# cucibala/FaceRecognizeOnnx

Measured on AMD Instinct MI355X. Metric: faces/sec end-to-end (detect+align+embed), batch=128 640x640, higher is better.
Workload: dtype f32; 1 GPU; C-headline: 128 frames 640x640 per GPU, SCRFD det_500m + decode + NMS, first 1 face(s)/frame aligned to 112x112, IResNet-50 (w600k_r50) embed, L2-norm; frames_per_gpu=128, faces_per_frame=1, weights=synthetic seeded (det seed 100, rec seed 200), input_residency=HBM-resident before the timed region, gallery_rows=0, topk=0, parallelism=frame-sharded x1, no data-path collective

## Files before the change

### facerecognizeonnx_amd/_lib.py

```python
from __future__ import annotations

import ctypes as C
import os
import subprocess

import numpy as np

_HERE = os.path.dirname(os.path.abspath(__file__))
LIB_PATH = os.path.join(_HERE, "libfacehip.so")
CSRC = os.path.join(_HERE, "csrc")

FACE_DTYPE = np.dtype([("x", "<i4"), ("y", "<i4"), ("w", "<i4"), ("h", "<i4"),
                       ("score", "<f4"), ("lm", "<f4", (10,))])
assert FACE_DTYPE.itemsize == 60


class FhFace(C.Structure):
    _fields_ = [("x", C.c_int32), ("y", C.c_int32), ("w", C.c_int32), ("h", C.c_int32),
                ("score", C.c_float), ("lm", C.c_float * 10)]


class FhFrame(C.Structure):
    _fields_ = [("bgr", C.c_void_p), ("rows", C.c_int32), ("cols", C.c_int32), ("step", C.c_int32)]

# ... 90 lines not shown
    "fh_det_input_dev": (_vp, [_vp]),
    "fh_det_postprocess_dev": (_i, [_vp, _i, _f, _f, _vp, _i, _vp, _vp]),
    "fh_postprocess_rows_dev": (_i, [_vp, _i, _i, _i, _f, _f, _f, _vp, _i, _vp, _vp]),
    "fh_rec_create": (_vp, [C.c_char_p]),
    "fh_rec_destroy": (None, [_vp]),
    "fh_rec_input_size": (_i, [_vp, _ip, _ip]),
    "fh_rec_feature_dim": (_i, [_vp]),
    "fh_rec_macs_per_face": (_d, [_vp]),
    "fh_rec_act_bytes_per_face": (_d, [_vp]),
    "fh_rec_set_chunk": (_i, [_vp, _i]),
    "fh_rec_extract": (_i, [_vp, _vp, _i, _i, _i, _vp, _vp, _i]),
    "fh_rec_extract_simple": (_i, [_vp, _vp, _i, _i, _i, _vp, _i]),
    "fh_compare": (_f, [_vp, _i, _vp, _i]),
    "fh_rec_embed_aligned_dev": (_i, [_vp, _vp, _i, _vp, _vp, _vp]),
    "fh_rec_run_input_dev": (_i, [_vp, _vp, _i, _vp, _vp, _vp]),
    "fh_rec_align_dev": (_i, [_vp, _vp, _i, _i, _i, _ll, _vp, _vp, _i, _vp, _vp, _vp]),
    "fh_rec_input_dev": (_vp, [_vp]),
    "fh_rec_embed_faces_dev": (_i, [_vp, _vp, _i, _i, _i, _ll, _vp, _vp, _i, _vp, _vp, _vp]),
    "fh_pipeline_run_dev": (_i, [_vp, _vp, _vp, _i, _i, _i, _i, _ll, _f, _f, _i, _vp, _vp, _vp, _vp]),
    "fh_pipeline_submit_dev": (_i, [_vp, _vp, _vp, _i, _i, _i, _i, _ll, _f, _f, _i, _vp, _vp, _vp, _vp, _vp, _vp]),
    "fh_letterbox_plan": (_i, [_i, _i, _i, _i, _ip, _ip, C.POINTER(C.c_float)]),
    "fh_det_letterbox_ragged_dev": (_i, [_vp, _vp, _i, _vp, _vp]),
    "fh_det_run_network_ragged_dev": (_i, [_vp, _vp, _i, _vp]),
    "fh_det_detect_ragged_dev": (_i, [_vp, _vp, _i, _f, _f, _vp, _i, _vp, _vp]),
    "fh_rec_align_ragged_dev": (_i, [_vp, _vp, _i, _vp, _vp, _i, _vp, _vp, _vp]),
    "fh_rec_embed_faces_ragged_dev": (_i, [_vp, _vp, _i, _vp, _vp, _i, _vp, _vp, _vp]),
    "fh_pipeline_run_ragged_dev": (_i, [_vp, _vp, _vp, _i, _f, _f, _i, _vp, _vp, _vp, _vp]),
    "fh_pipeline_run_images": (_i, [_vp, _vp, _vp, _i, _f, _f, _i, _vp, _vp, _vp, _i]),
    "fh_tile_plan": (_i, [_i, _i, _vp, _vp, _i]),
    "fh_det_detect_tiled_dev": (_i, [_vp, _vp, _i, _vp, _f, _f, _vp, _i, _vp, _vp]),
    "fh_det_run_network_tiled_dev": (_i, [_vp, _vp, _i, _vp, _vp]),
    "fh_postprocess_rows_tiled_dev": (_i, [_vp, _vp, _vp, _i, _vp, _i, _i, _i, _i, _f, _f, _vp, _i, _vp, _vp]),
    "fh_pipeline_run_tiled_dev": (_i, [_vp, _vp, _vp, _i, _vp, _f, _f, _i, _vp, _vp, _vp, _vp]),
    "fh_det_detect_tiled": (_i, [_vp, _vp, _i, _i, _i, _vp, _f, _f, _vp, _i]),
    "fh_stream_create": (_vp, [_vp, _vp, _i, _i, _i, _i]),
    "fh_stream_destroy": (None, [_vp]),
    "fh_stream_submit": (_i, [_vp, _vp, _i, _f, _f]),
    "fh_stream_collect": (_i, [_vp, _vp, _vp, _vp, _i]),
    "fh_tracker_create": (_vp, [_i, _i, _f, _i, _i]),
    "fh_tracker_destroy": (None, [_vp]),
    "fh_tracker_reset": (_i, [_vp, _i]),
    "fh_tracker_get_state": (_i, [_vp, _i, _vp, _ip, _ip]),
    "fh_track_plan": (_i, [_vp, _i, _i, _vp, _vp]),
    "fh_track_update_dev": (_i, [_vp, _vp, _vp, _i, _i, _vp, _vp, _vp, _vp]),
    "fh_track_select_dev": (_i, [_vp, _vp, _i, _i, _vp, _vp, _vp, _vp, _vp, _vp]),
    "fh_pipeline_run_tracked_dev": (_i, [_vp, _vp, _vp, _vp, _i, _i, _i, _i, _ll, _vp, _f, _f, _i, _vp, _vp, _vp, _vp, _vp, _vp, _vp, _vp]),
    "fh_track_update_slots_dev": (_i, [_vp, _vp, _vp, _i, _i, _vp, _vp, _vp, _vp, _vp]),
    "fh_tracker_enable_identity": (_i, [_vp, _i, _i]),
    "fh_track_identify_dev": (_i, [_vp, _vp, _f, _vp, _vp, _vp, _vp, _i, _i, _i, _vp, _vp, _vp, _vp]),
    "fh_tracker_queries_dev": (_vp, [_vp]),
    "fh_tracker_get_identity": (_i, [_vp, _i, _vp, _vp]),
    "fh_pipeline_run_identified_dev": (_i, [_vp, _vp, _vp, _vp, _f, _vp, _i, _i, _i, _i, _ll, _vp, _f, _f, _i, _vp, _vp, _vp, _vp, _vp, _vp, _vp,
                                            _vp, _vp, _vp]),
    "fh_face_quality_dev": (_i, [_vp, _i, _i, _i, _i, _ll, _vp, _vp, _i, _vp, _vp]),
    "fh_face_quality_ragged_dev": (_i, [_vp, _i, _vp, _vp, _i, _vp, _vp]),
    "fh_tracker_set_bestshot": (_i, [_vp, _i, _i, _i, _i]),
    "fh_tracker_get_quality": (_i, [_vp, _i, _vp]),
    "fh_tracker_quality_dev": (_vp, [_vp]),
    "fh_track_update_q_dev": (_i, [_vp, _vp, _vp, _i, _i, _vp, _vp, _vp, _vp, _vp, _vp]),
    "fh_track_identify_q_dev": (_i, [_vp, _vp, _f, _vp, _vp, _vp, _vp, _vp, _i, _i, _i, _vp, _vp, _vp, _vp]),
    "fh_tracker_enable_relink": (_i, [_vp, _i, _f, _i]),
    "fh_track_identify_link_dev": (_i, [_vp, _vp, _f, _vp, _vp, _vp, _vp, _vp, _i, _i, _i, _vp, _vp, _vp, _vp, _vp]),
    "fh_tracker_get_links": (_i, [_vp, _i, _vp, _vp]),
    "fh_tracker_roots_dev": (_vp, [_vp]),
    "fh_gallery_create": (_vp, [_i]),
    "fh_gallery_destroy": (None, [_vp]),
    "fh_gallery_upload": (_i, [_vp, _vp, _ll, _i, _ll]),
    "fh_gallery_enroll": (_ll, [_vp, _vp, _ll, _i]),
    "fh_gallery_size": (_ll, [_vp]),
    "fh_gallery_label_dev": (_i, [_vp, _vp, _i, _f, _vp, _vp, _vp]),
    "fh_gallery_topk_dev": (_i, [_vp, _vp, _i, _i, _vp, _vp, _vp]),
    "fh_gallery_set_scan": (_i, [_vp, _i]),
    "fh_gallery_get_scan": (_i, [_vp]),
    "fh_gallery_scan_stats": (_i, [_vp, C.POINTER(_ll), C.POINTER(_ll)]),
    "fh_topk_merge_dev": (_i, [_vp, _vp, _i, _i, _i, _vp, _vp, _vp]),
    "fh_gallery_enroll_ids": (_ll, [_vp, _vp, _vp, _ll, _i]),
    "fh_gallery_upload_ids": (_i, [_vp, _vp, _vp, _ll, _i, _ll]),
    "fh_gallery_topk_ids_dev": (_i, [_vp, _vp, _i, _i, _vp, _vp, _vp, _vp]),
    "fh_gallery_label_ids_dev": (_i, [_vp, _vp, _i, _f, _vp, _vp, _vp]),
    "fh_gallery_remove_ids": (_ll, [_vp, _vp, _ll]),
    "fh_gallery_get_ids": (_ll, [_vp, _ll, _ll, _vp]),
    "fh_topk_merge_ids_dev": (_i, [_vp, _vp, _vp, _i, _i, _i, _vp, _vp, _vp, _vp]),
    "fh_gallery_group_ids": (_ll, [_vp, _ll, _vp, _vp, _vp]),
    "fh_gallery_fuse_ids": (_ll, [_vp, _vp, _i]),
    "fh_gallery_get_rows": (_ll, [_vp, _ll, _ll, _vp]),
    "fh_gallery_self_scores_dev": (_i, [_vp, _vp, _vp, _vp]),
    "fh_cluster_scores": (_i, [_vp, _i, _f, _i, _i, _vp, _vp]),
    "fh_gallery_cluster_dev": (_i, [_vp, _f, _i, _i, _vp, _vp, _vp]),
    "fh_hist_bin": (_i, [_f]),
    "fh_roc_from_hist": (_i, [_vp, _d, _vp]),
    "fh_gallery_pair_hist_dev": (_i, [_vp, _vp, _vp, _vp]),
    "fh_pairs_from_scores": (_i, [_vp, _i, _vp, _i, _i, _f, _i, _ll, _vp, _vp, _vp, _vp]),
    "fh_gallery_pairs_dev": (_i, [_vp, _i, _i, _f, _i, _vp, _vp, _vp, _vp, _vp]),
    "fh_gallery_set_ids": (_ll, [_vp, _vp, _i]),
    "fh_gallery_set_tags": (_ll, [_vp, _ll, _ll, _vp, _i]),
    "fh_gallery_get_tags": (_ll, [_vp, _ll, _ll, _vp]),
    "fh_gallery_topk_tagged_dev": (_i, [_vp, _vp, _vp, _i, _i, _vp, _vp, _vp]),
    "fh_gallery_topk_ids_tagged_dev": (_i, [_vp, _vp, _vp, _i, _i, _vp, _vp, _vp, _vp]),
    "fh_gallery_label_tagged_dev": (_i, [_vp, _vp, _vp, _i, _f, _vp, _vp, _vp]),
    "fh_gallery_label_ids_tagged_dev": (_i, [_vp, _vp, _vp, _i, _f, _vp, _vp, _vp]),
    "fh_gallery_tag_stats": (_i, [_vp, C.POINTER(_ll), C.POINTER(_ll)]),
    "fh_tracker_set_stream_masks": (_i, [_vp, _vp]),
    "fh_gallery_range_dev": (_i, [_vp, _vp, _vp, _i, _f, _i, _vp, _vp, _vp, _vp, _vp]),
    "fh_range_from_scores": (_i, [_vp, _ll, _ll, _vp, C.c_uint32, _f, _i, C.POINTER(_ll), _vp, _vp]),
    "fh_gallery_topk_deep_dev": (_i, [_vp, _vp, _vp, _i, _i, _vp, _vp, _vp, _vp]),
    "fh_topk_from_scores": (_i, [_vp, _ll, _ll, _vp, C.c_uint32, _i, _vp, _vp]),
    "fh_debug_deep_blocks": (_i, [_vp, _ll, _vp, C.c_uint32, _i, _vp]),
    "fh_comm_unique_id": (_i, [_vp]),
    "fh_comm_create": (_vp, [_i, _i, _vp, _i]),
    "fh_comm_destroy": (None, [_vp]),
    "fh_comm_rank": (_i, [_vp]),
    "fh_comm_world": (_i, [_vp]),
    "fh_comm_allgather_f32_dev": (_i, [_vp, _vp, _vp, _ll, _vp]),
    "fh_gallery_topk_sharded_dev": (_i, [_vp, _vp, _vp, _i, _i, _vp, _vp, _vp]),
    "fh_timing_enable": (_i, [_i]),
    "fh_timing_num_tags": (_i, []),
    "fh_timing_collect": (_i, [_vp, _vp, _vp, _vp, _i]),
    "fh_timing_collect_ops": (_i, [_vp, _vp, _vp, _i]),
    "fh_det_set_conv_cfg": (_i, [_vp, _i, _i]),
    "fh_rec_set_conv_cfg": (_i, [_vp, _i, _i]),
    "fh_memcpy_d2h": (_i, [_vp, _vp, C.c_size_t]),
    "fh_det_sync": (_i, [_vp, _vp]),
    "fh_rec_sync": (_i, [_vp, _vp]),
    "fh_imread": (_i, [C.c_char_p, C.POINTER(_vp), C.POINTER(_i), C.POINTER(_i)]),
    "fh_image_decode": (_i, [_vp, C.c_size_t, C.POINTER(_vp), C.POINTER(_i), C.POINTER(_i)]),
    "fh_image_free": (None, [_vp]),
    "fh_jpeg_header": (_i, [_vp, C.c_size_t, _vp]),
    "fh_jpeg_entropy": (_i, [_vp, C.c_size_t, _vp, _vp, C.c_size_t]),
    "fh_jpeg_reconstruct": (_i, [_vp, _vp, _vp, _i]),
    "fh_jpeg_desc_check": (_i, [_vp]),
    "fh_jpegdec_create": (_vp, []),
    "fh_jpegdec_destroy": (None, [_vp]),
    "fh_jpeg_reconstruct_batch_dev": (_i, [_vp, _vp, _i, _vp, _vp, _vp, _vp]),
    "fh_jpeg_decode_batch": (_i, [_vp, _vp, _i, _i, _vp, _vp, _vp]),
    "fh_pipeline_run_files": (_i, [_vp, _vp, _vp, _vp, _i, _i, _f, _f, _i, _vp, _vp, _vp, _i, _vp]),
    "fh_jpeg_quant_tables": (_i, [_i, _vp, _vp]),
    "fh_jpeg_enc_desc": (_i, [_i, _i, _i, _i, _i, _vp]),
    "fh_jpeg_enc_check": (_i, [_vp]),
    "fh_jpeg_forward": (_i, [_vp, _vp, _i, _vp, C.c_size_t]),
    "fh_jpeg_write": (_i, [_vp, _vp, _vp, C.c_size_t, _vp]),
    "fh_jpeg_write_bound": (C.c_size_t, [_vp]),
    "fh_imwrite_jpeg": (_i, [C.c_char_p, _vp, _i, _i, _i, _i, _i]),
    "fh_jpegenc_create": (_vp, []),
    "fh_jpegenc_destroy": (None, [_vp]),
    "fh_jpeg_forward_batch_dev": (_i, [_vp, _vp, _i, _vp, _vp, _vp, _vp]),
    "fh_jpeg_encode_batch": (_i, [_vp, _vp, _i, _i, _i, _i, _vp, _vp]),
    "fh_det_set_winograd": (_i, [_vp, _i]),
    "fh_rec_set_winograd": (_i, [_vp, _i]),
    "fh_rec_set_wino_fusion": (_i, [_vp, _i]),
    "fh_rec_set_wino_x3": (_i, [_vp, _i]),
    "fh_rec_get_wino_x3": (_i, [_vp]),
    "fh_rec_get_conv_x3": (_i, [_vp]),
    "fh_rec_get_pw_x3": (_i, [_vp]),
    "fh_det_set_x3": (_i, [_vp, _i]),
    "fh_det_get_x3": (_i, [_vp]),
    "fh_rec_set_shortcut_fold": (_i, [_vp, _i]),
    "fh_rec_set_precision": (_i, [_vp, _i, C.POINTER(C.c_float)]),
    "fh_rec_get_precision": (_i, [_vp]),
    "fh_det_set_cus": (_i, [_vp, _i]),
    "fh_rec_set_cus": (_i, [_vp, _i]),
    "fh_debug_streamk": (_i, [_i, _i]),
    "fh_debug_conv_plan": (_i, [_i, _vp, _i, _vp, _i]),
    "fh_debug_wino_slots": (_i, [_i]),
    "fh_debug_cluster_tiles": (_i, [_i]),
    "fh_debug_hist_copies": (_i, [_i]),
    "fh_debug_pairs_room": (_i, [_i]),
    "fh_debug_tag_skip": (_i, [_i]),
    "fh_debug_topk_merge_strided_dev": (_i, [_vp, _vp, _i, _i, _i, _ll, _vp, _vp, _vp]),
    "fh_set_graph_replay": (_i, [_i]),
    "fh_det_workspace_dev": (_vp, [_vp]),
    "fh_det_graph_stats": (_i, [_vp, _vp]),
    "fh_rec_graph_stats": (_i, [_vp, _vp]),
    "fh_det_set_fused_stem": (_i, [_vp, _i]),
    "fh_rec_set_fused_stem": (_i, [_vp, _i]),
    "fh_det_set_fused_front": (_i, [_vp, _i]),
    "fh_det_set_halo_conv": (_i, [_vp, _i]),
    "fh_resize_u8c3_dev": (_i, [_vp, _i, _i, _i, _vp, _i, _i, _i, _vp]),
    "fh_conv_forward_dev": (_i, [_vp, _vp, _vp, _vp, _i, _i, _i, _i, _i, _i, _i, _i, _i, _vp]),
    "fh_conv_forward_ex_dev": (_i, [_vp, _vp, _vp, _vp, _i, _i, _i, _i, _i, _i, _i, _i, _i, _i, _vp, _i, _i, _i, _i, _i, _vp]),
    "fh_conv_forward_ep_dev": (_i, [_vp, _vp, _vp, _vp, _i, _i, _i, _i, _i, _i, _i, _i, _i, _i, _vp, _i, _i, _i, _i, _i, _i, _vp, _vp]),
    "fh_conv_winograd_dev": (_i, [_vp, _vp, _vp, _vp, _i, _i, _i, _i, _i, _vp]),
    "fh_conv_winograd_ex_dev": (_i, [_vp, _vp, _vp, _vp, _i, _i, _i, _i, _i, _i, _vp]),
    "fh_debug_pack_bf16x2_dev": (_i, [_vp, _vp, _ll]),
    "fh_debug_wino_gemm_rows": (_ll, [_i, _i, _i, _i, _i, _i]),
    "fh_debug_wino_gemm_dev": (_i, [_vp, _vp, _vp, _i, _i, _i, _i, _i, _i, _i, _vp]),
    "fh_debug_wino2_clock_mhz": (_d, []),
    "fh_conv_wino2_dev": (_i, [_vp, _vp, _vp, _vp, _vp, _vp, _i, _i, _i, _i, _i, _i, _i, _vp]),
    "fh_conv_wino2_ex_dev": (_i, [_vp, _vp, _vp, _vp, _vp, _vp, _vp, _vp, _vp, _i, _vp, _vp, _vp, _i, _i, _i, _i, _i, _i, _i, _vp]),
    "fh_conv_wt_rows": (_i, [_i]),
    "fh_conv_pack_weights": (_i, [_vp, _i, _i, _i, _vp]),
    "fh_conv_kpad": (_i, [_i]),
}

_LIB = None


def lib() -> C.CDLL:
    global _LIB
    if _LIB is None:
        path = build()
        path = os.environ.get("FACEHIP_LIB") or path
        try:
            import torch
        except ImportError:
            pass
        L = C.CDLL(path)
        for name, (res, args) in PROTOTYPES.items():
            fn = getattr(L, name)
            fn.restype = res
            fn.argtypes = args
        _LIB = L
    return _LIB


def last_error() -> str:
    return lib().fh_last_error().decode(errors="replace")


class FaceHipError(RuntimeError):
    pass


def check(rc: int, what: str) -> int:
    if rc < 0:
        raise FaceHipError(f"{what} failed ({rc}): {last_error()}")
    return rc
```

### facerecognizeonnx_amd/csrc/api.cpp

```cpp
#include <algorithm>
#include <atomic>
#include <cmath>
#include <cstddef>
#include <cstdio>
#include <cstring>
#include <memory>
#include <string>
#include <thread>
#include <vector>

#include "../../include/facehip.h"
#include "cluster_plan.h"
#include "deep_plan.h"
#include "pairs_plan.h"
#include "range_plan.h"
#include "roc_plan.h"
#include "engine.h"
#include "group_ids.h"
#include "jpeg_dev.h"
#include "jpeg_enc.h"
#include "track_plan.h"

static_assert(sizeof(fh_face) == 60 && sizeof(fh::FaceRec) == 60, "FaceBox mirror must stay 60 bytes");
static_assert(sizeof(fh_frame) == 24 && sizeof(fh::FrameIn) == 24 && offsetof(fh_frame, rows) == offsetof(fh::FrameIn, rows) &&
// ... 1650 lines not shown
    return FH_OK;
}
int fh_gallery_pair_hist_dev(fh_gallery* g, unsigned long long* d_hist, unsigned long long* d_nan, void* stream) {
    if (!g || !d_hist) return arg_error("fh_gallery_pair_hist_dev: null argument");
    if (g->g.size() > 0 && !g->g.labelled()) {
        g_err = "gallery: fh_gallery_pair_hist_dev needs a labelled gallery (rows enrolled with ids, or fh_gallery_set_ids)";
        return FH_ERR_STATE;
    }
    return guarded([&] { g->g.pair_hist_dev(d_hist, d_nan, S(stream)); return (int)FH_OK; });
}
int fh_debug_hist_copies(int copies) { fh::cluster_debug_hist_copies(copies); return 0; }

static_assert(FH_PAIRS_GENUINE == fh::kPairsGenuine && FH_PAIRS_IMPOSTOR == fh::kPairsImpostor && FH_PAIRS_ANY == fh::kPairsAny &&
              FH_PAIRS_ABOVE == fh::kPairsAbove && FH_PAIRS_NOT_ABOVE == fh::kPairsNotAbove && FH_PAIRS_MAX_CAP == fh::kPairsMaxCap &&
              FH_PAIRS_ROOM == fh::kPairsRoom, "facehip.h mirrors pairs_plan.h and kernels.h");
namespace {
const char* bad_pairs(int cls, int side, float threshold, int cap) {
    if (threshold != threshold) return "the threshold is a NaN";
    if (cls != FH_PAIRS_GENUINE && cls != FH_PAIRS_IMPOSTOR && cls != FH_PAIRS_ANY) return "unknown class";
    if (side != FH_PAIRS_ABOVE && side != FH_PAIRS_NOT_ABOVE) return "unknown side";
    if (cap < 1 || cap > FH_PAIRS_MAX_CAP) return "need 1 <= cap <= FH_PAIRS_MAX_CAP";
    return nullptr;
}
}
int fh_pairs_from_scores(const float* scores, int n, const int* ids, int cls, int side, float threshold, int cap, long long room,
                         unsigned long long* info, float* out_scores, int* out_rows, int* out_ids) {
    if (const char* why = bad_pairs(cls, side, threshold, cap)) return frames_error("fh_pairs_from_scores", why);
    int listed = -1;
    const int rc = guarded([&] {
        listed = fh::pairs_from_scores(scores, n, ids, cls, side, threshold, cap, room, info, out_scores, out_rows, out_ids);
        return 0;
    });
    if (rc < 0) return rc;
    return listed < 0 ? arg_error("fh_pairs_from_scores: bad argument (n < 0, null scores or info, a class without ids, room < cap)") : listed;
}
int fh_gallery_pairs_dev(fh_gallery* g, int cls, int side, float threshold, int cap, unsigned long long* d_info, float* d_scores, int* d_rows,
                         int* d_ids, void* stream) {
    if (!g || !d_info) return arg_error("fh_gallery_pairs_dev: null argument");
    if (const char* why = bad_pairs(cls, side, threshold, cap)) return frames_error("fh_gallery_pairs_dev", why);
    if (g->g.dim() % 64) return arg_error("fh_gallery_pairs_dev: the gallery's dim must be a multiple of 64");
    if ((cls != FH_PAIRS_ANY || d_ids) && g->g.size() > 0 && !g->g.labelled()) {
        g_err = "gallery: fh_gallery_pairs_dev with a class other than FH_PAIRS_ANY or with d_ids needs a labelled gallery (rows enrolled with "
                "ids, or fh_gallery_set_ids)";
        return FH_ERR_STATE;
    }
    return guarded([&] { g->g.pairs_dev(cls, side, threshold, cap, d_info, d_scores, d_rows, d_ids, S(stream)); return (int)FH_OK; });
}
int fh_debug_pairs_room(int room) { fh::pairs_debug_room(room); return 0; }

static_assert(FH_RANGE_MAX_CAP == fh::kRangeMaxCap && FH_TAG_ALL == fh::kRangeTagAll, "facehip.h mirrors range_plan.h");
int fh_range_from_scores(const float* scores, long long n, long long index_base, const uint32_t* tags, uint32_t mask, float threshold, int cap,
                         long long* count, float* out_scores, int* out_indices) {
    int listed = -1;
    const int rc = guarded([&] {
        listed = fh::range_from_scores(scores, n, index_base, tags, mask, threshold, cap, count, out_scores, out_indices);
        return 0;
    });
    if (rc < 0) return rc;
    return listed < 0 ? arg_error("fh_range_from_scores: bad argument (null scores or count, NaN threshold, cap outside 1..1024, index beyond 31 bits)")
                      : listed;
}
int fh_gallery_range_dev(fh_gallery* g, const float* d_queries, const uint32_t* d_masks, int nq, float threshold, int cap, long long* d_counts,
                         float* d_scores, int* d_indices, int* d_ids, void* stream) {
    if (!g) return arg_error("fh_gallery_range_dev: null handle");
    if (nq < 0 || nq > 256) return arg_error("fh_gallery_range_dev: need 0 <= nq <= 256");
    if (cap < 1 || cap > FH_RANGE_MAX_CAP) return arg_error("fh_gallery_range_dev: need 1 <= cap <= FH_RANGE_MAX_CAP");
    if (threshold != threshold) return arg_error("fh_gallery_range_dev: the threshold is a NaN");
    if (g->g.dim() % 64) return arg_error("fh_gallery_range_dev: the gallery's dim must be a multiple of 64");
    if (nq == 0) return 0;
    if (!d_queries || !d_counts) return arg_error("fh_gallery_range_dev: null argument");
    if (d_ids && g->g.size() > 0 && !g->g.labelled()) {
        g_err = "gallery: fh_gallery_range_dev with d_ids needs a labelled gallery (rows enrolled with ids, or fh_gallery_set_ids)";
        return FH_ERR_STATE;
    }
    return guarded([&] { g->g.range_dev(d_queries, d_masks, nq, threshold, cap, d_counts, d_scores, d_indices, d_ids, S(stream)); return nq; });
}

static_assert(FH_TOPK_DEEP_MAX == fh::kDeepMaxK && FH_TOPK_DEEP_MAX == fh::GAL_DEEP_MAX, "facehip.h and kernels.h mirror deep_plan.h");
int fh_topk_from_scores(const float* scores, long long n, long long index_base, const uint32_t* tags, uint32_t mask, int k, float* out_scores,
                        int* out_indices) {
    int listed = -1;
    const int rc = guarded([&] {
        listed = fh::topk_from_scores(scores, n, index_base, tags, mask, k, out_scores, out_indices);
        return 0;
    });
    if (rc < 0) return rc;
    return listed < 0 ? arg_error("fh_topk_from_scores: bad argument (null scores, k outside 1..1024, index beyond 31 bits)") : listed;
}
int fh_debug_deep_blocks(const float* scores, long long n, const uint32_t* tags, uint32_t mask, int k, long long* out_blocks) {
    if (!out_blocks) return arg_error("fh_debug_deep_blocks: null argument");
    int chosen = -1;
    const int rc = guarded([&] {
        std::vector<long long> blocks;
        chosen = fh::deep_chosen_blocks(scores, n, tags, mask, k, &blocks);
        std::copy(blocks.begin(), blocks.end(), out_blocks);
        return 0;
    });
    if (rc < 0) return rc;
    return chosen < 0 ? arg_error("fh_debug_deep_blocks: bad argument (null scores, k outside 1..1024)") : chosen;
}
int fh_gallery_topk_deep_dev(fh_gallery* g, const float* d_queries, const uint32_t* d_masks, int nq, int k, float* d_scores, int* d_indices,
                             int* d_ids, void* stream) {
    if (!g) return arg_error("fh_gallery_topk_deep_dev: null handle");
    if (nq < 0 || nq > 256) return arg_error("fh_gallery_topk_deep_dev: need 0 <= nq <= 256");
    if (k < 1 || k > FH_TOPK_DEEP_MAX) return arg_error("fh_gallery_topk_deep_dev: need 1 <= k <= FH_TOPK_DEEP_MAX");
    if (g->g.dim() % 64) return arg_error("fh_gallery_topk_deep_dev: the gallery's dim must be a multiple of 64");
    if (!d_scores && !d_indices && !d_ids) return arg_error("fh_gallery_topk_deep_dev: all three list pointers are null");
    if (nq == 0) return 0;
    if (!d_queries) return arg_error("fh_gallery_topk_deep_dev: null argument");
    if (d_ids && g->g.size() > 0 && !g->g.labelled()) {
        g_err = "gallery: fh_gallery_topk_deep_dev with d_ids needs a labelled gallery (rows enrolled with ids, or fh_gallery_set_ids)";
        return FH_ERR_STATE;
    }
    return guarded([&] { g->g.topk_deep_dev(d_queries, d_masks, nq, k, d_scores, d_indices, d_ids, S(stream)); return nq; });
}

int fh_debug_topk_merge_strided_dev(const float* ps, const int* pi, int nparts, int nq, int k, long long part_stride, float* scores, int* indices,
                                    void* stream) {
    if (!ps || !pi || !scores || !indices) return arg_error("fh_debug_topk_merge_strided_dev: null argument");
    if (nparts <= 0 || nq <= 0 || k <= 0 || k > 16 || (long)nparts * k > 65536 || part_stride < (long long)nq * k)
        return arg_error("fh_debug_topk_merge_strided_dev: bad size");
    return guarded([&] {
        fh::launch_topk_merge_strided(ps, pi, nparts, nq, k, (long)part_stride, scores, indices, S(stream));
        FH_HIP(hipGetLastError());
        return nq;
    });
}

int fh_timing_enable(int on) { fh::KernelTimer::get().enabled = on != 0; return FH_OK; }
int fh_timing_num_tags(void) { return fh::KernelTimer::kTags; }
int fh_timing_collect(double* ms, double* flops, double* bytes, long long* launches, int n) {
    if (!ms || !flops || !bytes || !launches || n < fh::KernelTimer::kTags) return arg_error("fh_timing_collect: need fh_timing_num_tags()-entry arrays");
    return guarded([&] { fh::KernelTimer::get().collect(ms, flops, bytes, launches); return fh::KernelTimer::kTags; });
}
int fh_timing_collect_ops(double* ms, double* flops, int* tag, int cap) {
    if (!ms || !flops || !tag || cap <= 0) return arg_error("fh_timing_collect_ops: bad argument");
    return guarded([&] { return fh::KernelTimer::get().collect_ops(ms, flops, tag, cap); });
}
int fh_det_set_conv_cfg(fh_det* d, int cfg, int stream_k) {
    if (!d) return arg_error("null handle");
    d->det.net().force_cfg = cfg; d->det.net().sk_enable = stream_k != 0;
    return FH_OK;
}
int fh_det_set_winograd(fh_det* d, int on) { if (!d) return arg_error("null handle"); d->det.net().winograd = on != 0; return FH_OK; }
int fh_rec_set_winograd(fh_rec* r, int on) { if (!r) return arg_error("null handle"); r->rec.net().winograd = on != 0; return FH_OK; }
int fh_rec_set_wino_x3(fh_rec* r, int on) {
    if (!r) return arg_error("null handle");
    Owns owns(&r->rec.net());
    return guarded([&] { return r->rec.net().set_wino_x3(on != 0, nullptr); });
}
int fh_rec_get_wino_x3(fh_rec* r) { return r && r->rec.net().wino_x3() ? 1 : 0; }
int fh_rec_get_conv_x3(fh_rec* r) { return r ? r->rec.net().conv_x3_layers() : 0; }
int fh_rec_get_pw_x3(fh_rec* r) { return r ? r->rec.net().pw_x3_layers() : 0; }
int fh_det_set_x3(fh_det* d, int on) {
    if (!d) return arg_error("null handle");
    Owns owns(&d->det.net());
    return guarded([&] { return d->det.net().set_pw_x3(on != 0, nullptr); });
}
int fh_det_get_x3(fh_det* d) { return d ? d->det.net().pw_x3_layers() : 0; }
int fh_rec_set_wino_fusion(fh_rec* r, int on) { if (!r) return arg_error("null handle"); r->rec.net().fuse_wino = on != 0; return FH_OK; }
int fh_rec_set_precision(fh_rec* r, int mode, float* worst_out) {
    if (!r || (mode != FH_PREC_FP32 && mode != FH_PREC_BF16X2)) return arg_error("fh_rec_set_precision: bad argument");
    if (worst_out) *worst_out = 0.f;
    Owns owns(&r->rec.net());
    if (mode == FH_PREC_FP32) return guarded([&] { r->rec.net().set_bf16x2(false, nullptr); return (int)FH_OK; });
    return guarded([&] {
        fh::Net& net = r->rec.net();
        const int n = 64, dim = r->rec.dim();
        const size_t crop = (size_t)net.in_h() * net.in_w() * 3;
        std::vector<uint8_t> h((size_t)n * crop);
        uint32_t st = 0x9E3779B9u;
        for (int i = 0; i < n; ++i) {
            const int amp = 16 + 3 * i;
            for (size_t e = 0; e < crop; ++e) {
                st = st * 1664525u + 1013904223u;
                const int px = (int)(e / 3) % net.in_w(), py = (int)(e / 3) / net.in_w();
                const int v = 128 + ((px * (i + 1) + py * (n - i)) % 97 - 48) + (int)((st >> 24) % (2 * amp + 1)) - amp;
                h[(size_t)i * crop + e] = (uint8_t)std::min(255, std::max(0, v));
            }
        }
        fh::DevBuf dc, de;
        dc.ensure(h.size()); de.ensure((size_t)2 * n * dim * sizeof(float));
        FH_HIP(hipMemcpy(dc.p, h.data(), h.size(), hipMemcpyHostToDevice));
        const bool was = net.bf16x2();
        net.set_bf16x2(false, nullptr);
        r->rec.embed_aligned_dev(dc.as<uint8_t>(), n, de.as<float>(), nullptr);
        const int layers = net.set_bf16x2(true, nullptr);
        if (layers == 0) { net.set_bf16x2(was, nullptr); throw std::runtime_error("fh_rec_set_precision: this model has no layer with a split-bf16 form"); }
        struct Rollback { fh::Net& n; bool armed = true; ~Rollback() { if (armed) { try { n.set_bf16x2(false, nullptr); } catch (...) {} } } } rollback{net};
        r->rec.embed_aligned_dev(dc.as<uint8_t>(), n, de.as<float>() + (size_t)n * dim, nullptr);
        std::vector<float> e((size_t)2 * n * dim);
        FH_HIP(hipDeviceSynchronize());
        FH_HIP(hipMemcpy(e.data(), de.p, e.size() * sizeof(float), hipMemcpyDeviceToHost));
        double worst = 0;
        for (int i = 0; i < n; ++i) {
            double dot = 0, na = 0, nb = 0;
            for (int c = 0; c < dim; ++c) {
                const double a = e[(size_t)i * dim + c], b = e[(size_t)(n + i) * dim + c];
                dot += a * b; na += a * a; nb += b * b;
            }
            const double err = (na > 0 && nb > 0) ? 1.0 - dot / std::sqrt(na * nb) : 1.0;
            worst = std::max(worst, std::isfinite(err) ? err : 1.0);
        }
        if (worst_out) *worst_out = (float)worst;
        double gate = 1e-3;
        if (const char* g = getenv("FACEHIP_PRECISION_GATE")) gate = std::min(gate, atof(g));
        if (!(worst < gate))
            throw std::runtime_error("fh_rec_set_precision: split-bf16 embeddings differ from fp32 by 1 - cos = " + std::to_string(worst) +
                                 " (gate " + std::to_string(gate) + "): staying fp32");
        rollback.armed = false;
        return layers;
    });
}
int fh_rec_get_precision(fh_rec* r) { return r && r->rec.net().bf16x2() ? FH_PREC_BF16X2 : FH_PREC_FP32; }
int fh_rec_set_shortcut_fold(fh_rec* r, int on) { if (!r) return arg_error("null handle"); r->rec.net().fold_shortcut = on != 0; return FH_OK; }
int fh_det_set_halo_conv(fh_det* d, int on) { if (!d) return arg_error("null handle"); d->det.net().halo_conv = on != 0; return FH_OK; }
int fh_det_set_cus(fh_det* d, int cus) { if (!d || cus < 0) return arg_error("bad argument"); d->det.net().cus = cus; return FH_OK; }
int fh_rec_set_cus(fh_rec* r, int cus) { if (!r || cus < 0) return arg_error("bad argument"); r->rec.net().cus = cus; return FH_OK; }
int fh_det_set_fused_stem(fh_det* d, int on) { if (!d) return arg_error("null handle"); d->det.net().fuse_stem = on != 0; return FH_OK; }
int fh_det_set_fused_front(fh_det* d, int on) { if (!d) return arg_error("null handle"); d->det.net().fuse_front = on != 0; return FH_OK; }
int fh_rec_set_fused_stem(fh_rec* r, int on) { if (!r) return arg_error("null handle"); r->rec.net().fuse_stem = on != 0; return FH_OK; }
int fh_rec_set_conv_cfg(fh_rec* r, int cfg, int stream_k) {
    if (!r) return arg_error("null handle");
    r->rec.net().force_cfg = cfg; r->rec.net().sk_enable = stream_k != 0;
    return FH_OK;
}

int fh_memcpy_d2h(void* dst, const void* src, size_t bytes) {
    if (!dst || !src) return arg_error("fh_memcpy_d2h: null argument");
    return guarded([&] { FH_HIP(hipDeviceSynchronize()); FH_HIP(hipMemcpy(dst, src, bytes, hipMemcpyDeviceToHost)); return 0; });
}
int fh_resize_u8c3_dev(const uint8_t* src, int sh, int sw, int sstep, uint8_t* dst, int dh, int dw, int dstep, void* stream) {
    if (!src || !dst || sh <= 0 || sw <= 0 || dh <= 0 || dw <= 0) return arg_error("fh_resize_u8c3_dev: bad argument");
    return guarded([&] {
        fh::launch_resize_u8c3(src, (long)sh * sstep, sh, sw, sstep, dst, (long)dh * dstep, dh, dw, dstep, 1, S(stream));
        FH_HIP(hipGetLastError());
        return 0;
    });
}
int fh_conv_winograd_ex_dev(const float* d_in, const float* w_ohwi, const float* d_bias, float* d_out, int batch, int h, int w, int cin,
                            int cout, int precision, void* stream) {
    if (!d_in || !w_ohwi || !d_out || cin % 32 || cout % 4 || (precision != FH_PREC_FP32 && precision != FH_PREC_BF16X2 && precision != FH_PREC_F32X3))
        return arg_error("fh_conv_winograd_dev: bad argument");
    const bool bf2 = precision == FH_PREC_BF16X2, x3 = precision == FH_PREC_F32X3;
    Owns owns(nullptr);
    return guarded([&] {
        if ((bf2 || x3) && !fh::wino_gemm_ok_bf16x2(cin, cout)) throw std::runtime_error("winograd: this layer has no split-bf16 GEMM");
        const int rows = fh::conv_wt_rows(cout);
        std::vector<float> u36((size_t)36 * rows * cin, 0.f), uf((size_t)cout * cin);
        std::vector<double> uall((size_t)cout * cin * 36);
        for (int co = 0; co < cout; ++co)
            for (int ci = 0; ci < cin; ++ci) {
                double g[9];
                for (int t = 0; t < 9; ++t) g[t] = w_ohwi[((size_t)co * 9 + t) * cin + ci];
                fh::wino_filter_transform(g, &uall[((size_t)co * cin + ci) * 36]);
            }
        for (int f = 0; f < 36; ++f) {
            for (size_t e = 0; e < uf.size(); ++e) uf[e] = (float)uall[e * 36 + f];
            fh::conv_pack_weights(uf.data(), cout, cin, 1, u36.data() + (size_t)f * rows * cin);
        }
        const size_t tiles = (size_t)batch * ((h + 3) / 4) * ((w + 3) / 4);
        fh::DevBuf dU, dV, dM;
        dU.ensure(u36.size() * sizeof(float));
        dV.ensure((36 * (size_t)fh::wino_rows((long)tiles) + 100 * 128) * cin * sizeof(float));
        dM.ensure((36 * (size_t)fh::wino_rows((long)tiles) + 100 * 128) * cout * sizeof(float));
        FH_HIP(hipMemcpy(dU.p, u36.data(), u36.size() * sizeof(float), hipMemcpyHostToDevice));
        fh::DevBuf dUp;
        if (bf2) {
            dUp.ensure(u36.size() * sizeof(float));
            fh::launch_pack_bf16x2(dU.as<float>(), dUp.as<float>(), (long)u36.size(), S(stream));
        } else if (x3) {
            dUp.ensure(36 * fh::wino_x3_floats(rows, cin) * sizeof(float));
            fh::launch_pack_x3(dU.as<float>(), dUp.as<float>(), rows, cin, S(stream));
        }
        static fh::DevBuf slabs;
        static unsigned slabs_gen = 0;
        if (!slabs.p) { slabs.ensure(fh::conv_slab_floats() * sizeof(float)); fh::conv_workspace_init(slabs.as<float>()); slabs_gen = fh::conv_error_generation(); }
        if (slabs_gen != fh::conv_error_generation()) { fh::conv_workspace_reset_async(slabs.as<float>(), S(stream)); slabs_gen = fh::conv_error_generation(); }
        fh::ConvArgs a{};
        a.in = d_in; a.bias = d_bias; a.out1 = d_out; a.slabs = slabs.as<float>(); a.sk_enable = 1;
        a.B = batch; a.H = h; a.W = w; a.Ho = h; a.Wo = w; a.Cin = cin; a.Cout = cout; a.ks = 3; a.stride = 1; a.pad = 1;
        a.act = (int)fh::Act::NONE; a.res_mode = (int)fh::ResMode::NONE;
        fh::launch_conv_winograd(a, (bf2 || x3 ? dUp : dU).as<float>(), dV.as<float>(), dM.as<float>(), 2, nullptr, nullptr, S(stream), precision);
        FH_HIP(hipStreamSynchronize(S(stream)));
        return 0;
    });
}
int fh_conv_winograd_dev(const float* d_in, const float* w_ohwi, const float* d_bias, float* d_out, int batch, int h, int w, int cin,
                         int cout, void* stream) {
    return fh_conv_winograd_ex_dev(d_in, w_ohwi, d_bias, d_out, batch, h, w, cin, cout, FH_PREC_FP32, stream);
}
int fh_debug_pack_bf16x2_dev(const float* d_in, float* d_out, long long n) {
    if (!d_in || !d_out || n < 0 || n % 4) return arg_error("fh_debug_pack_bf16x2_dev: bad argument (n % 4 == 0)");
    return guarded([&] {
        fh::launch_pack_bf16x2(d_in, d_out, (long)n, nullptr);
        FH_HIP(hipGetLastError());
        FH_HIP(hipStreamSynchronize(nullptr));
        return 0;
    });
}
static long long wino_gemm_rows(int batch, int h, int w, int k, int n, int mixed, fh::WinoPlanes* pl) {
    if (batch <= 0 || h <= 0 || w <= 0 || k <= 0 || n <= 0 || k % 32 || n % 32) return -1;
    if (!mixed) return 36LL * fh::wino_rows((long)batch * ((h + 3) / 4) * ((w + 3) / 4));
    fh::WinoPlanes p{};
    if (!fh::wino_mix_layout(batch, h, w, k, n, &p)) return -2;
    if (pl) *pl = p;
    return 128LL * p.total_tiles;
}
long long fh_debug_wino_gemm_rows(int batch, int h, int w, int k, int n, int mixed) {
    const long long r = wino_gemm_rows(batch, h, w, k, n, mixed, nullptr);
    if (r == -2) return arg_error("fh_debug_wino_gemm_rows: the mixed tiling does not apply to this layer");
    if (r < 0) return arg_error("fh_debug_wino_gemm_rows: bad argument (k % 32 == 0, n % 32 == 0)");
    return r;
}
int fh_debug_wino_gemm_dev(const float* d_V, const float* d_U, float* d_M, int batch, int h, int w, int k, int n, int precision, int mixed,
                           void* stream) {
    if (!d_V || !d_U || !d_M || (precision != FH_PREC_FP32 && precision != FH_PREC_BF16X2 && precision != FH_PREC_F32X3))
        return arg_error("fh_debug_wino_gemm_dev: bad argument");
    fh::WinoPlanes pl{};
    const long long rows = wino_gemm_rows(batch, h, w, k, n, mixed, &pl);
    if (rows == -2) return arg_error("fh_debug_wino_gemm_dev: the mixed tiling does not apply to this layer");
    if (rows < 0) return arg_error("fh_debug_wino_gemm_dev: bad argument (k % 32 == 0, n % 32 == 0)");
    const bool bf2 = precision == FH_PREC_BF16X2, x3 = precision == FH_PREC_F32X3;
    Owns owns(nullptr);
    return guarded([&] {
        if ((bf2 || x3) && !fh::wino_gemm_ok_bf16x2(k, n)) throw std::runtime_error("winograd: this layer has no split-bf16 GEMM");
        const size_t nv = (size_t)rows * k, nu = (size_t)36 * fh::conv_wt_rows(n) * k;
        fh::DevBuf dVp, dUp;
        if (bf2) {
            dVp.ensure(nv * sizeof(float)); dUp.ensure(nu * sizeof(float));
            fh::launch_pack_bf16x2(d_V, dVp.as<float>(), (long)nv, S(stream));
            fh::launch_pack_bf16x2(d_U, dUp.as<float>(), (long)nu, S(stream));
        } else if (x3) {
            dUp.ensure(36 * fh::wino_x3_floats(fh::conv_wt_rows(n), k) * sizeof(float));
            fh::launch_pack_x3(d_U, dUp.as<float>(), fh::conv_wt_rows(n), k, S(stream));
        }
        fh::ConvArgs a{};
        a.B = batch; a.H = h; a.W = w; a.Ho = h; a.Wo = w; a.Cin = k; a.Cout = n; a.ks = 3; a.stride = 1; a.pad = 1;
        a.act = (int)fh::Act::NONE; a.res_mode = (int)fh::ResMode::NONE;
        fh::launch_wino_gemm(a, bf2 || x3 ? dUp.as<float>() : d_U, bf2 ? dVp.as<float>() : d_V, d_M, 2, precision, S(stream), mixed ? &pl : nullptr);
        FH_HIP(hipGetLastError());
        FH_HIP(hipStreamSynchronize(S(stream)));
        return 0;
    });
}
int fh_conv_wino2_ex_dev(const float* d_in, const float* w_ohwi, const float* d_bias, const float* d_slope, const float* d_res, float* d_out,
                         float* d_out2, const float* d_s2, const float* d_t2, int n_outs, float* const* d_outs, const int* oc0, const int* oact,
                         int batch, int h, int w, int cin, int cout, int act, int bias_cls, void* stream) {
    if (!d_in || !w_ohwi || batch <= 0 || h <= 0 || w <= 0 || cin != 64 || cout <= 0) return arg_error("fh_conv_wino2_dev: bad argument (cin = 64, positive sizes)");
    if (n_outs < 0 || n_outs > 3 || (n_outs > 0 && (!d_outs || !oc0 || !oact))) return arg_error("fh_conv_wino2_dev: bad merged-output description");
    if (n_outs == 0 && ((!d_out && !d_out2) || cout % 64)) return arg_error("fh_conv_wino2_dev: plain layers need an output and cout % 64 == 0");
    if (d_out2 && (!d_s2 || !d_t2)) return arg_error("fh_conv_wino2_dev: a second output needs its scale and shift");
    Owns owns(nullptr);
    return guarded([&] {
        fh::ConvArgs a{};
        a.in = d_in; a.bias = d_bias; a.slope = d_slope; a.res = d_res; a.out1 = d_out; a.out2 = d_out2; a.s2 = d_s2; a.t2 = d_t2;
        a.B = batch; a.H = h; a.W = w; a.Ho = h; a.Wo = w; a.Cin = cin; a.Cout = cout; a.ks = 3; a.stride = 1; a.pad = 1;
        a.act = act; a.bias_cls = bias_cls; a.res_mode = d_res ? (int)fh::ResMode::SAME : (int)fh::ResMode::NONE;
        a.n_outs = n_outs;
        for (int g = 0; g < n_outs; ++g) { a.outs[g] = d_outs[g]; a.oact[g] = oact[g]; a.oc0[g] = oc0[g]; }
        if (n_outs > 0) a.oc0[n_outs] = oc0[n_outs];
        if (!fh::wino2_ok(a)) throw std::runtime_error("fh_conv_wino2_dev: layer shape not supported by the fused F(2x2) kernel");
        std::vector<float> u(fh::wino2_weight_floats(cin, cout));
        fh::wino2_pack_weights(w_ohwi, cout, cin, u.data());
        fh::DevBuf dU;
        dU.ensure(u.size() * sizeof(float));
        FH_HIP(hipMemcpy(dU.p, u.data(), u.size() * sizeof(float), hipMemcpyHostToDevice));
        a.wt = dU.as<float>();
        fh::launch_wino2(a, S(stream));
        FH_HIP(hipGetLastError());
        FH_HIP(hipStreamSynchronize(S(stream)));
        return 0;
    });
}
int fh_conv_wino2_dev(const float* d_in, const float* w_ohwi, const float* d_bias, const float* d_slope, const float* d_res, float* d_out,
                      int batch, int h, int w, int cin, int cout, int act, int bias_cls, void* stream) {
    return fh_conv_wino2_ex_dev(d_in, w_ohwi, d_bias, d_slope, d_res, d_out, nullptr, nullptr, nullptr, 0, nullptr, nullptr, nullptr, batch, h, w,
                                cin, cout, act, bias_cls, stream);
}
double fh_debug_wino2_clock_mhz(void) { return fh::wino2_debug_clock_mhz(); }
int fh_conv_wt_rows(int cout) { return fh::conv_wt_rows(cout); }
int fh_conv_pack_weights(const float* w_ohwi, int cout, int cin, int ksize, float* dst_packed) {
    if (!w_ohwi || !dst_packed || cout <= 0 || cin <= 0) return arg_error("fh_conv_pack_weights: bad argument");
    memset(dst_packed, 0, (size_t)fh::conv_wt_rows(cout) * fh::conv_kpad(ksize * ksize * cin) * sizeof(float));
    fh::conv_pack_weights(w_ohwi, cout, cin, ksize, dst_packed);
    return 0;
}
int fh_conv_kpad(int ktot) { return fh::conv_kpad(ktot); }
const float* fh_det_workspace_dev(fh_det* d) { return d ? d->det.net().workspace() : nullptr; }
int fh_set_graph_replay(int on) { g_graph_replay = on != 0; return FH_OK; }
int fh_det_graph_stats(fh_det* d, long long* replays) {
    if (!d) return arg_error("null handle");
    if (replays) *replays = d->gcall.replays;
    return (int)d->gcall.nodes;
}
int fh_rec_graph_stats(fh_rec* r, long long* replays) {
    if (!r) return arg_error("null handle");
    if (replays) *replays = r->gcall.replays + r->gcall_simple.replays;
    return (int)(r->gcall.nodes ? r->gcall.nodes : r->gcall_simple.nodes);
}
int fh_debug_wino_slots(int slots) { fh::wino_debug_slots(slots); return 0; }
int fh_debug_streamk(int drop_publish, int timeout_ms) { fh::conv_debug_streamk(drop_publish, timeout_ms); return 0; }
int fh_debug_conv_plan(int what, const int* in, int n_in, long long* out, int n_out) {
    static const int BMs[4] = {128, 256, 128, 64}, BNs[4] = {128, 64, 32, 64};
    const fh::ConvKnobs knobs;
    auto need = [&](int ni, int no) { return n_in == ni && n_out == no && out && (in || !ni); };
    auto geom = [&] {
        const int Ho = (in[1] + 2 * in[7] - in[5]) / in[6] + 1, Wo = (in[2] + 2 * in[7] - in[5]) / in[6] + 1;
        return fh::ConvGeom{(long)in[0] * Ho * Wo, in[1], in[2], in[3], Ho, Wo, in[4], in[5], in[6], in[7], fh::conv_kpad(in[5] * in[5] * in[3]), in[8],
                            false, false, in[9] != 0, false};
    };
    auto shape_ok = [&] { return in[0] > 0 && in[1] > 0 && in[2] > 0 && in[3] > 0 && in[4] > 0 && in[5] > 0 && in[6] > 0 && in[7] >= 0 && in[10] > 0 &&
                                 in[1] + 2 * in[7] >= in[5] && in[2] + 2 * in[7] >= in[5]; };
    if (what == 0 && need(8, 9) && in[0] >= 0 && in[1] > 0 && in[2] > 0 && in[3] > 0 && in[4] > 0) {
        const fh::ConvSkPlan p = fh::conv_streamk_plan(in[0], in[1], in[2], in[3], in[4], in[5], in[6], in[7] != 0, knobs);
        const int v[9] = {p.full, p.rem, p.helpers, p.owners, p.fixup, p.units, p.q, p.owner_chunks, p.maxp};
        for (int i = 0; i < 9; ++i) out[i] = v[i];
    } else if (what == 1 && need(11, 1) && shape_ok()) {
        out[0] = fh::conv_pw_bn(geom(), in[10], knobs);
    } else if (what == 2 && need(12, 3) && shape_ok() && in[11] >= -1 && in[11] < 4) {
        const fh::ConvGeom g = geom();
        const int cfg = in[11] < 0 ? fh::conv_pick_cfg(g.M, g.Cout) : in[11], BM = BMs[cfg], BN = BNs[cfg];
        const int tiles_n = (g.Cout + BN - 1) / BN, tiles = (int)((g.M + BM - 1) / BM) * tiles_n;
        fh::ConvTallPlan t{0, 0, 0};
        if (cfg == 1 || cfg == 2) t = fh::conv_tall_plan(g, BM, BN, 32, tiles, tiles_n, in[10], knobs);
        out[0] = t.tiles; out[1] = t.tiles ? t.rows_a : 0; out[2] = t.tiles ? (long long)t.lds : 0;
    } else if (what == 3 && need(4, 2) && in[0] >= 0 && in[1] > in[0] && in[2] > 0 && in[3] > 0) {
        out[0] = out[1] = fh::conv_sk_nparts(in[0], in[2], in[3]);
        for (int r = in[0] + 1; r < in[1]; ++r) {
            const int n = fh::conv_sk_nparts(r, in[2], in[3]);
            if (n < out[0]) out[0] = n;
            if (n > out[1]) out[1] = n;
        }
    } else if (what == 4 && need(0, 2)) {
        out[0] = (long long)fh::SK_SLAB_FLOATS; out[1] = (long long)fh::SK_COUNTERS;
    } else if (what == 5 && need(4, 2) && in[0] >= 0 && in[1] > 0 && in[2] > 0 && in[3] > 0) {
        out[0] = fh::conv_x3_pays(in[0], in[1], in[2], in[3], knobs) ? 1 : 0; out[1] = fh::conv_x3_bn(in[2]);
    } else if (what == 6 && need(11, 3) && shape_ok()) {
        const fh::ConvGeom g = geom();
        const int bn = fh::conv_pw_x3_bn(g, in[10], knobs);
        out[0] = bn; out[1] = bn ? (g.M / 128) * ((g.Cout + bn - 1) / bn) : 0;
        out[2] = bn && fh::conv_pw_x3_pays(out[1], g.Kpad, g.Cout, in[10], knobs) ? 1 : 0;
    } else if (what == 7 && need(4, 1) && in[0] >= 0 && in[1] > 0 && in[2] > 0 && in[3] > 0) {
        out[0] = fh::conv_pw_x3_pays(in[0], in[1], in[2], in[3], knobs) ? 1 : 0;
    } else {
        return arg_error("fh_debug_conv_plan: unknown question, wrong array lengths or a non-positive size");
    }
    return n_out;
}
int fh_conv_forward_dev(const float* in, const float* wt, const float* bias, float* out, int batch, int h, int w, int cin, int cout,
                        int ks, int stride, int kpad, int cfg, void* stream) {
    return fh_conv_forward_ex_dev(in, wt, bias, out, batch, h, w, cin, cout, ks, stride, kpad, cfg, FH_PREC_FP32, nullptr, 0, 0, 0, 0, 0, stream);
}
int fh_conv_forward_ex_dev(const float* in, const float* wt, const float* bias, float* out, int batch, int h, int w, int cin, int cout,
                           int ks, int stride, int kpad, int cfg, int precision, const float* sc_in, int sc_h, int sc_w, int sc_c, int sc_stride,
                           int cus, void* stream) {
    return fh_conv_forward_ep_dev(in, wt, bias, out, batch, h, w, cin, cout, ks, stride, kpad, cfg, precision, sc_in, sc_h, sc_w, sc_c, sc_stride, cus,
                                  0, nullptr, stream);
}
int fh_conv_forward_ep_dev(const float* in, const float* wt, const float* bias, float* out, int batch, int h, int w, int cin, int cout,
                           int ks, int stride, int kpad, int cfg, int precision, const float* sc_in, int sc_h, int sc_w, int sc_c, int sc_stride,
                           int cus, int act, const float* res, void* stream) {
    static const char* const no_pw_x3 = "fh_conv_forward_ex_dev: this 1x1 layer has no three-piece bf16 form (it needs stride 1, cin % 4 == 0, "
                                        "cout % 4 == 0, kpad % 32 == 0, whole 128-row tiles and a tile per CU)";
    const bool x3 = precision == FH_PREC_F32X3, pw3 = x3 && ks == 1;
    if (pw3 && in && wt && out && batch > 0 && cin > 0 && cout > 0 && (cin % 4 || cout % 4 || stride != 1 || sc_in || kpad % 32 || kpad < cin))
        return arg_error(no_pw_x3);
    if (!in || !wt || !out || batch <= 0 || (ks != 1 && ks != 3) || cin % 4 || cout <= 0 || stride <= 0 || cus < 0 || (act != 0 && act != 1) ||
        (precision != FH_PREC_FP32 && precision != FH_PREC_F32X3) || (sc_in && (sc_h <= 0 || sc_w <= 0 || sc_c <= 0 || sc_stride <= 0)))
        return arg_error("fh_conv_forward_dev: bad argument");
    if (x3 && !pw3 && !fh::conv_x3_ok(cin, cout))
        return arg_error("fh_conv_forward_ex_dev: this layer has no three-piece bf16 form (it needs cin % 32 == 0 and cout % 64 == 0)");
    Owns owns(nullptr);
    return guarded([&] {
        fh::ConvArgs a{};
        const int pad = ks / 2;
        a.in = in; a.wt = wt; a.bias = bias; a.out1 = out;
        a.B = batch; a.H = h; a.W = w; a.Cin = cin; a.Cout = cout; a.ks = ks; a.stride = stride; a.pad = pad;
        a.Ho = (h + 2 * pad - ks) / stride + 1; a.Wo = (w + 2 * pad - ks) / stride + 1;
        a.Kpad = kpad;
        a.cus = cus;
        a.act = act;
        if (res) { a.res = res; a.res_mode = (int)fh::ResMode::SAME; }
        if (sc_in) {
            if ((a.Ho - 1) * sc_stride >= sc_h || (a.Wo - 1) * sc_stride >= sc_w) throw std::runtime_error("conv: the shortcut's input does not cover the output grid");
            a.sc_in = sc_in; a.sc_H = sc_h; a.sc_W = sc_w; a.sc_C = sc_c; a.sc_stride = sc_stride;
        }
        static fh::DevBuf slabs;
        static unsigned slabs_gen = 0;
        if (!slabs.p) { slabs.ensure(fh::conv_slab_floats() * sizeof(float)); fh::conv_workspace_init(slabs.as<float>()); slabs_gen = fh::conv_error_generation(); }
        if (slabs_gen != fh::conv_error_generation()) { fh::conv_workspace_reset_async(slabs.as<float>(), S(stream)); slabs_gen = fh::conv_error_generation(); }
        a.slabs = slabs.as<float>(); a.sk_enable = 1;
        if (x3) {
            static fh::DevBuf w3;
            const int rows = fh::conv_wt_rows(cout);
            FH_HIP(hipStreamSynchronize(S(stream)));
            w3.ensure(fh::wino_x3_floats(rows, kpad) * sizeof(float));
            fh::launch_pack_x3(wt, w3.as<float>(), rows, kpad, S(stream), 1);
            if (pw3) {
                if (!fh::launch_conv_pw_x3(a, w3.as<float>(), true, S(stream))) throw std::invalid_argument(no_pw_x3);
            } else {
                a.wt = w3.as<float>();
                fh::launch_conv_x3(a, 0, S(stream));
            }
            FH_HIP(hipGetLastError());
            FH_HIP(hipStreamSynchronize(S(stream)));
            return 0;
        }
        fh::launch_conv(a, cfg, S(stream));
        FH_HIP(hipGetLastError());
        return 0;
    });
}

}

namespace fh {
Gallery& gallery_of(fh_gallery* g) { return g->g; }
}
```

### facerecognizeonnx_amd/csrc/conv_plan.h

```cpp
#pragma once
#include <cstddef>
#include <cstdlib>

#if defined(__HIPCC__)
#define FH_CONV_HD __host__ __device__
#else
#define FH_CONV_HD
#endif

namespace fh {

constexpr size_t SK_SLAB_FLOATS = (size_t)2 * 1280 * 128 * 128;
constexpr size_t SK_COUNTERS = 4096;

struct ConvKnobs {
    int sk_b_ratio = 4;
    int sk_min_owner = 12;
    int sk_margin2 = 3;
    int tall_tail_q = 3;
    int conv_pw = 1;
    int conv_tall = 1;
    int ep_direct = 0;
    int conv_x3 = 1;
    int pw_x3 = 1;
    int pw_x3_bn = 0;
};
inline const ConvKnobs& conv_knobs() {
    static const ConvKnobs k = [] {
        ConvKnobs v;
        auto env = [](const char* name, int& x) { if (const char* e = getenv(name)) x = atoi(e); };
        env("FACEHIP_SK_B_RATIO", v.sk_b_ratio); env("FACEHIP_SK_MIN_OWNER", v.sk_min_owner); env("FACEHIP_SK_MARGIN", v.sk_margin2);
        env("FACEHIP_TALL_TAIL_Q", v.tall_tail_q); env("FACEHIP_CONV_PW", v.conv_pw); env("FACEHIP_CONV_TALL", v.conv_tall);
        env("FACEHIP_EP_DIRECT", v.ep_direct); env("FACEHIP_CONV_X3", v.conv_x3); env("FACEHIP_PW_X3", v.pw_x3); env("FACEHIP_PW_X3_BN", v.pw_x3_bn);
        return v;
    }();
    return k;
}

struct ConvGeom {
    long M;
    int H, W, Cin, Ho, Wo, Cout, ks, stride, pad, Kpad, n_outs;
    bool grouped, sc, up2x, no_pw;
};

inline int conv_pick_cfg(long M, int Cout) {
    auto cols = [&](int bn) { return (Cout + bn - 1) / bn * bn; };
    int bn = 32;
    if (cols(64) * 10 <= cols(32) * 11) bn = 64;
    if (cols(128) * 10 <= cols(bn) * 11) bn = 128;
    if (bn == 128) return 0;
    if (bn == 64) return (M / 256) * (cols(64) / 64) >= 1024 ? 1 : 3;
    return 2;
}

inline int conv_x3_bn(int Cout) { return Cout <= 0 ? 0 : Cout % 128 == 0 ? 128 : Cout % 64 == 0 ? 64 : 0; }
inline bool conv_x3_pays(long tiles, int Kpad, int Cout, int cus, const ConvKnobs& k) {
    if (!k.conv_x3 || !conv_x3_bn(Cout) || Kpad % 32 || cus <= 0) return false;
    if (k.conv_x3 == 2) return true;
    return tiles * 16 >= (long)cus && Kpad >= 640;
}

inline double conv_tile_us(long tile_floats, int Kpad) { return 2.0 * tile_floats * (double)Kpad / 0.43e6; }

inline int conv_pw_bn(const ConvGeom& g, int cus, const ConvKnobs& k) {
    if (!k.conv_pw || g.no_pw || g.ks != 1 || g.stride != 1 || g.pad != 0 || g.grouped || g.sc || g.n_outs > 0 || (g.Cin & 3) || (g.Cout & 3) ||
        (g.M & 127) || g.H != g.Ho || g.W != g.Wo || g.Kpad % 32 || g.Kpad < g.Cin)
        return 0;
    auto cols = [&](int bn) { return (g.Cout + bn - 1) / bn * bn; };
    int bn = 32;
    if (cols(64) * 100 <= g.Cout * 107) bn = 64;
    if (cols(96) * 100 <= g.Cout * 107 && cols(96) <= cols(64)) bn = 96;
    return (g.M / 128) * (cols(bn) / bn) < (long)cus ? 0 : bn;
}

inline int conv_pw_x3_bn(const ConvGeom& g, int cus, const ConvKnobs& k) {
    if (!conv_pw_bn(g, cus, k)) return 0;
    auto cols = [&](int bn) { return (g.Cout + bn - 1) / bn * bn; };
    int bn = k.pw_x3_bn == 64 ? 64 : 32;
    if (cols(64) * 100 <= g.Cout * 107) bn = 64;
    if (cols(96) * 100 <= g.Cout * 107 && cols(96) <= cols(64)) bn = 96;
    return (g.M / 128) * (cols(bn) / bn) < (long)cus ? 0 : bn;
}
constexpr int PW_X3_MIN_KPAD = 64;
inline bool conv_pw_x3_pays(long tiles, int Kpad, int Cout, int cus, const ConvKnobs& k) {
    if (!k.pw_x3 || Cout <= 0 || (Cout & 3) || Kpad <= 0 || Kpad % 32 || cus <= 0) return false;
    if (k.pw_x3 == 2) return true;
    return tiles >= (long)cus * (Cout < 32 ? 2 : 1) && Kpad >= PW_X3_MIN_KPAD;
}

struct ConvTallPlan { int tiles, rows_a; size_t lds; };
inline ConvTallPlan conv_tall_plan(const ConvGeom& g, int BM, int BN, int rp, int T, int tiles_n, int cus, const ConvKnobs& k) {
    const int occ = BM == 256 ? 2 : 3;
    const int St = cus * occ;
    ConvTallPlan t{0, 0, 0};
    if (!k.conv_tall || g.grouped || g.sc || g.ks != 3 || g.stride != 1 || g.pad != 1 || (g.Cin & 31) || g.H != g.Ho || g.W != g.Wo || g.W > 112 ||
        !(BN == 32 ? g.n_outs > 0 || (g.Cout & 3) == 0 : g.n_outs == 0 && (g.Cout & 3) == 0) || g.up2x || T < St)
        return t;
    t.rows_a = (BM + 2 * g.W + 2 + rp - 1) / rp * rp;
    t.lds = ((size_t)t.rows_a * 8 + 2 * BN * 8) * 16;
    t.tiles = (T / St) * St;
    t.tiles -= t.tiles % tiles_n;
    if (t.tiles > 0 && T - t.tiles <= cus && conv_tile_us((long)BM * BN, g.Kpad) < 30.0) t.tiles = T;
    if (t.lds > (size_t)(160 / occ) * 1024) t.tiles = 0;
    return t;
}

FH_CONV_HD inline int conv_sk_nparts(int r, int Kh, int q) { return ((r + 1) * Kh - 1) / q - (r * Kh) / q + 1; }

struct ConvSkPlan { int full, rem, helpers, owners, fixup, units, q, owner_chunks, maxp; };
inline ConvSkPlan conv_streamk_plan(int T, int S, int chunks, long tile_floats, int cus, int Kpad, int tile0, bool slabs_ok, const ConvKnobs& k) {
    ConvSkPlan pl{(T / S) * S, 0, 0, 0, 0, 0, 1, 0, 1};
    const int R = T - pl.full;
    const bool cheap_whole = ((R + cus - 1) / cus - (double)R / cus) * conv_tile_us(tile_floats, Kpad) < 10.0;
    if (R > 0 && R * 10 <= S * 9 && slabs_ok && !cheap_whole) {
        const int H = S - R;
        const int q_o = (int)(((long)R * chunks + (long)H * k.sk_margin2 / 2 + S - 1) / S);
        const int Kh = chunks - q_o;
        if (Kh >= 1 && q_o >= k.sk_min_owner && R <= (int)SK_COUNTERS) {
            const long U = (long)R * Kh;
            const int q_h = (int)((U + H - 1) / H);
            const int maxp = (Kh + q_h - 1) / q_h + 1;
            if (maxp <= 3 && (size_t)R * maxp * tile_floats <= SK_SLAB_FLOATS) {
                pl.units = (int)U; pl.q = q_h; pl.owner_chunks = q_o; pl.maxp = maxp;
                pl.helpers = (int)((U + q_h - 1) / q_h); pl.owners = R;
            }
        }
        if (!pl.owners) {
            const long U = (long)R * chunks;
            int q = (int)((U + S - 1) / S);
            const int min_q = tile0 > 0 ? (chunks < k.tall_tail_q ? chunks : k.tall_tail_q) : chunks < 8 ? chunks : chunks >= 256 ? 24 : 8;
            if (q < min_q) q = min_q;
            const int maxp = (chunks + q - 1) / q + 1;
            if (q * k.sk_b_ratio <= chunks * 2 && q < chunks && (size_t)R * maxp * tile_floats <= SK_SLAB_FLOATS) {
                pl.units = (int)U; pl.q = q; pl.maxp = maxp;
                pl.helpers = (int)((U + q - 1) / q); pl.fixup = 1;
            }
        }
    }
    if (pl.helpers) pl.rem = R; else pl.full = T;
    return pl;
}

}
```

### facerecognizeonnx_amd/csrc/conv_wino2.hip

```cpp
#include <hip/hip_runtime.h>

#include <algorithm>
#include <cstdlib>
#include <cstring>
#include <stdexcept>
#include <vector>

#include "gemm_tile.h"
#include "kernels.h"
#include "plan.h"

namespace fh {

namespace {

__device__ __forceinline__ float act1(float v, bool relu, float sl) {
    const float a = v >= 0.f ? v : v * sl;
    return relu ? fmaxf(v, 0.f) : a;
}

constexpr int kYA[4] = {0, 1, 2, 1}, kYB[4] = {2, 2, 1, 3};
constexpr int kSA[4] = {1, 1, 1, 1}, kSB[4] = {-1, 1, -1, -1};
constexpr int kAT[2][4] = {{1, 1, 1, 0}, {0, 1, -1, -1}};

// ... 86 lines not shown
            if constexpr (c11 != 0) asm volatile("" : "+v"(Y[1][1][cb]));
        }
    };
    v4f d[2][4] = {};
    auto fetch_d = [&](auto fc, auto jc, auto bc) __attribute__((always_inline)) {
        constexpr int f = decltype(fc)::value, j = decltype(jc)::value, buf = decltype(bc)::value;
        constexpr int fi = f >> 2, fj = f & 3;
        constexpr int ya = kYA[fi], yb = kYB[fi], xa = kYA[fj], xb = kYB[fj];
        if (abl_d) return;
        unsigned gxr = j << 6;
        asm volatile("" : "+s"(gxr));
        d[buf][0] = *reinterpret_cast<lds_v4f>((size_t)(rb[ya * 4 + xa] ^ gxr));
        d[buf][1] = *reinterpret_cast<lds_v4f>((size_t)(rb[ya * 4 + xb] ^ gxr));
        d[buf][2] = *reinterpret_cast<lds_v4f>((size_t)(rb[yb * 4 + xa] ^ gxr));
        d[buf][3] = *reinterpret_cast<lds_v4f>((size_t)(rb[yb * 4 + xb] ^ gxr));
    };
    auto stage = [&](auto fc) __attribute__((always_inline)) {
        constexpr int f = decltype(fc)::value;
        constexpr int fi = f >> 2, fj = f & 3;
        constexpr int sab = kSA[fi] * kSB[fj], sba = kSB[fi] * kSA[fj], sbb = kSB[fi] * kSB[fj];
        v4f M[CB];
#pragma unroll
        for (int cb = 0; cb < CB; ++cb) M[cb] = v4f{0.f, 0.f, 0.f, 0.f};
        auto step = [&](auto jc) __attribute__((always_inline)) {
            constexpr int j = decltype(jc)::value, k = f * 4 + j;
            fetch_w(k + WD - 1 < 64, (k + WD - 1) % WD);
            if constexpr (j < 3) fetch_d(IC<f>{}, IC<j + 1>{}, IC<(k + 1) & 1>{});
            else if constexpr (f < 15) fetch_d(IC<f + 1>{}, IC<0>{}, IC<(k + 1) & 1>{});
            __builtin_amdgcn_sched_barrier(0);
            const v4f* dd = d[k & 1];
            v4f v = dd[0];
            v = sab > 0 ? v + dd[1] : v - dd[1];
            v = sba > 0 ? v + dd[2] : v - dd[2];
            v = sbb > 0 ? v + dd[3] : v - dd[3];
            asm volatile("" : "+v"(v));
            __builtin_amdgcn_sched_barrier(0);
#pragma unroll
            for (int e = 0; e < 4; ++e)
#pragma unroll
                for (int cb = 0; cb < CB; ++cb) M[cb] = __builtin_amdgcn_mfma_f32_16x16x4f32(wr[k % WD][cb][e], v[e], M[cb], 0, 0, 0);
            __builtin_amdgcn_sched_barrier(0);
        };
        step(IC<0>{}); step(IC<1>{});
        y_update(IC<(f + 15) & 15>{}, Mp);
        step(IC<2>{}); step(IC<3>{});
#pragma unroll
        for (int cb = 0; cb < CB; ++cb) Mp[cb] = M[cb];
        __builtin_amdgcn_sched_barrier(0);
    };
    fetch_w(false, 0);
#pragma unroll
    for (int q = 1; q < WD - 1; ++q) fetch_w(true, q);
    asm volatile("s_waitcnt vmcnt(0)" ::: "memory");
    if constexpr (NW > 1) __syncthreads();
    fetch_d(IC<0>{}, IC<0>{}, IC<0>{});
    stage(IC<0>{}); stage(IC<1>{}); stage(IC<2>{}); stage(IC<3>{}); stage(IC<4>{}); stage(IC<5>{}); stage(IC<6>{}); stage(IC<7>{});
    stage(IC<8>{}); stage(IC<9>{}); stage(IC<10>{}); stage(IC<11>{}); stage(IC<12>{}); stage(IC<13>{}); stage(IC<14>{}); stage(IC<15>{});
    y_update(IC<15>{}, Mp);

    asm volatile("" ::: "memory");
    __builtin_amdgcn_sched_barrier(0);
    if (abl_st && lane != 0) return;
    const int oy0 = 2 * (4 * gy + tr), ox0 = 2 * (4 * gx + tc);
    const int n0 = (tile_n * NW + wv) * 16 * CB, Cout = p.Cout;
    const float* __restrict__ res = p.res;
    float* __restrict__ out1 = p.out1;
    float* __restrict__ out2 = p.out2;
    const bool relu = p.act == (int)Act::RELU, prelu = p.act == (int)Act::PRELU;
    float bm[CB][4];
    if constexpr (MERGED) {
#pragma unroll
        for (int cb = 0; cb < CB; ++cb)
#pragma unroll
            for (int e = 0; e < 4; ++e) { const int co = n0 + 16 * cb + 4 * kq + e; bm[cb][e] = co < Cout ? p.bias[co] : 0.f; }
    }
#pragma unroll
    for (int a = 0; a < 2; ++a)
#pragma unroll
        for (int b = 0; b < 2; ++b) {
            const int oy = oy0 + a, ox = ox0 + b;
            if (!MERGED || oy >= p.Ho || ox >= p.Wo) continue;
            const size_t pix = ((size_t)gn * p.Ho + oy) * p.Wo + ox;
            if constexpr (MERGED) {
#pragma unroll
                for (int cb = 0; cb < CB; ++cb)
#pragma unroll
                    for (int e = 0; e < 4; e += 2) {
                        const int co = n0 + 16 * cb + 4 * kq + e;
                        if (co >= Cout) continue;
                        const int g = co >= p.oc0[2] && p.n_outs > 2 ? 2 : co >= p.oc0[1] ? 1 : 0;
                        const int cg = p.oc0[g + 1] - p.oc0[g], ga = p.oact[g];
                        auto fin = [&](float v) { return ga == (int)Act::RELU ? fmaxf(v, 0.f) : ga == (int)Act::SIGMOID ? 1.0f / (1.0f + expf(-v)) : v; };
                        float* const dst = p.outs[g] + pix * cg + (co - p.oc0[g]);
                        const float v0 = fin(Y[a][b][cb][e] + bm[cb][e]);
                        if (co + 1 < p.oc0[g + 1] && !((cg | (co - p.oc0[g])) & 1)) {
                            *reinterpret_cast<float2*>(dst) = float2{v0, fin(Y[a][b][cb][e + 1] + bm[cb][e + 1])};
                        } else {
                            dst[0] = v0;
                            if (co + 1 < Cout) {
                                const int g1 = co + 1 >= p.oc0[2] && p.n_outs > 2 ? 2 : co + 1 >= p.oc0[1] ? 1 : 0;
                                const int cg1 = p.oc0[g1 + 1] - p.oc0[g1], ga1 = p.oact[g1];
                                float v1 = Y[a][b][cb][e + 1] + bm[cb][e + 1];
                                v1 = ga1 == (int)Act::RELU ? fmaxf(v1, 0.f) : ga1 == (int)Act::SIGMOID ? 1.0f / (1.0f + expf(-v1)) : v1;
                                p.outs[g1][pix * cg1 + (co + 1 - p.oc0[g1])] = v1;
                            }
                        }
                    }
                continue;
            }
        }
    if constexpr (!MERGED) {
        const int n0 = (tile_n * NW + wv) * 16 * CB + 4 * kq;
        bool live[4]; size_t row[4]; v4f b4[4][CB], r4[4][CB], sl[CB];
#pragma unroll
        for (int cb = 0; cb < CB; ++cb) sl[cb] = prelu ? *reinterpret_cast<const v4f*>(p.slope + n0 + 16 * cb) : v4f{1.f, 1.f, 1.f, 1.f};
#pragma unroll
        for (int q = 0; q < 4; ++q) {
            const int oy = oy0 + (q >> 1), ox = ox0 + (q & 1);
            live[q] = oy < p.Ho && ox < p.Wo;
            const int oyc = min(oy, p.Ho - 1), oxc = min(ox, p.Wo - 1);
            row[q] = (((size_t)gn * p.Ho + oyc) * p.Wo + oxc) * Cout + n0;
            const int cls = p.bias_cls ? 3 * (oyc == 0 ? 0 : oyc == p.Ho - 1 ? 2 : 1) + (oxc == 0 ? 0 : oxc == p.Wo - 1 ? 2 : 1) : 0;
#pragma unroll
            for (int cb = 0; cb < CB; ++cb) {
                b4[q][cb] = p.bias ? *reinterpret_cast<const v4f*>(p.bias + cls * Cout + n0 + 16 * cb) : v4f{0.f, 0.f, 0.f, 0.f};
                if (p.res_mode != (int)ResMode::NONE) r4[q][cb] = *reinterpret_cast<const v4f*>(res + row[q] + 16 * cb);
            }
        }
#pragma unroll
        for (int q = 0; q < 4; ++q) {
            if (!live[q]) continue;
#pragma unroll
            for (int cb = 0; cb < CB; ++cb) {
                v4f v;
#pragma unroll
                for (int e = 0; e < 4; ++e) v[e] = act1(Y[q >> 1][q & 1][cb][e] + b4[q][cb][e], relu, sl[cb][e]);
                if (p.res_mode != (int)ResMode::NONE) v += r4[q][cb];
                if (out1) *reinterpret_cast<v4f*>(out1 + row[q] + 16 * cb) = v;
                if (out2) {
                    const v4f s2 = *reinterpret_cast<const v4f*>(p.s2 + n0 + 16 * cb), t2 = *reinterpret_cast<const v4f*>(p.t2 + n0 + 16 * cb);
                    *reinterpret_cast<v4f*>(out2 + row[q] + 16 * cb) = v * s2 + t2;
                }
            }
        }
    }
#ifdef FACEHIP_W2_PROF
    if (lane == 0 && p.slabs && blockIdx.x < (1u << 17)) {
        const long long dc = __builtin_readcyclecounter() - prof_c0, dr = (long long)__builtin_amdgcn_s_memrealtime() - prof_r0;
        reinterpret_cast<float*>(p.slabs)[blockIdx.x] = (float)(dc * 1000 / (dr + 1));
    }
#endif
}

bool shape_ok(int Cin, int Cout) { return Cin == 64 && (Cout % 64 == 0 || Cout <= 32); }

template <int CB, int NW, bool MERGED>
void launch_cb(const ConvArgs& a, hipStream_t s) {
    const int tgy = ((a.H + 1) / 2 + 3) / 4, tgx = ((a.W + 1) / 2 + 3) / 4;
    const long n_tg = (long)a.B * tgy * tgx;
    const int tiles_n = (a.Cout + 16 * CB * NW - 1) / (16 * CB * NW);
    static const bool lds_ok = [] {
        hipFuncAttributes fa{};
        FH_HIP(hipFuncGetAttributes(&fa, reinterpret_cast<const void*>(&wino2_kernel<CB, NW, MERGED>)));
        return fa.sharedSizeBytes % 256 == 0;
    }();
    if (!lds_ok) throw std::runtime_error("wino2: static LDS moved the halo off its 256-byte alignment (see the address XOR in fetch_d)");
    KernelTimer& timer = KernelTimer::get();
    timer.begin(s);
    hipLaunchKernelGGL((wino2_kernel<CB, NW, MERGED>), dim3((unsigned)(n_tg * tiles_n)), dim3(64 * NW), 25600, s, a, tiles_n, tgx, tgy, (int)n_tg);
    timer.end(s, 12, 2.0 * 16 * 16.0 * (double)n_tg * a.Cin * (16.0 * CB * NW * tiles_n), a.t_flops);
}

}

size_t wino2_weight_floats(int Cin, int Cout) { return (size_t)16 * Cin * (Cout <= 32 ? 32 : Cout); }
void wino2_pack_weights(const float* w, int Cout, int Cin, float* dst) {
    static const double Gm[4][3] = {{1, 0, 0}, {.5, .5, .5}, {.5, -.5, .5}, {0, 0, 1}};
    if (!shape_ok(Cin, Cout)) throw std::runtime_error("wino2_pack_weights: layer shape not supported");
    const int CB = Cout <= 32 ? 2 : 4;
    memset(dst, 0, wino2_weight_floats(Cin, Cout) * sizeof(float));
    for (int co = 0; co < Cout; ++co)
        for (int ci = 0; ci < Cin; ++ci) {
            double g[3][3], t[4][3];
            for (int k = 0; k < 9; ++k) g[k / 3][k % 3] = w[((size_t)co * 9 + k) * Cin + ci];
            for (int i = 0; i < 4; ++i)
                for (int x = 0; x < 3; ++x) t[i][x] = Gm[i][0] * g[0][x] + Gm[i][1] * g[1][x] + Gm[i][2] * g[2][x];
            const int tn = co / (16 * CB), cb = (co % (16 * CB)) / 16, m = co % 16;
            const int j = ci / 16, kq = (ci % 16) / 4, e = ci % 4;
            for (int i = 0; i < 4; ++i)
                for (int jj = 0; jj < 4; ++jj) {
                    const double u = t[i][0] * Gm[jj][0] + t[i][1] * Gm[jj][1] + t[i][2] * Gm[jj][2];
                    const size_t step = ((size_t)tn * 16 + (i * 4 + jj)) * 4 + j;
                    dst[(step * CB + cb) * 256 + (kq * 16 + m) * 4 + e] = (float)u;
                }
        }
}

bool wino2_ok(const ConvArgs& a) {
    if (!(a.ks == 3 && a.stride == 1 && a.pad == 1 && a.H == a.Ho && a.W == a.Wo && a.H >= 2 && a.W >= 2 && shape_ok(a.Cin, a.Cout) &&
          a.act != (int)Act::SIGMOID && !a.sc_in && !a.dw_w && !a.u8_src && a.wt_group_rows == 0 &&
          (a.res_mode == (int)ResMode::NONE || a.res_mode == (int)ResMode::SAME)))
        return false;
    if (a.n_outs > 0)
        return a.Cout <= 32 && a.res_mode == (int)ResMode::NONE && !a.out2 && !a.bias_cls;
    return a.Cout % 64 == 0;
}

static float* g_w2_clock = nullptr;
double wino2_debug_clock_mhz() {
    if (!g_w2_clock) return 0.0;
    std::vector<float> h(1 << 17);
    if (hipMemcpy(h.data(), g_w2_clock, h.size() * sizeof(float), hipMemcpyDeviceToHost) != hipSuccess) return 0.0;
    std::vector<float> v;
    for (float x : h) if (x > 0.f) v.push_back(x);
    if (v.empty()) return 0.0;
    std::nth_element(v.begin(), v.begin() + v.size() / 2, v.end());
    return v[v.size() / 2] / 10.0;
}

long wino2_blocks(const ConvArgs& a) {
    return (long)a.B * (((a.H + 1) / 2 + 3) / 4) * (((a.W + 1) / 2 + 3) / 4) * ((a.Cout + 63) / 64) / 4;
}

void launch_wino2(const ConvArgs& a_in, hipStream_t s) {
    if (!wino2_ok(a_in)) throw std::runtime_error("launch_wino2: layer shape not supported");
    ConvArgs a = a_in;
    a.zeros = conv_zero_line();
    static const int ablate = [] { const char* e = getenv("FACEHIP_W2_ABLATE"); return e ? atoi(e) : -1; }();
    a.sk_test_drop = ablate < 0 ? 0 : ablate;
    if (ablate >= 0 && !g_w2_clock) { void* q = nullptr; if (hipMalloc(&q, sizeof(float) << 17) == hipSuccess) g_w2_clock = (float*)q; }
    if (g_w2_clock) (void)hipMemsetAsync(g_w2_clock, 0, sizeof(float) << 17, s);
    a.slabs = g_w2_clock;
    static const int nw = [] { const char* e = getenv("FACEHIP_WINO2_NW"); return e ? atoi(e) : 2; }();
    if (a.Cout <= 32) launch_cb<2, 1, true>(a, s);
    else if (nw == 2) launch_cb<2, 2, false>(a, s);
    else launch_cb<4, 1, false>(a, s);
}

}
```

### facerecognizeonnx_amd/csrc/engine.cpp

```cpp
#include "engine.h"

#include "group_ids.h"
#include "roc_plan.h"

#include <atomic>
#include <climits>
#include <cstdio>
#include <cstdlib>
#include <algorithm>
#include <cmath>
#include <cstring>

namespace fh {

void hip_check(hipError_t e, const char* what) {
    if (e != hipSuccess) throw std::runtime_error(std::string("HIP error: ") + hipGetErrorString(e) + " in " + what);
}

static std::atomic<unsigned long long> g_layout_epoch{1};
unsigned long long layout_epoch() { return g_layout_epoch.load(std::memory_order_relaxed); }

DevBuf::~DevBuf() {
    if (p) { (void)hipFree(p); g_layout_epoch.fetch_add(1, std::memory_order_relaxed); }
}
// ... 6 lines not shown
}

KernelTimer& KernelTimer::get() { static KernelTimer t; return t; }
hipEvent_t KernelTimer::take() {
    if (!pool_.empty()) { hipEvent_t e = pool_.back(); pool_.pop_back(); return e; }
    hipEvent_t e; FH_HIP(hipEventCreate(&e)); return e;
}
void KernelTimer::begin(hipStream_t s) {
    if (!enabled) return;
    cur_ = take();
    FH_HIP(hipEventRecord(cur_, s));
}
void KernelTimer::end(hipStream_t s, int tag, double flops, double bytes) {
    if (!enabled || !cur_) return;
    hipEvent_t b = take();
    FH_HIP(hipEventRecord(b, s));
    recs_.push_back(Rec{cur_, b, tag, flops, bytes});
    cur_ = nullptr;
}
void KernelTimer::collect(double* ms, double* flops, double* bytes, long long* launches) {
    for (int i = 0; i < kTags; ++i) { ms[i] = 0; flops[i] = 0; bytes[i] = 0; launches[i] = 0; }
    for (auto& r : recs_) {
        FH_HIP(hipEventSynchronize(r.b));
        float t = 0.f;
        FH_HIP(hipEventElapsedTime(&t, r.a, r.b));
        ms[r.tag] += t; flops[r.tag] += r.flops; bytes[r.tag] += r.bytes; launches[r.tag] += 1;
        pool_.push_back(r.a); pool_.push_back(r.b);
    }
    recs_.clear();
}

int KernelTimer::collect_ops(double* ms, double* flops, int* tag, int cap) {
    int n = 0;
    for (auto& r : recs_) {
        FH_HIP(hipEventSynchronize(r.b));
        float t = 0.f;
        FH_HIP(hipEventElapsedTime(&t, r.a, r.b));
        if (n < cap) { ms[n] = t; flops[n] = r.flops; tag[n] = r.tag; ++n; }
        pool_.push_back(r.a); pool_.push_back(r.b);
    }
    recs_.clear();
    return n;
}

static bool debug_sync() {
    static int v = -1;
    if (v < 0) { const char* e = getenv("FACEHIP_DEBUG_SYNC"); v = e ? atoi(e) : 0; }
    return v != 0;
}


static constexpr int kWinoMinCin = 128;
static constexpr long kWinoMinTiles = 256;
static long wino2_min_blocks() {
    static long v = -1;
    if (v < 0) {
        const char* e = getenv("FACEHIP_WINO2");
        const char* m = getenv("FACEHIP_WINO2_MIN");
        v = e && atoi(e) == 0 ? (1L << 60) : m ? atol(m) : 64;
    }
    return v;
}

Net::Net(const std::string& onnx_path, int default_h, int default_w) {
    OnnxModel m = load_onnx(onnx_path);
    int H = default_h, W = default_w;
    const auto& shp = m.inputs[0].shape;
    if (shp.size() == 4) {
        if (shp[2] > 0) H = (int)shp[2];
        if (shp[3] > 0) W = (int)shp[3];
    }
    plan_ = build_plan(m, H, W);

    std::vector<float> host;
    auto push = [&](const float* src, size_t n) {
        size_t off = (host.size() + 63) / 64 * 64;
        host.resize(off + n, 0.f);
        if (n) memcpy(host.data() + off, src, n * sizeof(float));
        return off;
    };
    dev_.resize(plan_.ops.size());
    for (size_t i = 0; i < plan_.ops.size(); ++i) {
        POp& c = plan_.ops[i];
        if (c.bn_src < 0 || c.kind != OpKind::CONV || c.ks != 3 || c.stride != 1 || c.pad != 1 || c.H < 2 || c.W < 2) continue;
        const bool wino_ok = c.Cin >= kWinoMinCin && c.Cin % 32 == 0 && c.Cout % 4 == 0 && c.outs.empty() && c.res_mode != ResMode::UP2X;
        const POp& pr = plan_.ops[c.bn_src];
        if (wino_ok || !c.outs.empty() || (int)pr.s2.size() < c.Cin || pr.out < 0) continue;
        std::vector<float> b9((size_t)9 * c.Cout);
        for (int co = 0; co < c.Cout; ++co) {
            double tap_shift[9];
            for (int t = 0; t < 9; ++t) {
                double acc = 0;
                for (int ci = 0; ci < c.Cin; ++ci) acc += (double)c.weight[((size_t)co * 9 + t) * c.Cin + ci] * pr.t2[ci];
                tap_shift[t] = acc;
            }
            for (int ry = 0; ry < 3; ++ry)
                for (int rx = 0; rx < 3; ++rx) {
                    double b = c.bias[co];
                    for (int ky = 0; ky < 3; ++ky)
                        for (int kx = 0; kx < 3; ++kx) {
                            const bool in_y = !(ry == 0 && ky == 0) && !(ry == 2 && ky == 2);
                            const bool in_x = !(rx == 0 && kx == 0) && !(rx == 2 && kx == 2);
                            if (in_y && in_x) b += tap_shift[ky * 3 + kx];
                        }
                    b9[(size_t)(ry * 3 + rx) * c.Cout + co] = (float)b;
                }
            for (int t = 0; t < 9; ++t)
                for (int ci = 0; ci < c.Cin; ++ci) c.weight[((size_t)co * 9 + t) * c.Cin + ci] *= pr.s2[ci];
        }
        c.bias = b9;
        dev_[i].bn_fold_src = c.bn_src;
        dev_[c.bn_src].bn_fold_dst = true;
    }
    for (size_t i = 0; i < plan_.ops.size(); ++i) {
        const POp& op = plan_.ops[i];
        DevOp& d = dev_[i];
        if (op.kind == OpKind::DWPW) {
            d.dww = push(op.dw_weight.data(), op.dw_weight.size());
            d.dwb = push(op.dw_bias.data(), op.dw_bias.size());
        }
        if (op.kind == OpKind::CONV || op.kind == OpKind::GEMM || op.kind == OpKind::DWPW) {
            const int Ktot = op.ks * op.ks * op.Cin;
            d.Kpad = conv_kpad(Ktot);
            const int rows = conv_wt_rows(op.Cout);
            std::vector<float> packed((size_t)rows * d.Kpad, 0.f);
            conv_pack_weights(op.weight.data(), op.Cout, op.Cin, op.ks, packed.data());
            d.wt = push(packed.data(), packed.size());
            if (op.kind == OpKind::CONV) {
                ConvArgs probe{};
                probe.ks = op.ks; probe.stride = op.stride; probe.pad = op.pad; probe.Cin = op.Cin; probe.Cout = op.Cout; probe.act = (int)op.act;
                probe.res_mode = (int)op.res_mode; probe.H = op.H; probe.W = op.W;
                float dummy = 0.f;
                probe.out2 = op.out2 >= 0 ? &dummy : nullptr;
                probe.bias_cls = dev_[i].bn_fold_src >= 0 ? 1 : 0;
                if (conv_halo_ok(probe) && op.Ho * op.Wo >= 400) {
                    std::vector<float> wf(conv_halo_wfrag_floats(op.Cin, op.Cout));
                    conv_halo_pack_weights(op.weight.data(), op.Cout, op.Cin, wf.data());
                    d.wfrag = push(wf.data(), wf.size());
                    d.halo = true;
                }
            }
            if (op.kind == OpKind::CONV && op.Cin < kWinoMinCin) {
                ConvArgs probe{};
                probe.ks = op.ks; probe.stride = op.stride; probe.pad = op.pad; probe.Cin = op.Cin; probe.Cout = op.Cout; probe.act = (int)op.act;
                probe.res_mode = (int)op.res_mode; probe.H = op.H; probe.W = op.W; probe.Ho = op.Ho; probe.Wo = op.Wo;
                probe.n_outs = (int)op.outs.size(); probe.bias_cls = dev_[i].bn_fold_src >= 0 ? 1 : 0;
                float dummy2 = 0.f;
                probe.out2 = op.out2 >= 0 ? &dummy2 : nullptr;
                if (wino2_ok(probe)) {
                    std::vector<float> u(wino2_weight_floats(op.Cin, op.Cout));
                    wino2_pack_weights(op.weight.data(), op.Cout, op.Cin, u.data());
                    d.w2 = push(u.data(), u.size());
                    d.w2ok = true;
                }
            }
            if (op.kind == OpKind::CONV && op.ks == 3 && op.stride == 1 && op.pad == 1 && op.Cin >= kWinoMinCin && op.Cin % 32 == 0 &&
                op.Cout % 4 == 0 && op.outs.empty() && op.res_mode != ResMode::UP2X) {
                std::vector<float> u36((size_t)36 * rows * op.Cin, 0.f), uf((size_t)op.Cout * op.Cin);
                std::vector<double> uall((size_t)op.Cout * op.Cin * 36);
                for (int co = 0; co < op.Cout; ++co)
                    for (int ci = 0; ci < op.Cin; ++ci) {
                        double g[9];
                        for (int t = 0; t < 9; ++t) g[t] = op.weight[((size_t)co * 9 + t) * op.Cin + ci];
                        wino_filter_transform(g, &uall[((size_t)co * op.Cin + ci) * 36]);
                    }
                for (int f = 0; f < 36; ++f) {
                    for (size_t e = 0; e < uf.size(); ++e) uf[e] = (float)uall[e * 36 + f];
                    conv_pack_weights(uf.data(), op.Cout, op.Cin, 1, u36.data() + (size_t)f * rows * op.Cin);
                }
                d.w36 = push(u36.data(), u36.size());
                d.w36n = u36.size();
                d.w36k = op.Cin;
                d.wino = true;
                d.bf2 = wino_gemm_ok_bf16x2(op.Cin, op.Cout);
                const size_t tiles = (size_t)((op.H + 3) / 4) * ((op.W + 3) / 4);
                wino_elems_ = std::max(wino_elems_, 36 * tiles * (size_t)std::max(op.Cin, op.Cout));
                wino_maxc_ = std::max(wino_maxc_, (size_t)std::max(op.Cin, op.Cout));
            }
        } else if (op.kind == OpKind::DWCONV || op.kind == OpKind::DWGLOBAL || op.kind == OpKind::GCONV) {
            d.wt = push(op.weight.data(), op.weight.size());
        }
        if (!op.bias.empty()) d.bias = push(op.bias.data(), op.bias.size());
        if (!op.slope.empty()) { d.slope = push(op.slope.data(), op.slope.size()); d.has_slope = true; }
        if (!op.s2.empty()) { d.s2 = push(op.s2.data(), op.s2.size()); d.t2 = push(op.t2.data(), op.t2.size()); d.has_aff = true; }
    }
    for (size_t i = 0; i < plan_.ops.size(); ++i) {
        const POp& c = plan_.ops[i];
        if (c.sc_src < 0 || dev_[i].bn_fold_src >= 0 || c.bias.size() != (size_t)c.Cout) continue;
        if (dev_[i].wino || dev_[i].halo) continue;
        const POp& x = plan_.ops[c.sc_src];
        const int K9 = 9 * c.Cin, K = K9 + x.Cin, rows = conv_wt_rows(c.Cout);
        std::vector<float> w((size_t)rows * K, 0.f), b((size_t)c.Cout);
        for (int co = 0; co < c.Cout; ++co) {
            std::copy_n(&c.weight[(size_t)co * K9], K9, &w[(size_t)co * K]);
            std::copy_n(&x.weight[(size_t)co * x.Cin], x.Cin, &w[(size_t)co * K + K9]);
            b[co] = c.bias[co] + (x.bias.empty() ? 0.f : x.bias[co]);
        }
        dev_[i].wt_sc = push(w.data(), w.size());
        dev_[i].bias_sc = push(b.data(), b.size());
        dev_[i].Kpad_sc = K;
        dev_[i].sc_src = c.sc_src;
        dev_[c.sc_src].sc_dst = true;
    }
    for (size_t i = 0; i < plan_.ops.size(); ++i) {
        const int prod = plan_.ops[i].bn_src;
        if (!dev_[i].wino || prod <= 0 || !dev_[prod].has_aff) continue;
        dev_[i].aff_src = prod; dev_[prod].aff_dst = (int)i;
    }
    for (size_t i = 0; i + 1 < plan_.ops.size(); ++i) {
        const POp& a = plan_.ops[i];
        const POp& b = plan_.ops[i + 1];
        if (!dev_[i].wino || !dev_[i + 1].wino || a.H != b.H || a.W != b.W || a.Cout != b.Cin || !wino_can_fuse(a.H, a.W, a.Cout, false)) continue;
        int feed = -1;
        if (dev_[i + 1].aff_src == (int)i) feed = 1;
        else if (a.out >= 0 && b.in == a.out) feed = 0;
        else if (a.out2 >= 0 && b.in == a.out2) feed = 1;
        if (feed < 0) continue;
        int other_uses = 0;
        if (a.out >= 0) {
            for (const POp& o : plan_.ops)
                for (int x : {o.in, o.in2, o.res}) if (x == a.out) ++other_uses;
            for (const auto& o : plan_.outputs) if (o.tensor == a.out) ++other_uses;
            if (b.in == a.out) --other_uses;
        }
        const bool writes_out2 = a.out2 >= 0 && dev_[i + 1].aff_src != (int)i;
        if (!wino_can_fuse(a.H, a.W, a.Cout, other_uses > 0 || a.res >= 0 || writes_out2)) continue;
        dev_[i].fuse_next = true; dev_[i].fuse_feed_aff = feed == 1; dev_[i].fuse_keep_out1 = other_uses > 0;
    }
    {
        const POp& op = plan_.ops[0];
        stem_ok_ = op.kind == OpKind::CONV && op.in == plan_.input && op.ks == 3 && op.Cin == 4 && op.res < 0 && op.outs.empty() &&
                   op.Cout % 4 == 0 && op.Cout <= 64 && (op.stride == 1 || op.stride == 2);
        if (stem_ok_) {
            std::vector<float> w27((size_t)27 * op.Cout);
            for (int co = 0; co < op.Cout; ++co)
                for (int t = 0; t < 9; ++t)
                    for (int ci = 0; ci < 3; ++ci) w27[(size_t)(t * 3 + ci) * op.Cout + co] = op.weight[((size_t)co * 9 + t) * 4 + ci];
            dev_[0].w27 = push(w27.data(), w27.size());
            std::vector<float> wf((size_t)27 * op.Cout), bf((size_t)op.Cout);
            for (int co = 0; co < op.Cout; ++co) {
                double sum = 0;
                for (int t = 0; t < 9; ++t)
                    for (int j = 0; j < 3; ++j) {
                        const float w = op.weight[((size_t)co * 9 + t) * 4 + (2 - j)];
                        wf[(size_t)(t * 3 + j) * op.Cout + co] = w / 128.0f;
                        sum += w;
                    }
                bf[co] = (float)((double)op.bias[co] - 127.5 / 128.0 * sum);
            }
            dev_[0].wf = push(wf.data(), wf.size());
            dev_[0].bf = push(bf.data(), bf.size());
            if (op.Cout % 16 == 0) {
                std::vector<unsigned> fr((size_t)(op.Cout / 16) * 3 * 64 * 4, 0u);
                stem_pack_wfrag(wf.data(), op.Cout, fr.data());
                std::vector<float> asf(fr.size());
                memcpy(asf.data(), fr.data(), fr.size() * 4);
                dev_[0].wfr = push(asf.data(), asf.size());
            }
        }
    }
    if (stem_ok_ && plan_.ops.size() > 1) {
        const POp& st = plan_.ops[0];
        const POp& nx = plan_.ops[1];
        int uses = 0;
        for (const auto& o : plan_.ops) for (int x : {o.in, o.in2, o.res}) if (x == st.out) ++uses;
        for (const auto& o : plan_.outputs) if (o.tensor == st.out) ++uses;
        front_ok_ = st.Cout == 16 && st.out >= 0 && st.out2 < 0 && (st.act == Act::NONE || st.act == Act::RELU) && nx.kind == OpKind::DWPW &&
                    nx.in == st.out && uses == 1 && front_fused_ok(nx.Cin, nx.Cout, nx.dw_stride);
    }
    params_.ensure(std::max<size_t>(host.size(), 64) * sizeof(float));
    FH_HIP(hipMemcpy(params_.p, host.data(), host.size() * sizeof(float), hipMemcpyHostToDevice));
    for (auto& op : plan_.ops) { std::vector<float>().swap(op.weight); }
}

Net::SkRecord::~SkRecord() {
    if (!p) return;
    int cur = -1;
    (void)hipGetDevice(&cur);
    if (device >= 0 && device != cur) (void)hipSetDevice(device);
    (void)hipDeviceSynchronize();
    if (device >= 0 && device != cur && cur >= 0) (void)hipSetDevice(cur);
    conv_error_record_release(p);
}

void Net::reserve(int max_batch) {
    if (max_batch <= cap_) return;
    cap_ = max_batch;
    arena_.ensure(plan_.arena_elems * (size_t)cap_ * sizeof(float));
    if (partial_.bytes < conv_slab_floats() * sizeof(float)) {
        partial_.ensure(conv_slab_floats() * sizeof(float));
        conv_workspace_init(partial_.as<float>());
        if (!sk_rec_.p) { sk_rec_.p = conv_error_record_new(); (void)hipGetDevice(&sk_rec_.device); }
        if (!sk_rec_.p) throw std::runtime_error("HIP error: cannot allocate the stream-K watchdog record");
        sk_gen_ = conv_error_generation();
    }
    if (wino_elems_) {
        const size_t pad = 36 * 256 * wino_maxc_;
        wino_v_.ensure((wino_elems_ * (size_t)cap_ + pad) * sizeof(float));
        wino_m_.ensure((wino_elems_ * (size_t)cap_ + pad) * sizeof(float));
    }
    FH_HIP(hipMemset(arena_.p, 0, arena_.bytes));
}

void Net::run_u8(const uint8_t* src, long img_stride, int srcH, int srcW, int step, int batch, hipStream_t s) {
    if (batch <= 0) return;
    if (batch > cap_) throw std::runtime_error("Net::run_u8: batch exceeds reserved capacity");
    if (stem_ok_ && fuse_stem && front_ok_ && fuse_front && srcW >= 2) {
        const POp& st = plan_.ops[0];
        const POp& op = plan_.ops[1];
        const DevOp& d0 = dev_[0];
        const DevOp& d = dev_[1];
        const float* P = params_.as<float>();
        ConvArgs a{};
        a.wt = P + d.wt; a.bias = P + d.bias;
        a.out1 = tensor_ptr(op.out);
        a.dw_w = P + d.dww; a.dw_b = P + d.dwb; a.dw_act = (int)op.dw_act; a.dw_stride = op.dw_stride;
        a.B = batch; a.H = op.H; a.W = op.W; a.Cin = op.Cin; a.Ho = op.Ho; a.Wo = op.Wo; a.Cout = op.Cout;
        a.ks = 1; a.stride = 1; a.pad = 0; a.Kpad = d.Kpad; a.act = (int)op.act;
        a.u8_src = src; a.u8_img_stride = img_stride; a.u8_step = step; a.u8_srcH = srcH; a.u8_srcW = srcW; a.u8_inH = plan_.inH; a.u8_inW = plan_.inW;
        a.slabs = partial_.as<float>();
        a.u8_stride = st.stride; a.stem_act = (int)st.act; a.stem_wf = P + d0.wf; a.stem_bf = P + d0.bf;
        a.stem_wfrag = reinterpret_cast<const unsigned*>(P + d0.wfr);
        a.cus = cus;
        a.t_flops = 2.0 * (st.macs + op.macs) * batch;
        a.t_bytes = ((double)srcH * srcW * 3 + (double)op.Ho * op.Wo * op.Cout * 4) * batch;
        launch_dwpw(a, s);
        run(batch, s, 2);
        return;
    }
    if (stem_ok_ && fuse_stem) {
        const POp& op = plan_.ops[0];
        const DevOp& d = dev_[0];
        const float* P = params_.as<float>();
        KernelTimer& timer = KernelTimer::get();
        timer.begin(s);
        StemArgs a{};
        a.src = src; a.img_stride = img_stride; a.srcH = srcH; a.srcW = srcW; a.step = step; a.B = batch; a.inH = plan_.inH; a.inW = plan_.inW;
        a.stride = op.stride; a.Cout = op.Cout; a.w27 = P + d.w27; a.bias = P + d.bias; a.wf = P + d.wf; a.biasf = P + d.bf;
        a.wfrag = d.wfr ? reinterpret_cast<const unsigned*>(P + d.wfr) : nullptr;
        a.slope = d.has_slope ? P + d.slope : nullptr; a.act = (int)op.act; a.cus = cus;
        a.out1 = op.out >= 0 ? tensor_ptr(op.out) : nullptr; a.out2 = op.out2 >= 0 && !d.bn_fold_dst ? tensor_ptr(op.out2) : nullptr;
        if (d.has_aff) { a.s2 = P + d.s2; a.t2 = P + d.t2; }
        launch_stem(a, s);
        timer.end(s, 5, 2.0 * op.macs * batch, op.bytes * batch);
        run(batch, s, 1);
        return;
    }
    launch_det_preprocess(src, img_stride, srcH, srcW, step, batch, plan_.inH, plan_.inW, srcH, srcW, input(), s);
    run(batch, s, 0);
}

int Net::set_bf16x2(bool on, hipStream_t s) {
    int layers = 0;
    size_t total = 0;
    for (auto& d : dev_) if (d.wino && d.bf2) { d.w36p = total; total += d.w36n; ++layers; }
    if (on && layers > 0 && w36_bf_.bytes < total * sizeof(float)) {
        w36_bf_.ensure(total * sizeof(float));
        for (const auto& d : dev_)
            if (d.wino && d.bf2) launch_pack_bf16x2(params_.as<float>() + d.w36, w36_bf_.as<float>() + d.w36p, (long)d.w36n, s);
        FH_HIP(hipStreamSynchronize(s));
    }
    bf16x2_ = on && layers > 0;
    return on ? layers : 0;
}

int Net::set_wino_x3(bool on, hipStream_t s) {
    int layers = 0;
    size_t total = 0;
    for (auto& d : dev_)
        if (d.wino && d.bf2) { d.w36x = total; total += 36 * wino_x3_floats((int)(d.w36n / 36 / d.w36k), d.w36k); ++layers; }
    if (on && layers > 0 && w36_x3_.bytes < total * sizeof(float)) {
        w36_x3_.ensure(total * sizeof(float));
        for (const auto& d : dev_)
            if (d.wino && d.bf2) launch_pack_x3(params_.as<float>() + d.w36, w36_x3_.as<float>() + d.w36x, (int)(d.w36n / 36 / d.w36k), d.w36k, s);
        FH_HIP(hipStreamSynchronize(s));
    }
    wino_x3_ = on && layers > 0;
    size_t sc_total = 0;
    conv_x3_n_ = 0;
    for (size_t i = 0; i < dev_.size(); ++i) {
        DevOp& d = dev_[i];
        d.sc_x3 = d.sc_src >= 0 && plan_.ops[i].ks == 3 && conv_x3_ok(plan_.ops[i].Cin, plan_.ops[i].Cout) && d.Kpad_sc % 32 == 0;
        if (d.sc_x3) { d.wt_sc_x3 = sc_total; sc_total += wino_x3_floats(conv_wt_rows(plan_.ops[i].Cout), d.Kpad_sc); ++conv_x3_n_; }
    }
    if (on && conv_x3_n_ > 0 && wsc_x3_.bytes < sc_total * sizeof(float)) {
        wsc_x3_.ensure(sc_total * sizeof(float));
        for (size_t i = 0; i < dev_.size(); ++i)
            if (dev_[i].sc_x3)
                launch_pack_x3(params_.as<float>() + dev_[i].wt_sc, wsc_x3_.as<float>() + dev_[i].wt_sc_x3, conv_wt_rows(plan_.ops[i].Cout), dev_[i].Kpad_sc, s, 1);
        FH_HIP(hipStreamSynchronize(s));
    }
    conv_x3_ = on && conv_x3_n_ > 0;
    set_pw_x3(on, s);
    return on ? layers : 0;
}

int Net::set_pw_x3(bool on, hipStream_t s) {
    size_t total = 0;
    pw_x3_n_ = 0;
    for (size_t i = 0; i < dev_.size(); ++i) {
        const POp& op = plan_.ops[i];
        DevOp& d = dev_[i];
        d.pw_x3 = op.kind == OpKind::CONV && op.ks == 1 && op.stride == 1 && op.pad == 0 && op.Cin % 4 == 0 && op.Cout % 4 == 0 && op.outs.empty() &&
                  d.Kpad % 32 == 0 && d.Kpad >= op.Cin && d.sc_src < 0 && !d.sc_dst;
        if (d.pw_x3) { d.wt_pw_x3 = total; total += wino_x3_floats(conv_wt_rows(op.Cout), d.Kpad); ++pw_x3_n_; }
    }
    if (on && pw_x3_n_ > 0 && wpw_x3_.bytes < total * sizeof(float)) {
        wpw_x3_.ensure(total * sizeof(float));
        for (size_t i = 0; i < dev_.size(); ++i)
            if (dev_[i].pw_x3)
                launch_pack_x3(params_.as<float>() + dev_[i].wt, wpw_x3_.as<float>() + dev_[i].wt_pw_x3, conv_wt_rows(plan_.ops[i].Cout), dev_[i].Kpad, s, 1);
        FH_HIP(hipStreamSynchronize(s));
    }
    pw_x3_ = on && pw_x3_n_ > 0;
    return pw_x3_layers();
}

void Net::run(int batch, hipStream_t s, int first_op) {
    if (batch <= 0) return;
    if ((sk_gen_ != conv_error_generation() || conv_error_pending(sk_rec_.p)) && partial_.p) {
        conv_workspace_reset_async(partial_.as<float>(), s);
        sk_gen_ = conv_error_generation();
    }
    if (batch > cap_) throw std::runtime_error("Net::run: batch exceeds reserved capacity");
    const float* P = params_.as<float>();
    KernelTimer& timer = KernelTimer::get();
    bool v_ready = false;
    for (size_t i = (size_t)first_op; i < plan_.ops.size(); ++i) {
        const POp& op = plan_.ops[i];
        const DevOp& d = dev_[i];
        int tag = 5;
        const bool dense = op.kind == OpKind::CONV || op.kind == OpKind::GEMM || op.kind == OpKind::DWPW;
        if (!dense) timer.begin(s);
        switch (op.kind) {
            case OpKind::CONV:
            case OpKind::GEMM: {
                if (d.sc_dst && fold_shortcut && force_cfg < 0) break;
                ConvArgs a{};
                a.in = tensor_ptr(op.in);
                a.wt = P + d.wt;
                a.bias = P + d.bias;
                a.slope = d.has_slope ? P + d.slope : nullptr;
                a.res = op.res >= 0 ? tensor_ptr(op.res) : nullptr;
                a.out1 = op.out >= 0 ? tensor_ptr(op.out) : nullptr;
                a.out2 = op.out2 >= 0 ? tensor_ptr(op.out2) : nullptr;
                if (d.bn_fold_dst) a.out2 = nullptr;
                if (d.bn_fold_src >= 0) { a.in = tensor_ptr(plan_.ops[d.bn_fold_src].out); a.bias_cls = 1; }
                if (d.aff_dst >= 0 && winograd) {
                    const POp& c = plan_.ops[d.aff_dst];
                    if ((long)batch * ((c.H + 3) / 4) * ((c.W + 3) / 4) >= kWinoMinTiles) a.out2 = nullptr;
                }
                a.s2 = d.has_aff ? P + d.s2 : nullptr;
                a.t2 = d.has_aff ? P + d.t2 : nullptr;
                a.slabs = partial_.as<float>();
                a.sk_err = sk_rec_.p;
                a.sk_enable = sk_enable ? 1 : 0;
                a.cus = cus;
                a.no_pw = force_cfg >= 0 ? 1 : 0;
                a.B = batch; a.H = op.H; a.W = op.W; a.Cin = op.Cin; a.Ho = op.Ho; a.Wo = op.Wo; a.Cout = op.Cout;
                a.ks = op.ks; a.stride = op.stride; a.pad = op.pad; a.Kpad = d.Kpad;
                a.act = (int)op.act; a.res_mode = (int)op.res_mode;
                a.n_outs = (int)op.outs.size();
                for (int g = 0; g < a.n_outs && g < 3; ++g) { a.outs[g] = tensor_ptr(op.outs[g]); a.oact[g] = op.out_act[g]; a.oc0[g] = op.out_c0[g]; }
                if (a.n_outs > 0) a.oc0[a.n_outs] = op.out_c0[a.n_outs];
                const long M = (long)batch * op.Ho * op.Wo;
                int cfg = force_cfg >= 0 ? force_cfg : conv_pick_cfg(M, op.Cout);
                if (force_cfg < 0 && cfg == 0 && ((M + 127) / 128) * ((op.Cout + 127) / 128) < 128) cfg = 3;
                a.t_flops = 2.0 * op.macs * batch; a.t_bytes = op.bytes * batch;
                if (d.sc_src >= 0 && fold_shortcut && force_cfg < 0) {
                    const POp& x = plan_.ops[d.sc_src];
                    a.wt = P + d.wt_sc; a.bias = P + d.bias_sc; a.Kpad = d.Kpad_sc;
                    a.res = nullptr; a.res_mode = (int)ResMode::NONE;
                    a.sc_in = tensor_ptr(x.in); a.sc_H = x.H; a.sc_W = x.W; a.sc_C = x.Cin; a.sc_stride = x.stride;
                    a.t_flops += 2.0 * x.macs * batch;
                }
                if (d.halo && halo_conv && force_cfg < 0) {
                    launch_conv_halo(a, P + d.wfrag, s);
                    tag = 9;
                    break;
                }
                if (d.w2ok && winograd && force_cfg < 0 && d.sc_src < 0 && wino2_blocks(a) >= wino2_min_blocks()) {
                    a.wt = P + d.w2;
                    launch_wino2(a, s);
                    break;
                }
                const bool use_wino = d.wino && winograd && (long)batch * ((op.H + 3) / 4) * ((op.W + 3) / 4) >= kWinoMinTiles;
                if (use_wino) {
                    const int wcfg = force_cfg >= 0 ? force_cfg : 2;
                    const bool bf2 = bf16x2_ && d.bf2 && force_cfg < 0;
                    WinoPlanes pl;
                    const bool mix = wcfg == 2 && wino_mix_layout(batch, op.H, op.W, op.Cin, op.Cout, &pl);
                    const long row_tiles = mix ? pl.total_tiles : 36 * wino_rows((long)batch * ((op.H + 3) / 4) * ((op.W + 3) / 4)) / 128;
                    const bool x3 = !bf2 && wino_x3_ && d.bf2 && force_cfg < 0 && wcfg == 2 && wino_x3_pays(row_tiles, op.Cin, op.Cout);
                    const float* const u36 = bf2 ? w36_bf_.as<float>() + d.w36p : x3 ? w36_x3_.as<float>() + d.w36x : P + d.w36;
                    if (!v_ready) {
                        const float* in_s = nullptr; const float* in_t = nullptr;
                        if (d.aff_src >= 0) {
                            a.in = tensor_ptr(plan_.ops[d.aff_src].out);
                            in_s = P + dev_[d.aff_src].s2; in_t = P + dev_[d.aff_src].t2;
                        }
                        if (mix) launch_wino_mix(a, pl, nullptr, wino_v_.as<float>(), 0, in_s, in_t, bf2, s);
                        else launch_wino_input(a, wino_v_.as<float>(), in_s, in_t, bf2, s);
                    }
                    launch_wino_gemm(a, u36, wino_v_.as<float>(), wino_m_.as<float>(), wcfg, bf2 ? 1 : x3 ? 2 : 0, s, mix ? &pl : nullptr);
                    v_ready = false;
                    if (d.fuse_next && fuse_wino && i + 1 < plan_.ops.size()) {
                        const POp& nx = plan_.ops[i + 1];
                        const bool next_wino = dev_[i + 1].wino && (long)batch * ((nx.H + 3) / 4) * ((nx.W + 3) / 4) >= kWinoMinTiles;
                        const bool next_mix = next_wino && wcfg == 2 && wino_mix_layout(batch, nx.H, nx.W, nx.Cin, nx.Cout, nullptr);
                        if (next_wino && mix == next_mix) {
                            ConvArgs e = a;
                            if (!d.fuse_keep_out1) e.out1 = nullptr;
                            const bool pack_next = bf16x2_ && dev_[i + 1].bf2 && force_cfg < 0;
                            if (mix) launch_wino_mix(e, pl, wino_m_.as<float>(), wino_v_.as<float>(), d.fuse_feed_aff ? 1 : 0, nullptr, nullptr, pack_next, s);
                            else launch_wino_fused(e, wino_m_.as<float>(), wino_v_.as<float>(), d.fuse_feed_aff ? 1 : 0, pack_next, s);
                            v_ready = true;
                        }
                    }
                    if (!v_ready) {
                        if (mix) launch_wino_mix(a, pl, wino_m_.as<float>(), nullptr, 0, nullptr, nullptr, false, s);
                        else launch_wino_output(a, wino_m_.as<float>(), s);
                    }
                    tag = 7;
                    break;
                }
                if (conv_x3_ && d.sc_x3 && a.sc_in && conv_x3_pays(((M + 127) / 128) * (op.Cout / conv_x3_bn(op.Cout)), a.Kpad, op.Cout,
                                                                     cus > 0 ? cus : conv_num_cus(), conv_knobs())) {
                    a.wt = wsc_x3_.as<float>() + d.wt_sc_x3;
                    launch_conv_x3(a, cfg, s);
                } else if (pw_x3_ && d.pw_x3 && force_cfg < 0 && launch_conv_pw_x3(a, wpw_x3_.as<float>() + d.wt_pw_x3, false, s)) {
                } else {
                    launch_conv(a, cfg, s);
                }
                tag = cfg;
                break;
            }
            case OpKind::DWPW: {
                ConvArgs a{};
                a.in = tensor_ptr(op.in);
                a.wt = P + d.wt; a.bias = P + d.bias;
                a.out1 = tensor_ptr(op.out);
                a.dw_w = P + d.dww; a.dw_b = P + d.dwb; a.dw_act = (int)op.dw_act; a.dw_stride = op.dw_stride;
                a.B = batch; a.H = op.H; a.W = op.W; a.Cin = op.Cin; a.Ho = op.Ho; a.Wo = op.Wo; a.Cout = op.Cout;
                a.ks = 1; a.stride = 1; a.pad = 0; a.Kpad = d.Kpad; a.act = (int)op.act;
                a.t_flops = 2.0 * op.macs * batch; a.t_bytes = op.bytes * batch;
                a.slabs = partial_.as<float>();
                a.cus = cus;
                launch_dwpw(a, s);
                break;
            }
            case OpKind::DWCONV:
                launch_dwconv3x3(tensor_ptr(op.in), P + d.wt, P + d.bias, tensor_ptr(op.out), batch, op.H, op.W, op.Cin, op.stride,
                                 (int)op.act, d.has_slope ? P + d.slope : nullptr, s);
                tag = 4;
                break;
            case OpKind::DWGLOBAL:
                launch_dwglobal(tensor_ptr(op.in), P + d.wt, P + d.bias, tensor_ptr(op.out), batch, op.ks * op.ks, op.Cin, (int)op.act,
                                d.has_slope ? P + d.slope : nullptr, s);
                break;
            case OpKind::GCONV:
                launch_gconv3x3(tensor_ptr(op.in), P + d.wt, P + d.bias, tensor_ptr(op.out), batch, op.H, op.W, op.Cin,
                                (int)(op.weight_group), op.stride, (int)op.act, d.has_slope ? P + d.slope : nullptr, s);
                tag = 4;
                break;
            case OpKind::AFFINE:
                launch_affine(tensor_ptr(op.in), P + d.s2, P + d.t2, tensor_ptr(op.out), (long)batch * op.H * op.W, op.Cin, s);
                break;
            case OpKind::ACT:
                launch_act(tensor_ptr(op.in), d.has_slope ? P + d.slope : nullptr, tensor_ptr(op.out), (long)batch * op.H * op.W,
                           op.Cin, (int)op.act, s);
                break;
            case OpKind::ADD:
                launch_add(tensor_ptr(op.in), tensor_ptr(op.in2), tensor_ptr(op.out), (long)batch * op.H * op.W * op.Cin, s);
                break;
            case OpKind::UPSAMPLE:
                launch_upsample2x(tensor_ptr(op.in), tensor_ptr(op.out), batch, op.H, op.W, op.Cin, s);
                break;
        }
        if (!dense) timer.end(s, tag, 2.0 * op.macs * batch, op.bytes * batch);
        if (debug_sync()) {
            fprintf(stderr, "[facehip] op %zu %s batch %d done-launch\n", i, op.name.c_str(), batch); fflush(stderr);
            const hipError_t e1 = hipGetLastError(), e2 = hipStreamSynchronize(s);
            if (e1 != hipSuccess || e2 != hipSuccess)
                throw std::runtime_error("HIP error after op " + std::to_string(i) + " (" + op.name + "): " + hipGetErrorString(e1 != hipSuccess ? e1 : e2));
        }
    }
    FH_HIP(hipGetLastError());
}

Detector::Detector(const std::string& onnx_path) : net_(onnx_path, 640, 640) {
    const auto& outs = net_.plan().outputs;
    const int H = net_.in_h(), W = net_.in_w();
    if (outs.size() == 9) {
        static const int cols[9] = {1, 1, 1, 4, 4, 4, 10, 10, 10};
        static const int strides[3] = {8, 16, 32};
        bool ok = true;
        for (int i = 0; i < 9; ++i) {
            const int s = strides[i % 3];
            ok = ok && outs[i].cols == cols[i] && outs[i].rows == (H / s) * (W / s) * 2;
        }
        if (ok) anchors_ = ((H / 8) * (W / 8) + (H / 16) * (W / 16) + (H / 32) * (W / 32)) * 2;
    } else if (outs.size() >= 1 && outs[0].cols >= 15) {
        predecoded_ = true;
        anchors_ = outs[0].rows;
        feat_ = outs[0].cols;
    }
    cap_ = 1;
    while (cap_ < std::max(anchors_, 1)) cap_ <<= 1;
    if (det_x3_default()) net_.set_pw_x3(true, nullptr);
}

bool det_x3_default() {
    static const int v = [] { const char* e = getenv("FACEHIP_DET_X3"); return e ? atoi(e) : 1; }();
    return v != 0;
}

void Detector::reserve(int n, int rows, int cols) {
    (void)rows; (void)cols;
    net_.reserve(n);
    if (n > nb_) {
        nb_ = n;
        cand_.ensure((size_t)n * cap_ * sizeof(FaceRec));
        keys_.ensure((size_t)n * cap_ * sizeof(unsigned long long));
        ws_.ensure((size_t)n * cap_ * sizeof(int));
        count_.ensure((size_t)n * sizeof(int));
    }
}

int letterbox_plan(int rows, int cols, int in_w, int in_h, int* new_w, int* new_h, float* scale) {
    int nw = 0, nh = 0;
    float sc = 0.f;
    if (rows > 0 && cols > 0 && in_w > 0 && in_h > 0) {
        const float scaleW = (float)in_w / (float)cols, scaleH = (float)in_h / (float)rows;
        sc = std::min(scaleW, scaleH);
// ... 303 lines not shown
```

### facerecognizeonnx_amd/csrc/engine.h

```cpp
#pragma once
#include <hip/hip_runtime.h>

#include <cstdint>
#include <stdexcept>
#include <string>
#include <utility>
#include <vector>

#include "kernels.h"
#include "plan.h"
#include "tile_plan.h"

namespace fh {


struct DevBuf {
    void* p = nullptr;
    size_t bytes = 0;
    DevBuf() = default;
    DevBuf(const DevBuf&) = delete;
    DevBuf& operator=(const DevBuf&) = delete;
    ~DevBuf();
    void ensure(size_t n);
    void swap(DevBuf& o) { std::swap(p, o.p); std::swap(bytes, o.bytes); }
    void grow(size_t n, size_t keep) {
        if (n <= bytes) return;
        if (keep == 0) return ensure(n);
        DevBuf bigger;
        bigger.ensure(n);
        FH_HIP(hipMemcpy(bigger.p, p, keep, hipMemcpyDeviceToDevice));
        swap(bigger);
    }
    template <class T> T* as() const { return reinterpret_cast<T*>(p); }
};

unsigned long long layout_epoch();

class Net {
  public:
    Net(const std::string& onnx_path, int default_h, int default_w);
    void reserve(int max_batch);
    float* input() const { return arena_.as<float>() + plan_.tensors[plan_.input].offset * (size_t)cap_; }
    float* output(int i) const { return tensor_ptr(plan_.outputs[i].tensor); }
    void run(int batch, hipStream_t s, int first_op = 0);
    void run_u8(const uint8_t* src, long img_stride, int srcH, int srcW, int step, int batch, hipStream_t s);
    bool fuse_stem = true;
    bool fuse_front = true;
    const Plan& plan() const { return plan_; }
    int in_h() const { return plan_.inH; }
    int in_w() const { return plan_.inW; }
    int capacity() const { return cap_; }
    bool winograd = true;
    bool halo_conv = true;
    bool fold_shortcut = true;
    bool fuse_wino = true;
    int set_bf16x2(bool on, hipStream_t s);
    bool bf16x2() const { return bf16x2_; }
    int set_wino_x3(bool on, hipStream_t s);
    bool wino_x3() const { return wino_x3_; }
    int conv_x3_layers() const { return conv_x3_ ? conv_x3_n_ : 0; }
    int set_pw_x3(bool on, hipStream_t s);
    int pw_x3_layers() const { return pw_x3_ ? pw_x3_n_ : 0; }
    int cus = 0;
    int force_cfg = -1;
    bool sk_enable = true;
    long long config_word() const {
        return (long long)fuse_stem | (long long)fuse_front << 1 | (long long)winograd << 2 | (long long)halo_conv << 3 |
               (long long)fold_shortcut << 4 | (long long)fuse_wino << 5 | (long long)bf16x2_ << 6 | (long long)sk_enable << 7 |
               (long long)(cus & 0xffff) << 8 | (long long)((force_cfg + 1) & 0xff) << 24 | (long long)wino_x3_ << 32 | (long long)conv_x3_ << 33 |
               (long long)pw_x3_ << 34;
    }

  private:
    struct DevOp {
        size_t wt = 0, bias = 0, slope = 0, s2 = 0, t2 = 0;
        bool has_slope = false, has_aff = false;
        size_t w27 = 0;
        size_t wfr = 0;
        size_t wf = 0, bf = 0;
        size_t dww = 0, dwb = 0;
        size_t w36 = 0;
        size_t w36n = 0, w36p = 0;
        size_t w36x = 0;
        int w36k = 0;
        bool bf2 = false;
        size_t wfrag = 0;
        bool halo = false;
        bool wino = false;
        size_t w2 = 0;
        bool w2ok = false;
        int aff_src = -1;
        int aff_dst = -1;
        int bn_fold_src = -1;
        bool bn_fold_dst = false;
        int sc_src = -1;
        size_t wt_sc = 0, bias_sc = 0;
        int Kpad_sc = 0;
        size_t wt_sc_x3 = 0;
        bool sc_x3 = false;
        size_t wt_pw_x3 = 0;
        bool pw_x3 = false;
        bool sc_dst = false;
        bool fuse_next = false;
        bool fuse_feed_aff = false;
        bool fuse_keep_out1 = true;
        int Kpad = 0;
    };
  public:
    float* workspace() const { return partial_.as<float>(); }
    unsigned* error_record() const { return sk_rec_.p; }
  private:
    float* tensor_ptr(int t) const { return arena_.as<float>() + plan_.tensors[t].offset * (size_t)cap_; }
    Plan plan_;
    std::vector<DevOp> dev_;
    DevBuf params_, arena_, partial_, wino_v_, wino_m_, w36_bf_, w36_x3_, wsc_x3_, wpw_x3_;
    bool bf16x2_ = false, wino_x3_ = false, conv_x3_ = false, pw_x3_ = false;
    int conv_x3_n_ = 0, pw_x3_n_ = 0;
    size_t wino_maxc_ = 0;
    size_t wino_elems_ = 0;
    int cap_ = 0;
    struct SkRecord {
        unsigned* p = nullptr;
        int device = -1;
        SkRecord() = default;
        SkRecord(const SkRecord&) = delete;
        SkRecord& operator=(const SkRecord&) = delete;
        ~SkRecord();
    } sk_rec_;
    unsigned sk_gen_ = 0;
    bool stem_ok_ = false;
    bool front_ok_ = false;
};

int letterbox_plan(int rows, int cols, int in_w, int in_h, int* new_w, int* new_h, float* scale);

struct FrameIn {
    const uint8_t* bgr;
    int32_t rows, cols, step;
};
inline bool frame_empty(const FrameIn& f) { return !f.bgr || f.rows <= 0 || f.cols <= 0; }

class StagedTable {
  public:
    StagedTable() = default;
    StagedTable(const StagedTable&) = delete;
    StagedTable& operator=(const StagedTable&) = delete;
    ~StagedTable();
    void* stage(size_t bytes);
    void* send(size_t bytes, hipStream_t s);
    void* dev() const { return dev_.p; }

  private:
    static constexpr int kSlots = 4;
    struct Slot { void* p = nullptr; size_t bytes = 0; hipEvent_t ev = nullptr; bool pending = false; } slot_[kSlots];
    int next_ = 0, cur_ = 0;
    DevBuf dev_;
};

class FrameTable {
  public:
    const FrameDesc* upload(const FrameIn* frames, int n, int in_w, int in_h, hipStream_t s);
    const FrameDesc* table() const { return static_cast<const FrameDesc*>(st_.dev()); }
    const float* scales() const { return reinterpret_cast<const float*>(table() + n_); }
    int size() const { return n_; }

  private:
    int n_ = 0;
    StagedTable st_;
};

struct TilePlan {
    std::vector<FrameIn> view_frames;
    std::vector<ViewDesc> views;
    std::vector<FrameSeg> segs;
    size_t key_total = 0;
    int plan(const FrameIn* frames, int n, const Tiling& t, int in_w, int in_h, int cap, int max_views);
};
constexpr int kTileMaxViews = 256;

class TileTable {
  public:
    void upload(const TilePlan& p, hipStream_t s);
    const ViewDesc* views() const { return static_cast<const ViewDesc*>(st_.dev()); }
    const FrameSeg* segs() const { return reinterpret_cast<const FrameSeg*>(views() + V_); }

  private:
    int V_ = 0;
    StagedTable st_;
};

void postprocess_views(PostArgs a, int n_frames, const TileTable* tab, float nms_thr, int* sup, FaceRec* out, int max_out, int* counts,
                       hipStream_t s);

bool det_x3_default();

class Detector {
  public:
    explicit Detector(const std::string& onnx_path);
    void detect_dev(const uint8_t* frames, int n, int rows, int cols, int step, long stride, float score_thr, float nms_thr,
                    FaceRec* out, int max_out, int* counts, hipStream_t s);
    Net& net() { return net_; }
    int num_anchors() const { return anchors_; }
    bool predecoded() const { return predecoded_; }
    float last_scale() const { return scale_; }
    void run_network_dev(const uint8_t* frames, int n, int rows, int cols, int step, long stride, hipStream_t s);
    void postprocess_dev(int n, float score_thr, float nms_thr, FaceRec* out, int max_out, int* counts, hipStream_t s);
    void run_input_dev(const float* input, int n, hipStream_t s);
    void letterbox_ragged_dev(const FrameIn* frames, int n, uint8_t* canvas, hipStream_t s);
    void run_network_ragged_dev(const FrameIn* frames, int n, hipStream_t s);
    void detect_ragged_dev(const FrameIn* frames, int n, float score_thr, float nms_thr, FaceRec* out, int max_out, int* counts,
                           hipStream_t s);
    const FrameTable& frame_table() const { return table_; }
    int run_network_tiled_dev(const FrameIn* frames, int n, const Tiling& t, hipStream_t s);
    void detect_tiled_dev(const FrameIn* frames, int n, const Tiling& t, float score_thr, float nms_thr, FaceRec* out, int max_out,
                          int* counts, hipStream_t s);
    const FrameTable& tiled_frame_table() const { return frames_table_; }

  private:
    void reserve(int n, int rows, int cols);
    PostArgs post_source(int V, float score_thr);
    Net net_;
    bool predecoded_ = false;
    int anchors_ = 0, feat_ = 15, cap_ = 0, nb_ = 0;
    float scale_ = 1.f;
    bool ragged_ = false;
    FrameTable table_, frames_table_;
    TilePlan tplan_;
    TileTable ttab_;
    DevBuf resized_, cand_, keys_, count_, ws_;
};

class Recognizer {
  public:
    explicit Recognizer(const std::string& onnx_path);
    int dim() const { return dim_; }
    Net& net() { return net_; }
    void embed_aligned_dev(const uint8_t* crops, int n, float* out, hipStream_t s, float* raw_out = nullptr);
    void embed_faces_dev(const uint8_t* frames, int rows, int cols, int step, long stride, const FaceRec* faces,
                         const int* frame_of, int n, float* out, int* ok, hipStream_t s);
    void align_dev(const uint8_t* frames, int rows, int cols, int step, long stride, const FaceRec* faces, const int* frame_of,
                   int n, uint8_t* crops, int* ok, hipStream_t s);
    void resize_embed_dev(const uint8_t* frames, int n, int rows, int cols, int step, long stride, float* out, hipStream_t s);
    void align_table_dev(const FrameDesc* table, int n_frames, const FaceRec* faces, const int* frame_of, int n, uint8_t* crops, int* ok,
                         hipStream_t s);
    void embed_faces_table_dev(const FrameDesc* table, int n_frames, const FaceRec* faces, const int* frame_of, int n, float* out, int* ok,
                               hipStream_t s);
    void align_ragged_dev(const FrameIn* frames, int n_frames, const FaceRec* faces, const int* frame_of, int n, uint8_t* crops, int* ok,
                          hipStream_t s);
    void embed_faces_ragged_dev(const FrameIn* frames, int n_frames, const FaceRec* faces, const int* frame_of, int n, float* out, int* ok,
                                hipStream_t s);
    void embed_input_dev(const float* input, int n, float* out, hipStream_t s, float* raw_out = nullptr);
    int max_chunk = 256;

  private:
    Net net_;
    int dim_ = 0;
    FrameTable table_;
    DevBuf crops_, ok_, raw_;
};

class Gallery;
class Tracker {
  public:
    Tracker(int streams, int max_tracks, float iou_thr, int max_missed, int refresh);
    int streams() const { return streams_; }
    int max_tracks() const { return p_.max_tracks; }
    void reset(int stream);
    int get_state(int stream, TrackState* out, int* frame_no, int* next_id);
    void update_dev(const FaceRec* det, const int* counts, int n, int per_frame, const int* stream_of, int* track, int* embed, int* slot,
                    const int* quality, hipStream_t s);
// ... 118 lines not shown
```

### facerecognizeonnx_amd/csrc/kernels.h

```cpp
#pragma once
#include <hip/hip_runtime.h>

#include <cstdint>
#include <string>

#include <vector>

#include "conv_plan.h"

namespace fh {

void hip_check(hipError_t e, const char* what);
#define FH_HIP(x) ::fh::hip_check((x), #x)

#if defined(__HIPCC__)
__device__ __forceinline__ void wave_lds_order() {
#if defined(__HIP_DEVICE_COMPILE__)
    __builtin_amdgcn_fence(__ATOMIC_ACQ_REL, "wavefront");
    __builtin_amdgcn_wave_barrier();
#endif
}
#endif

struct KernelTimer {
    static constexpr int kTags = 13;
    bool enabled = false;
    void begin(hipStream_t s);
    void end(hipStream_t s, int tag, double flops, double bytes);
    void collect(double* ms, double* flops, double* bytes, long long* launches);
    int collect_ops(double* ms, double* flops, int* tag, int cap);
    static KernelTimer& get();

  private:
    struct Rec { hipEvent_t a, b; int tag; double flops, bytes; };
    std::vector<Rec> recs_;
    std::vector<hipEvent_t> pool_;
    hipEvent_t cur_ = nullptr;
    hipEvent_t take();
};


struct ConvArgs {
    const float* in;
    const float* wt;
    const float* bias;
    const float* slope;
    const float* res;
    float* out1;
    float* out2;
    const float* s2;
    const float* t2;
    float* slabs;
    const float* zeros;
    int B, H, W, Cin, Ho, Wo, Cout;
    int ks, stride, pad;
    int Kpad;
    int bias_cls;
    const float* sc_in;
    int sc_H, sc_W, sc_C, sc_stride;
    int act;
    int res_mode;
    const float* dw_w;
    const float* dw_b;
    int dw_act;
    int dw_stride;
    const uint8_t* u8_src;
    long u8_img_stride;
    int u8_step, u8_srcH, u8_srcW, u8_inH, u8_inW, u8_stride, stem_act;
    const float* stem_wf;
    const float* stem_bf;
    const unsigned* stem_wfrag;
    int no_prio;
    int no_pw;
    int n_outs;
    float* outs[3];
    int oc0[4];
    int oact[3];
    int sk_enable;
    int cus;
    int wt_group_rows;
    long wt_gs;
    double t_flops, t_bytes;
    int sk_full, sk_units, sk_q, sk_helpers, sk_rem, sk_owner_chunks, sk_maxp;
    unsigned* sk_err;
    int ep_direct;
    unsigned sk_timeout;
    int sk_test_drop;
    int tile0;
};

void launch_conv(const ConvArgs& a, int cfg, hipStream_t s);
void launch_conv_x3(const ConvArgs& a, int tag, hipStream_t s);
bool conv_x3_ok(int Cin, int Cout);
bool launch_conv_pw_x3(ConvArgs a, const float* wt3, bool force, hipStream_t s);
void conv_workspace_init(float* ws);
void conv_workspace_reset_async(float* ws, hipStream_t s);
unsigned* conv_error_words();
unsigned* conv_error_record_new();
void conv_error_record_release(unsigned* r);
bool conv_take_error(std::string& msg, unsigned* rec);
bool conv_error_pending(const unsigned* rec);
unsigned conv_error_generation();
void conv_debug_streamk(int drop_publish, int timeout_ms);
unsigned conv_debug_generation();
size_t wino2_weight_floats(int Cin, int Cout);
void wino2_pack_weights(const float* w_ohwi, int Cout, int Cin, float* dst);
bool wino2_ok(const ConvArgs& a);
void launch_wino2(const ConvArgs& a, hipStream_t s);
long wino2_blocks(const ConvArgs& a);
double wino2_debug_clock_mhz();
const float* conv_zero_line();
int conv_num_cus();
bool conv_halo_ok(const ConvArgs& a);
size_t conv_halo_wfrag_floats(int Cin, int Cout);
void conv_halo_pack_weights(const float* w_ohwi, int Cout, int Cin, float* dst);
void launch_conv_halo(const ConvArgs& a, const float* wfrag, hipStream_t s);
bool front_fused_ok(int Cin, int Cout, int dw_stride);
void launch_dwpw(const ConvArgs& a, hipStream_t s);
void launch_conv_winograd(const ConvArgs& a, const float* wt36, float* V, float* M, int cfg, const float* in_scale, const float* in_shift,
                          hipStream_t s, int prec = 0);
struct WinoPlanes;
void launch_wino_input(const ConvArgs& a, float* V, const float* in_scale, const float* in_shift, bool pack, hipStream_t s);
void launch_wino_gemm(const ConvArgs& a, const float* wt36, const float* V, float* M, int cfg, int prec, hipStream_t s,
                      const WinoPlanes* mix = nullptr);
bool wino_gemm_ok_bf16x2(int Cin, int Cout);
void launch_pack_x3(const float* in, float* out, int rows, int K, hipStream_t s, int freqs = 36);
inline size_t wino_x3_floats(int rows, int K) { return (size_t)rows * K * 3 / 2; }
bool wino_x3_default();
bool wino_x3_pays(long row_tiles, int Cin, int Cout);
void launch_wino_output(const ConvArgs& a, const float* M, hipStream_t s);
bool wino_can_fuse(int H, int W, int C, bool touches_memory);
void launch_wino_fused(const ConvArgs& a, const float* M, float* Vnext, int feed_aff, bool pack_next, hipStream_t s);
void launch_pack_bf16x2(const float* in, float* out, long n, hipStream_t s);
struct WinoPlanes {
    int e[4];
    int t[4];
    int nfc[4];
    int f2[4];
    int n[4];
    int rows[4];
    int base[4];
    int total_tiles;
    int planes;
};
bool wino_mix_layout(int B, int H, int W, int Cin, int Cout, WinoPlanes* out);
void launch_wino_mix(const ConvArgs& a, const WinoPlanes& pl, const float* M, float* Vnext, int feed_aff, const float* in_scale,
                     const float* in_shift, bool pack_next, hipStream_t s);
void wino_filter_transform(const double g[9], double u[36]);
void wino_debug_slots(int slots);
long wino_rows(long tiles);
int conv_wt_rows(int Cout);
size_t conv_slab_floats();
void conv_pack_weights(const float* w, int Cout, int Cin, int ks, float* dst);
inline int conv_kpad(int Ktot) { return (Ktot + 31) / 32 * 32; }

void launch_dwconv3x3(const float* in, const float* w9c, const float* bias, float* out, int B, int H, int W,
                      int C, int stride, int act, const float* slope, hipStream_t s);
void launch_dwglobal(const float* in, const float* w, const float* bias, float* out, int B, int taps, int C, int act, const float* slope,
                     hipStream_t s);
void launch_gconv3x3(const float* in, const float* w, const float* bias, float* out, int B, int H, int W, int C, int G, int stride, int act,
                     const float* slope, hipStream_t s);
void launch_affine(const float* in, const float* sc, const float* sh, float* out, long pixels, int C, hipStream_t s);
void launch_act(const float* in, const float* slope, float* out, long pixels, int C, int act, hipStream_t s);
void launch_add(const float* a, const float* b, float* out, long n, hipStream_t s);
void launch_upsample2x(const float* in, float* out, int B, int H, int W, int C, hipStream_t s);

struct FaceRec {
    int32_t x, y, w, h;
    float score;
    float lm[10];
};

void launch_det_preprocess(const uint8_t* frames, long img_stride, int rows, int cols, int step, int B,
                           int inH, int inW, int newH, int newW, float* out, hipStream_t s);
void launch_rec_preprocess(const uint8_t* crops, int n, int H, int W, float* out, hipStream_t s);

struct StemArgs {
    const uint8_t* src;
    long img_stride;
    int srcH, srcW, step, B;
    int inH, inW, stride, Cout;
    const float *w27, *bias;
    const float *wf, *biasf;
    const unsigned* wfrag;
    const float* slope;
    int act;
    float *out1, *out2;
    const float *s2, *t2;
    int cus;
};
void launch_stem(const StemArgs& a, hipStream_t s);
void stem_pack_wfrag(const float* wf, int Cout, unsigned* out);

struct ViewDesc {
    int32_t frame, local, x, y, w, h, edges;
    float scale;
};
static_assert(sizeof(ViewDesc) == 32, "ViewDesc is a 32-byte table row");
struct FrameSeg {
    int32_t first_view, views, key_off, seg_cap;
};
struct PostArgs {
    const float* score[3];
    const float* bbox[3];
    const float* kps[3];
    int inH, inW;
    const float* rows;
    int n_rows, feat;
    const ViewDesc* views;
    const FrameSeg* segs;
    const float* scales;
    float scale;
    int V, cap, border;
    float thr;
    FaceRec* cand;
    unsigned long long* keys;
    int* count;
};
void launch_scrfd_decode(const PostArgs& a, hipStream_t s);
void launch_rows_threshold(const PostArgs& a, hipStream_t s);
void launch_sort_nms(const FaceRec* cand, unsigned long long* keys, const int* count, const FrameSeg* segs, int cap, int n_frames,
                     float nms_thr, FaceRec* out, int* out_count, int max_out, int* order_ws, hipStream_t s);

void launch_align(const uint8_t* frames, long img_stride, int rows, int cols, int step, const FaceRec* faces,
                  const int* frame_of, int n, int outH, int outW, uint8_t* crops, int* ok, hipStream_t s);
struct FrameDesc {
    const uint8_t* bgr;
    int32_t rows, cols, step, new_h, new_w, pad_;
};
static_assert(sizeof(FrameDesc) == 32, "FrameDesc is a 32-byte table row");
void launch_letterbox_ragged(const FrameDesc* table, int n, int inH, int inW, uint8_t* canvas, hipStream_t s);
void launch_align_ragged(const FrameDesc* table, int n_frames, const FaceRec* faces, const int* frame_of, int n, int outH, int outW,
                         uint8_t* crops, int* ok, hipStream_t s);
void launch_resize_u8c3(const uint8_t* src, long src_stride, int sh, int sw, int sstep, uint8_t* dst, long dst_stride,
                        int dh, int dw, int dstep, int n, hipStream_t s);

void launch_l2_normalize(const float* in, float* out, int n, int dim, hipStream_t s);

int gallery_parts(long G, int Q, int* tiles_per_part);
void launch_label(const float* best_score, const int* best_idx, int n, float thr, int* labels, hipStream_t s);
void launch_topk_merge(const float* part_score, const int* part_idx, int nparts, int Q, int k, float* out_score,
                       int* out_idx, hipStream_t s, const int* qcount = nullptr);
void launch_topk_merge_strided(const float* part_score, const int* part_idx, int nparts, int Q, int k, long part_stride, float* out_score,
                               int* out_idx, hipStream_t s, const int* qcount = nullptr);

void launch_topk_merge_ids(const float* part_score, const int* part_id, const int* part_idx, int nparts, int Q, int k, float* out_score,
                           int* out_id, int* out_idx, hipStream_t s, const int* qcount = nullptr);
void launch_ids_of_rows(const float* score, const int* idx, int n, const int* ids, long idx_base, float thr, bool use_thr, int* out_id,
                        hipStream_t s);
void launch_gather_rows(const void* src, void* dst, const int* map, long m, size_t row_bytes, hipStream_t s);
void launch_gather_ids(const int* src, int* dst, const int* map, long m, hipStream_t s);

constexpr int GAL_TAG_TILE = 128;
void gallery_debug_tag_skip(int on);
void launch_tag_tile_or(const unsigned* tags, long G, long first, long n, unsigned* tile_or, hipStream_t s);
void launch_fuse_tags(const unsigned* src_tags, const int* order, const long long* starts, long m, unsigned* dst_tags, hipStream_t s);

struct FuseItem { int begin, count, out, final; };
void launch_gallery_fuse_sum(const float* src, const int* order, const FuseItem* items, long n_items, int dim, float* dst, float* part,
                             bool unit, hipStream_t s);
void launch_gallery_self_scores(const float* src, const int* src_ids, long n, const float* tmpl, const int* tmpl_ids, long m, int dim,
                                float* out, hipStream_t s);
// ... 112 lines not shown
```

### facerecognizeonnx_amd/csrc/plan.cpp

```cpp
#include "plan.h"

#include <algorithm>
#include <cmath>
#include <cstdio>
#include <map>
#include <set>
#include <sstream>
#include <stdexcept>

namespace fh {
namespace {

struct GNode {
    std::string op;
    std::vector<std::string> in;
    std::string out;
    const OnnxNode* src = nullptr;
    bool dead = false;
    int order = 0;
    std::vector<double> w;
    std::vector<double> b;
    int Cout = 0, CinG = 0, ks = 1, stride = 1, pad = 0, group = 1;
    Act act = Act::NONE;
    std::vector<float> slope;
// ... 80 lines not shown
    }
    outputs = m.outputs;
    for (auto& o : outputs) o.name = A(o.name);
    return true;
}

static Plan build_plan_impl(const OnnxModel& m, int inH, int inW);

Plan build_plan(const OnnxModel& m0, int inH, int inW) {
    std::vector<OnnxNode> nodes;
    std::vector<OnnxValueInfo> outputs;
    std::map<std::string, OnnxTensor> consts;
    if (!strip_passthrough(m0, nodes, outputs, consts)) return build_plan_impl(m0, inH, inW);
    OnnxModel m;
    m.nodes = std::move(nodes);
    m.outputs = std::move(outputs);
    m.inputs = m0.inputs;
    m.inits = m0.inits;
    for (auto& kv : consts) m.inits[kv.first] = std::move(kv.second);
    Plan P = build_plan_impl(m, inH, inW);
    for (size_t i = 0; i < P.outputs.size() && i < m0.outputs.size(); ++i) P.outputs[i].name = m0.outputs[i].name;
    return P;
}

static Plan build_plan_impl(const OnnxModel& m, int inH, int inW) {
    if (m.inputs.size() != 1) fail("expected exactly one graph input");
    struct Dim { int c = 0, h = 0, w = 0; };
    std::map<std::string, Dim> dims;
    std::map<std::string, std::vector<double>> cvals;
    std::set<std::string> shape_nodes;
    auto get_const = [&](const std::string& name, std::vector<double>& out) -> bool {
        auto it = cvals.find(name);
        if (it != cvals.end()) { out = it->second; return true; }
        auto ii = m.inits.find(name);
        if (ii == m.inits.end() || ii->second.numel() > 64) return false;
        out.clear();
        if (!ii->second.i.empty()) out.assign(ii->second.i.begin(), ii->second.i.end());
        else out.assign(ii->second.f.begin(), ii->second.f.end());
        return true;
    };
    dims[m.inputs[0].name] = Dim{3, inH, inW};
    for (const auto& n : m.nodes) {
        if (n.outputs.empty()) continue;
        const std::string& out = n.outputs[0];
        auto in_dim = [&](size_t k) -> const Dim* {
            if (k >= n.inputs.size()) return nullptr;
            auto it = dims.find(n.inputs[k]);
            return it == dims.end() ? nullptr : &it->second;
        };
        std::vector<double> a, b;
        if (n.op == "Conv") {
            const Dim* d = in_dim(0);
            auto wi = m.inits.find(n.inputs.size() > 1 ? n.inputs[1] : "");
            if (d && wi != m.inits.end() && wi->second.dims.size() == 4) {
                const int k = (int)wi->second.dims[2];
                auto st = n.attr_ints("strides"); auto pd = n.attr_ints("pads");
                const int s_ = st.empty() ? 1 : (int)st[0], p_ = pd.empty() ? 0 : (int)pd[0];
                dims[out] = Dim{(int)wi->second.dims[0], (d->h + 2 * p_ - k) / s_ + 1, (d->w + 2 * p_ - k) / s_ + 1};
            }
        } else if (n.op == "Resize" || n.op == "Upsample") {
            const Dim* d = in_dim(0);
            if (d) {
                Dim o = *d;
                bool ok = false;
                if (n.op == "Upsample") { if (get_const(n.inputs.at(1), a) && a.size() == 4) { o.h = (int)std::floor(d->h * a[2]); o.w = (int)std::floor(d->w * a[3]); ok = true; } }
                else {
                    if (n.inputs.size() > 3 && !n.inputs[3].empty() && get_const(n.inputs[3], a) && a.size() == 4) { o.h = (int)a[2]; o.w = (int)a[3]; ok = true; }
                    else if (n.inputs.size() > 2 && !n.inputs[2].empty() && get_const(n.inputs[2], a) && a.size() == 4) { o.h = (int)std::floor(d->h * a[2]); o.w = (int)std::floor(d->w * a[3]); ok = true; }
                    else if (n.inputs.size() == 2 && get_const(n.inputs[1], a) && a.size() == 4) { o.h = (int)std::floor(d->h * a[2]); o.w = (int)std::floor(d->w * a[3]); ok = true; }
                }
                if (ok) dims[out] = o;
            }
        } else if (n.op == "Shape") {
            const Dim* d = in_dim(0);
            if (d) { cvals[out] = {1.0, (double)d->c, (double)d->h, (double)d->w}; shape_nodes.insert(out); }
        } else if (n.op == "Constant") {
            auto it = n.attrs.find("value");
            if (it != n.attrs.end() && it->second.t.numel() <= 64) {
                std::vector<double> v;
                if (!it->second.t.i.empty()) v.assign(it->second.t.i.begin(), it->second.t.i.end());
                else v.assign(it->second.t.f.begin(), it->second.t.f.end());
                cvals[out] = v; shape_nodes.insert(out);
            }
        } else if (n.op == "Gather") {
            if (get_const(n.inputs.at(0), a) && get_const(n.inputs.at(1), b) && n.attr_i("axis", 0) == 0) {
                std::vector<double> v;
                for (double ix : b) { long q = (long)ix; if (q < 0) q += (long)a.size(); if (q < 0 || q >= (long)a.size()) fail("Gather index out of range"); v.push_back(a[(size_t)q]); }
                cvals[out] = v; shape_nodes.insert(out);
            }
        } else if (n.op == "Slice") {
            if (get_const(n.inputs.at(0), a)) {
                std::vector<double> st, en, ax, sp;
                bool ok = true;
                if (n.inputs.size() >= 3) {
                    ok = get_const(n.inputs[1], st) && get_const(n.inputs[2], en);
                    if (n.inputs.size() > 3 && !n.inputs[3].empty()) ok = ok && get_const(n.inputs[3], ax);
                    if (n.inputs.size() > 4 && !n.inputs[4].empty()) ok = ok && get_const(n.inputs[4], sp);
                } else {
                    for (auto v : n.attr_ints("starts")) st.push_back((double)v);
                    for (auto v : n.attr_ints("ends")) en.push_back((double)v);
                    for (auto v : n.attr_ints("axes")) ax.push_back((double)v);
                }
                if (ok && st.size() == 1 && en.size() == 1 && (ax.empty() || ax[0] == 0) && (sp.empty() || sp[0] == 1)) {
                    long L = (long)a.size(), s0 = (long)st[0], e0 = (long)std::min<double>(en[0], 1e9);
                    if (s0 < 0) s0 += L;
                    if (e0 < 0) e0 += L;
                    s0 = std::max(0L, std::min(L, s0)); e0 = std::max(0L, std::min(L, e0));
                    cvals[out] = std::vector<double>(a.begin() + s0, a.begin() + std::max(s0, e0)); shape_nodes.insert(out);
                }
            }
        } else if (n.op == "Concat") {
            std::vector<double> v;
            bool ok = !n.inputs.empty();
            for (auto& in : n.inputs) { if (!get_const(in, a) || dims.count(in)) { ok = false; break; } v.insert(v.end(), a.begin(), a.end()); }
            if (ok) { cvals[out] = v; shape_nodes.insert(out); }
        } else if (n.op == "Unsqueeze" || n.op == "Squeeze" || n.op == "Cast" || n.op == "Identity" || n.op == "Floor" || n.op == "Ceil") {
            if (!dims.count(n.inputs.at(0)) && get_const(n.inputs[0], a)) {
                if (n.op == "Floor" || (n.op == "Cast" && n.attr_i("to", 1) != 1 && n.attr_i("to", 1) != 11)) for (auto& v : a) v = std::floor(v);
                if (n.op == "Ceil") for (auto& v : a) v = std::ceil(v);
                cvals[out] = a; shape_nodes.insert(out);
            } else if (n.op == "Identity" && in_dim(0)) dims[out] = *in_dim(0);
        } else if ((n.op == "Mul" || n.op == "Div" || n.op == "Add" || n.op == "Sub") && n.inputs.size() == 2 &&
                   !dims.count(n.inputs[0]) && !dims.count(n.inputs[1]) && get_const(n.inputs[0], a) && get_const(n.inputs[1], b)) {
            const size_t L = std::max(a.size(), b.size());
            if ((a.size() == L || a.size() == 1) && (b.size() == L || b.size() == 1)) {
                std::vector<double> v(L);
                for (size_t k = 0; k < L; ++k) {
                    const double x = a[a.size() == 1 ? 0 : k], y = b[b.size() == 1 ? 0 : k];
                    v[k] = n.op == "Mul" ? x * y : n.op == "Div" ? x / y : n.op == "Add" ? x + y : x - y;
                }
                cvals[out] = v; shape_nodes.insert(out);
            }
        } else if (n.op == "Transpose" || n.op == "Reshape" || n.op == "Flatten" || n.op == "Gemm") {
        } else if (in_dim(0)) {
            dims[out] = *in_dim(0);
        }
    }
    std::vector<GNode> g;
    g.reserve(m.nodes.size());
    int ord = 0;
    for (const auto& n : m.nodes) {
        GNode x;
        x.op = n.op; x.src = &n; x.order = ord++;
        if (n.outputs.empty()) fail("node without output");
        x.out = n.outputs[0];
        if (shape_nodes.count(x.out)) { --ord; continue; }
        if (n.op == "Conv") {
            const auto& w = init_of(m, n.inputs.at(1));
            if (w.dims.size() != 4 || w.dims[2] != w.dims[3]) fail("Conv weight must be [Cout,Cin/g,k,k]");
            x.Cout = (int)w.dims[0]; x.CinG = (int)w.dims[1]; x.ks = (int)w.dims[2];
            x.group = (int)n.attr_i("group", 1);
            auto st = n.attr_ints("strides"); auto pd = n.attr_ints("pads"); auto dl = n.attr_ints("dilations");
            x.stride = st.empty() ? 1 : (int)st[0];
            if (!st.empty() && st[0] != st[1]) fail("anisotropic stride");
            x.pad = pd.empty() ? 0 : (int)pd[0];
            for (auto p : pd) if (p != x.pad) fail("asymmetric padding");
            for (auto d : dl) if (d != 1) fail("dilation != 1");
            if (n.attr_s("auto_pad", "NOTSET") != "NOTSET") fail("auto_pad not supported");
            if (!((x.ks == 3 && x.pad == 1) || (x.ks == 1 && x.pad == 0) || (x.group > 1 && x.pad == 0)))
                fail("only 3x3/p1 and 1x1/p0 convolutions are supported");
            x.w.assign(w.f.begin(), w.f.end());
            if (n.inputs.size() > 2 && !n.inputs[2].empty()) { const auto& b = init_of(m, n.inputs[2]).f; x.b.assign(b.begin(), b.end()); }
            else x.b.assign((size_t)x.Cout, 0.0);
            x.in = {n.inputs[0]};
        } else if (n.op == "MatMul") {
            const auto& w = init_of(m, n.inputs.at(1));
            if (w.dims.size() != 2) fail("MatMul: the second operand must be a 2-D initializer");
            const int K = (int)w.dims[0], N = (int)w.dims[1];
            x.op = "Gemm";
            x.Cout = N; x.CinG = K;
            x.w.resize((size_t)N * K);
            for (int k = 0; k < K; ++k)
                for (int j = 0; j < N; ++j) x.w[(size_t)j * K + k] = w.f[(size_t)k * N + j];
            x.b.assign((size_t)N, 0.0);
            x.in = {n.inputs[0]};
        } else if (n.op == "Gemm") {
            const auto& w = init_of(m, n.inputs.at(1));
            if (w.dims.size() != 2) fail("Gemm weight must be 2-D");
            if (n.attr_i("transB", 0) != 1 || n.attr_i("transA", 0) != 0 || n.attr_f("alpha", 1.f) != 1.f || n.attr_f("beta", 1.f) != 1.f)
                fail("Gemm: only alpha=beta=1, transB=1 supported");
            x.Cout = (int)w.dims[0]; x.CinG = (int)w.dims[1];
            x.w.assign(w.f.begin(), w.f.end());
            if (n.inputs.size() > 2 && !n.inputs[2].empty()) { const auto& b = init_of(m, n.inputs[2]).f; x.b.assign(b.begin(), b.end()); }
            else x.b.assign((size_t)x.Cout, 0.0);
            x.in = {n.inputs[0]};
        } else if (n.op == "BatchNormalization" || n.op == "Relu" || n.op == "Sigmoid" || n.op == "Flatten" ||
                   n.op == "Transpose" || n.op == "Reshape" || n.op == "PRelu" || n.op == "Resize" || n.op == "Upsample") {
            x.in = {n.inputs[0]};
        } else if ((n.op == "Mul" || n.op == "Add" || n.op == "Sub" || n.op == "Div") && n.inputs.size() == 2 &&
                   (m.inits.count(n.inputs[0]) != 0) != (m.inits.count(n.inputs[1]) != 0)) {
            x.op = "BatchNormalization";
            x.in = {m.inits.count(n.inputs[0]) ? n.inputs[1] : n.inputs[0]};
        } else if (n.op == "Add") {
            x.in = {n.inputs.at(0), n.inputs.at(1)};
        } else {
            fail("unsupported operator '" + n.op + "'");
        }
        g.push_back(std::move(x));
    }

    std::set<std::string> graph_outs;
    for (auto& o : m.outputs) graph_outs.insert(o.name);
    auto consumers = [&](const std::string& v) {
        int c = graph_outs.count(v) ? 1 : 0;
        for (auto& n : g) {
            if (n.dead) continue;
            for (auto& i : n.in) if (i == v) ++c;
            if (n.res == v) ++c;
        }
        return c;
    };
    auto producer = [&](const std::string& v) -> GNode* {
        for (auto& n : g) if (!n.dead && (n.out == v || (!n.out2.empty() && n.out2 == v))) return &n;
        return nullptr;
    };
    auto is_convlike = [](const GNode* n) { return n && (n->op == "Conv" || n->op == "Gemm"); };
    auto resize_is_up2 = [&](const GNode& r) {
        const OnnxNode& n = *r.src;
        if (n.attr_s("mode", "nearest") != "nearest") fail("Resize: only nearest supported");
        auto di = dims.find(n.inputs[0]);
        auto dn = dims.find(n.outputs[0]);
        if (di == dims.end() || dn == dims.end())
            fail("Resize: output size is not a load-time constant (unsupported shape sub-graph)");
        return dn->second.h == 2 * di->second.h && dn->second.w == 2 * di->second.w && dn->second.c == di->second.c;
    };

    for (auto& bn : g) {
        if (bn.dead || bn.op != "BatchNormalization") continue;
        GNode* p = producer(bn.in[0]);
        if (!is_convlike(p) || p->out != bn.in[0] || consumers(p->out) != 1) continue;
        if (p->act != Act::NONE || !p->res.empty() || !p->out2.empty()) continue;
        std::vector<double> s, t;
        bn_scale_shift(m, *bn.src, s, t, p->Cout);
        if ((int)s.size() != p->Cout) fail("BN channel mismatch after " + p->op);
        size_t per = p->w.size() / (size_t)p->Cout;
        for (int co = 0; co < p->Cout; ++co) {
            for (size_t k = 0; k < per; ++k) p->w[(size_t)co * per + k] *= s[co];
            p->b[co] = p->b[co] * s[co] + t[co];
        }
        p->out = bn.out;
        bn.dead = true;
    }
    for (auto& a : g) {
        if (a.dead || !(a.op == "Relu" || a.op == "PRelu" || a.op == "Sigmoid")) continue;
        GNode* p = producer(a.in[0]);
        if (!p || p->op != "Conv" || p->out != a.in[0] || consumers(p->out) != 1) continue;
        if (p->act != Act::NONE || !p->res.empty() || !p->out2.empty()) continue;
        if (a.op == "Relu") p->act = Act::RELU;
        else if (a.op == "Sigmoid") p->act = Act::SIGMOID;
        else {
            const auto& sl = init_of(m, a.src->inputs.at(1)).f;
            if (sl.size() == 1) p->slope.assign((size_t)p->Cout, sl[0]);
            else if ((int)sl.size() == p->Cout) p->slope = sl;
            else fail("PRelu slope size mismatch");
            p->act = Act::PRELU;
        }
        p->out = a.out;
        a.dead = true;
    }
    for (auto& add : g) {
        if (add.dead || add.op != "Add") continue;
        for (int side = 0; side < 2; ++side) {
            GNode* p = producer(add.in[side]);
            if (!p || p->op != "Conv" || p->group != 1 || p->out != add.in[side]) continue;
            if (consumers(p->out) != 1 || !p->res.empty() || !p->out2.empty()) continue;
            const std::string other = add.in[1 - side];
            if (other == p->out) continue;
            GNode* q = producer(other);
            if (q && (q->op == "Resize" || q->op == "Upsample") && consumers(q->out) == 1 && resize_is_up2(*q)) {
                p->res = q->in[0]; p->res_mode = ResMode::UP2X; q->dead = true;
            } else {
                p->res = other; p->res_mode = ResMode::SAME;
            }
            p->out = add.out;
            add.dead = true;
            break;
        }
    }
    for (auto& bn : g) {
        if (bn.dead || bn.op != "BatchNormalization") continue;
        GNode* p = producer(bn.in[0]);
        if (!p || p->op != "Conv" || p->group != 1 || p->out != bn.in[0] || !p->out2.empty()) continue;
        std::vector<double> s, t;
        bn_scale_shift(m, *bn.src, s, t, p->Cout);
        if ((int)s.size() != p->Cout) fail("BN channel mismatch (second output)");
        p->s2.assign(s.begin(), s.end());
        p->t2.assign(t.begin(), t.end());
        p->out2 = bn.out;
        bn.dead = true;
        if (consumers(p->out) == 0) p->write_out1 = false;
    }

    std::vector<GNode*> live;
    for (auto& n : g) if (!n.dead) live.push_back(&n);
    std::vector<GNode*> sorted;
    {
        std::set<std::string> ready;
        ready.insert(m.inputs[0].name);
        std::vector<bool> done(live.size(), false);
        for (size_t iter = 0; iter < live.size(); ++iter) {
            bool progressed = false;
            for (size_t i = 0; i < live.size(); ++i) {
                if (done[i]) continue;
                GNode* n = live[i];
                bool ok = true;
                for (auto& v : n->in) if (!ready.count(v)) ok = false;
                if (!n->res.empty() && !ready.count(n->res)) ok = false;
// ... 440 lines not shown
```

### include/facehip.h

```cpp
#ifndef FACEHIP_H_
#define FACEHIP_H_

#include <stddef.h>
#include <stdint.h>

#ifdef __cplusplus
extern "C" {
#endif

#define FH_API __attribute__((visibility("default")))

enum fh_status { FH_OK = 0, FH_ERR_ARG = -1, FH_ERR_MODEL = -2, FH_ERR_DEVICE = -3, FH_ERR_STATE = -4 };

typedef struct fh_face {
    int32_t x, y, w, h;
    float score;
    float lm[10];
} fh_face;

typedef struct fh_det fh_det;
typedef struct fh_rec fh_rec;
typedef struct fh_gallery fh_gallery;

FH_API const char* fh_version(void);
// ... 119 lines not shown
FH_API int fh_track_identify_dev(fh_tracker* t, fh_gallery* g, float threshold, const int* d_track, const int* d_slot, const int* d_embed,
                                 const float* d_emb, int total, int n, int per_frame, const int* stream_of ,
                                 int* d_label , float* d_score , void* stream);
FH_API const float* fh_tracker_queries_dev(fh_tracker* t);
FH_API int fh_tracker_get_identity(fh_tracker* t, int stream, fh_track_ident* host_out ,
                                   float* sums_out );
FH_API int fh_pipeline_run_identified_dev(fh_det* d, fh_rec* r, fh_tracker* t, fh_gallery* g, float threshold, const uint8_t* d_frames, int n,
                                          int rows, int cols, int step, long long frame_stride, const int* stream_of, float score_thr,
                                          float nms_thr, int faces_per_frame, fh_face* d_all, int* d_counts, int* d_track, fh_face* d_faces,
                                          int* d_frame_of, int* d_track_of, float* d_emb, int* d_label , float* d_score ,
                                          void* stream);

FH_API int fh_face_quality_dev(const uint8_t* d_frames, int n, int rows, int cols, int step, long long frame_stride, const fh_face* d_det,
                               const int* d_counts, int per_frame, int* d_quality , void* stream);
FH_API int fh_face_quality_ragged_dev(const fh_frame* frames, int n, const fh_face* d_det, const int* d_counts, int per_frame,
                                      int* d_quality , void* stream);
FH_API int fh_tracker_set_bestshot(fh_tracker* t, int on, int num, int den, int min_gap);
FH_API int fh_tracker_get_quality(fh_tracker* t, int stream, int* host_out );
FH_API const int* fh_tracker_quality_dev(fh_tracker* t);
FH_API int fh_track_update_q_dev(fh_tracker* t, const fh_face* d_det, const int* d_counts, int n, int per_frame, const int* stream_of,
                                 int* d_track, int* d_embed, int* d_slot , const int* d_quality ,
                                 void* stream);
FH_API int fh_track_identify_q_dev(fh_tracker* t, fh_gallery* g, float threshold, const int* d_track, const int* d_slot, const int* d_embed,
                                   const int* d_quality , const float* d_emb, int total, int n, int per_frame,
                                   const int* stream_of, int* d_label, float* d_score, void* stream);

#define FH_TRACK_LINK_MEMORY 256
typedef struct fh_track_link { int32_t owner, root, n_emb, label; float score; int32_t last_seen, links, pad; } fh_track_link;
FH_API int fh_tracker_enable_relink(fh_tracker* t, int memory, float link_thr, int max_age);
FH_API int fh_track_identify_link_dev(fh_tracker* t, fh_gallery* g, float threshold, const int* d_track, const int* d_slot, const int* d_embed,
                                      const int* d_quality , const float* d_emb, int total, int n, int per_frame,
                                      const int* stream_of, int* d_label, float* d_score, int* d_root , void* stream);
FH_API int fh_tracker_get_links(fh_tracker* t, int stream, fh_track_link* host_out ,
                                float* sums_out );
FH_API const int* fh_tracker_roots_dev(fh_tracker* t);

FH_API fh_gallery* fh_gallery_create(int dim);
FH_API void fh_gallery_destroy(fh_gallery* g);
FH_API int fh_gallery_upload(fh_gallery* g, const float* rows, long long n, int rows_on_device, long long index_base);
FH_API int fh_gallery_topk_dev(fh_gallery* g, const float* d_queries, int nq, int k, float* d_scores, int* d_indices,
                               void* stream);
enum fh_gallery_scan { FH_GAL_SCAN_FP32 = 0, FH_GAL_SCAN_F16_RERANK = 1 };
FH_API int fh_gallery_set_scan(fh_gallery* g, int mode);
FH_API int fh_gallery_get_scan(const fh_gallery* g);
FH_API int fh_gallery_scan_stats(fh_gallery* g, long long* certified, long long* fallback);
FH_API int fh_topk_merge_dev(const float* d_part_scores, const int* d_part_idx, int nparts, int nq, int k, float* d_scores,
                             int* d_indices, void* stream);
#define FH_COMM_ID_BYTES 128
typedef struct fh_comm fh_comm;
FH_API int fh_comm_unique_id(unsigned char id[FH_COMM_ID_BYTES]);
FH_API fh_comm* fh_comm_create(int rank, int world, const unsigned char id[FH_COMM_ID_BYTES], int device);
FH_API void fh_comm_destroy(fh_comm* c);
FH_API int fh_comm_rank(const fh_comm* c);
FH_API int fh_comm_world(const fh_comm* c);
FH_API int fh_comm_allgather_f32_dev(fh_comm* c, const float* d_send, float* d_recv, long long count, void* stream);
FH_API int fh_gallery_topk_sharded_dev(fh_gallery* g, fh_comm* c, const float* d_queries_local, int nq_local, int k,
                                       float* d_scores, int* d_indices, void* stream);
FH_API long long fh_gallery_enroll(fh_gallery* g, const float* rows, long long n, int rows_on_device);
FH_API long long fh_gallery_size(fh_gallery* g);
FH_API int fh_gallery_label_dev(fh_gallery* g, const float* d_queries, int nq, float threshold, int* d_labels,
                                float* d_scores, void* stream);

FH_API long long fh_gallery_enroll_ids(fh_gallery* g, const float* rows, const int* ids, long long n, int on_device);
FH_API int fh_gallery_upload_ids(fh_gallery* g, const float* rows, const int* ids, long long n, int on_device, long long index_base);
FH_API int fh_gallery_topk_ids_dev(fh_gallery* g, const float* d_queries, int nq, int k, float* d_scores, int* d_ids, int* d_rows,
                                   void* stream);
FH_API int fh_gallery_label_ids_dev(fh_gallery* g, const float* d_queries, int nq, float threshold, int* d_ids_out, float* d_scores,
                                    void* stream);
FH_API long long fh_gallery_remove_ids(fh_gallery* g, const int* ids_host, long long n_ids);
FH_API long long fh_gallery_get_ids(fh_gallery* g, long long first, long long n, int* ids_host_out);
FH_API int fh_topk_merge_ids_dev(const float* d_part_scores, const int* d_part_ids, const int* d_part_rows, int nparts, int nq, int k,
                                 float* d_scores, int* d_ids, int* d_rows, void* stream);

#define FH_FUSE_CHUNK 512
enum fh_gallery_fuse { FH_FUSE_UNIT = 0, FH_FUSE_SUM = 1 };
FH_API long long fh_gallery_group_ids(const int* ids, long long n, int* order, long long* starts, int* uniq);
FH_API long long fh_gallery_fuse_ids(fh_gallery* src, fh_gallery* dst, int mode);
FH_API long long fh_gallery_get_rows(fh_gallery* g, long long first, long long n, float* rows_host_out);
FH_API int fh_gallery_self_scores_dev(fh_gallery* src, fh_gallery* tmpl, float* d_scores, void* stream);

enum fh_cluster_noise { FH_CLUSTER_NOISE_NONE = 0, FH_CLUSTER_NOISE_SELF = 1 };
FH_API int fh_cluster_scores(const float* scores, int n, float threshold, int min_pts, int noise, int* labels, int* info);
FH_API int fh_gallery_cluster_dev(fh_gallery* g, float threshold, int min_pts, int noise, int* d_labels, int* d_info, void* stream);
FH_API long long fh_gallery_set_ids(fh_gallery* g, const int* ids, int on_device);

#define FH_HIST_BINS 2048
typedef struct fh_roc_point {
    float threshold;
    int32_t bin;
    unsigned long long true_accepts, false_accepts, genuine, impostor;
} fh_roc_point;
FH_API int fh_hist_bin(float score);
FH_API int fh_roc_from_hist(const unsigned long long* hist, double max_far, fh_roc_point out[2]);
FH_API int fh_gallery_pair_hist_dev(fh_gallery* g, unsigned long long* d_hist, unsigned long long* d_nan, void* stream);

#define FH_PAIRS_MAX_CAP 1024
#define FH_PAIRS_ROOM 65536
enum fh_pairs_class { FH_PAIRS_GENUINE = 0, FH_PAIRS_IMPOSTOR = 1, FH_PAIRS_ANY = 2 };
enum fh_pairs_side { FH_PAIRS_ABOVE = 0, FH_PAIRS_NOT_ABOVE = 1 };
FH_API int fh_pairs_from_scores(const float* scores, int n, const int* ids , int cls, int side, float threshold, int cap,
                                long long room, unsigned long long* info, float* out_scores ,
                                int* out_rows , int* out_ids );
FH_API int fh_gallery_pairs_dev(fh_gallery* g, int cls, int side, float threshold, int cap, unsigned long long* d_info,
                                float* d_scores , int* d_rows , int* d_ids ,
                                void* stream);

#define FH_TAG_ALL 0xFFFFFFFFu
FH_API long long fh_gallery_set_tags(fh_gallery* g, long long first, long long n, const uint32_t* tags, int on_device);
FH_API long long fh_gallery_get_tags(fh_gallery* g, long long first, long long n, uint32_t* tags_host_out);
FH_API int fh_gallery_topk_tagged_dev(fh_gallery* g, const float* d_queries, const uint32_t* d_masks, int nq, int k, float* d_scores,
                                      int* d_indices, void* stream);
FH_API int fh_gallery_topk_ids_tagged_dev(fh_gallery* g, const float* d_queries, const uint32_t* d_masks, int nq, int k, float* d_scores,
                                          int* d_ids, int* d_rows, void* stream);
FH_API int fh_gallery_label_tagged_dev(fh_gallery* g, const float* d_queries, const uint32_t* d_masks, int nq, float threshold,
                                       int* d_labels, float* d_scores, void* stream);
FH_API int fh_gallery_label_ids_tagged_dev(fh_gallery* g, const float* d_queries, const uint32_t* d_masks, int nq, float threshold,
                                           int* d_ids_out, float* d_scores, void* stream);
FH_API int fh_gallery_tag_stats(fh_gallery* g, long long* tiles_scanned, long long* tiles_skipped);
FH_API int fh_tracker_set_stream_masks(fh_tracker* t, const uint32_t* masks_host );

#define FH_RANGE_MAX_CAP 1024
FH_API int fh_gallery_range_dev(fh_gallery* g, const float* d_queries, const uint32_t* d_masks , int nq, float threshold,
                                int cap, long long* d_counts , float* d_scores ,
                                int* d_indices , int* d_ids , void* stream);
FH_API int fh_range_from_scores(const float* scores, long long n, long long index_base, const uint32_t* tags , uint32_t mask,
                                float threshold, int cap, long long* count, float* out_scores, int* out_indices);

#define FH_TOPK_DEEP_MAX 1024
FH_API int fh_gallery_topk_deep_dev(fh_gallery* g, const float* d_queries, const uint32_t* d_masks , int nq, int k,
                                    float* d_scores , int* d_indices ,
                                    int* d_ids , void* stream);
FH_API int fh_topk_from_scores(const float* scores, long long n, long long index_base, const uint32_t* tags ,
                               uint32_t mask, int k, float* out_scores, int* out_indices);
FH_API int fh_debug_deep_blocks(const float* scores, long long n, const uint32_t* tags , uint32_t mask, int k,
                                long long* out_blocks);

FH_API int fh_timing_enable(int on);
FH_API int fh_timing_num_tags(void);
FH_API int fh_timing_collect(double* ms, double* flops, double* bytes, long long* launches, int n);
FH_API int fh_timing_collect_ops(double* ms, double* flops, int* tag, int cap);
FH_API int fh_det_set_conv_cfg(fh_det* d, int cfg, int stream_k);
FH_API int fh_rec_set_conv_cfg(fh_rec* r, int cfg, int stream_k);
FH_API int fh_det_set_winograd(fh_det* d, int on);
FH_API int fh_rec_set_winograd(fh_rec* r, int on);
FH_API int fh_rec_set_wino_fusion(fh_rec* r, int on);
FH_API int fh_rec_set_shortcut_fold(fh_rec* r, int on);
enum fh_precision { FH_PREC_FP32 = 0, FH_PREC_BF16X2 = 1, FH_PREC_F32X3 = 2 };
FH_API int fh_rec_set_precision(fh_rec* r, int mode, float* worst);
FH_API int fh_rec_get_precision(fh_rec* r);
FH_API int fh_rec_set_wino_x3(fh_rec* r, int on);
FH_API int fh_rec_get_wino_x3(fh_rec* r);
FH_API int fh_rec_get_conv_x3(fh_rec* r);
FH_API int fh_rec_get_pw_x3(fh_rec* r);
FH_API int fh_det_set_x3(fh_det* d, int on);
FH_API int fh_det_get_x3(fh_det* d);
FH_API int fh_det_set_cus(fh_det* d, int cus);
FH_API int fh_rec_set_cus(fh_rec* r, int cus);
FH_API int fh_det_set_fused_stem(fh_det* d, int on);
FH_API int fh_rec_set_fused_stem(fh_rec* r, int on);
FH_API int fh_det_set_fused_front(fh_det* d, int on);
FH_API int fh_det_set_halo_conv(fh_det* d, int on);

FH_API int fh_imread(const char* path, unsigned char** bgr, int* rows, int* cols);
FH_API int fh_image_decode(const unsigned char* bytes, size_t n, unsigned char** bgr, int* rows, int* cols);
FH_API void fh_image_free(unsigned char* bgr);

typedef struct fh_jpeg_comp {
    int32_t h, v, wblocks, hblocks, dw, dh;
    int64_t coef_off;
    uint16_t quant[64];
} fh_jpeg_comp;
typedef struct fh_jpeg_desc {
    int32_t width, height, rows, cols, ncomp, hmax, vmax, color, orientation, reserved;
    int64_t coef_count;
    fh_jpeg_comp comp[3];
} fh_jpeg_desc;
FH_API int fh_jpeg_header(const unsigned char* bytes, size_t n, fh_jpeg_desc* desc);
FH_API int fh_jpeg_entropy(const unsigned char* bytes, size_t n, fh_jpeg_desc* desc, int16_t* coef, size_t cap);
FH_API int fh_jpeg_reconstruct(const fh_jpeg_desc* desc, const int16_t* coef, unsigned char* bgr, int step);
FH_API int fh_jpeg_desc_check(const fh_jpeg_desc* desc);
typedef struct fh_jpegdec fh_jpegdec;
FH_API fh_jpegdec* fh_jpegdec_create(void);
FH_API void fh_jpegdec_destroy(fh_jpegdec* dec);
FH_API int fh_jpeg_reconstruct_batch_dev(fh_jpegdec* dec, const fh_jpeg_desc* descs, int n, const int16_t* d_coef, const long long* coef_base,
                                         const fh_frame* out_frames, void* stream);
typedef struct fh_blob { const unsigned char* bytes; size_t n; } fh_blob;
FH_API int fh_jpeg_decode_batch(fh_jpegdec* dec, const fh_blob* files, int n, int threads, fh_frame* frames_out, int* status, void* stream);
FH_API int fh_pipeline_run_files(fh_det* d, fh_rec* r, fh_jpegdec* dec, const fh_blob* files, int n, int threads, float score_thr,
                                 float nms_thr, int faces_per_frame, fh_face* faces, int* frame_of, float* emb, int cap, int* status);

FH_API int fh_jpeg_quant_tables(int quality, uint16_t* luma, uint16_t* chroma);
FH_API int fh_jpeg_enc_desc(int width, int height, int gray, int subsampling, int quality, fh_jpeg_desc* desc);
FH_API int fh_jpeg_enc_check(const fh_jpeg_desc* desc);
FH_API int fh_jpeg_forward(const fh_jpeg_desc* desc, const unsigned char* bgr, int step, int16_t* coef, size_t cap);
FH_API int fh_jpeg_write(const fh_jpeg_desc* desc, const int16_t* coef, unsigned char* out, size_t cap, size_t* written);
FH_API size_t fh_jpeg_write_bound(const fh_jpeg_desc* desc);
FH_API int fh_imwrite_jpeg(const char* path, const unsigned char* bgr, int rows, int cols, int step, int quality, int subsampling);
typedef struct fh_jpegenc fh_jpegenc;
FH_API fh_jpegenc* fh_jpegenc_create(void);
FH_API void fh_jpegenc_destroy(fh_jpegenc* enc);
FH_API int fh_jpeg_forward_batch_dev(fh_jpegenc* enc, const fh_jpeg_desc* descs, int n, const fh_frame* frames, int16_t* d_coef,
                                     const long long* coef_base, void* stream);
FH_API int fh_jpeg_encode_batch(fh_jpegenc* enc, const fh_frame* frames, int n, int quality, int subsampling, int threads, fh_blob* files_out,
                                void* stream);

FH_API int fh_memcpy_d2h(void* host_dst, const void* dev_src, size_t bytes);
FH_API int fh_resize_u8c3_dev(const uint8_t* d_src, int sh, int sw, int sstep, uint8_t* d_dst, int dh, int dw, int dstep,
                              void* stream);
FH_API int fh_conv_forward_dev(const float* d_in, const float* d_wt_packed, const float* d_bias, float* d_out, int batch,
                               int h, int w, int cin, int cout, int ksize, int stride, int kpad, int cfg, void* stream);
FH_API int fh_conv_forward_ex_dev(const float* d_in, const float* d_wt_packed, const float* d_bias, float* d_out, int batch,
                                  int h, int w, int cin, int cout, int ksize, int stride, int kpad, int cfg, int precision,
                                  const float* d_sc_in, int sc_h, int sc_w, int sc_c, int sc_stride, int cus, void* stream);
FH_API int fh_conv_forward_ep_dev(const float* d_in, const float* d_wt_packed, const float* d_bias, float* d_out, int batch,
                                  int h, int w, int cin, int cout, int ksize, int stride, int kpad, int cfg, int precision,
                                  const float* d_sc_in, int sc_h, int sc_w, int sc_c, int sc_stride, int cus, int act, const float* d_res,
                                  void* stream);
FH_API int fh_conv_winograd_dev(const float* d_in, const float* w_ohwi_host, const float* d_bias, float* d_out, int batch, int h, int w,
                                int cin, int cout, void* stream);
FH_API int fh_conv_winograd_ex_dev(const float* d_in, const float* w_ohwi_host, const float* d_bias, float* d_out, int batch, int h, int w,
                                   int cin, int cout, int precision, void* stream);
FH_API int fh_conv_wino2_dev(const float* d_in, const float* w_ohwi_host, const float* d_bias, const float* d_slope, const float* d_res,
                             float* d_out, int batch, int h, int w, int cin, int cout, int act, int bias_cls, void* stream);
FH_API int fh_conv_wino2_ex_dev(const float* d_in, const float* w_ohwi_host, const float* d_bias, const float* d_slope, const float* d_res,
                                float* d_out, float* d_out2, const float* d_s2, const float* d_t2, int n_outs, float* const* d_outs,
                                const int* oc0, const int* oact, int batch, int h, int w, int cin, int cout, int act, int bias_cls,
                                void* stream);
FH_API double fh_debug_wino2_clock_mhz(void);
FH_API int fh_set_graph_replay(int on);
FH_API const float* fh_det_workspace_dev(fh_det* d);
FH_API int fh_det_graph_stats(fh_det* d, long long* replays);
FH_API int fh_rec_graph_stats(fh_rec* r, long long* replays);
FH_API int fh_debug_streamk(int drop_publish, int timeout_ms);
FH_API int fh_debug_conv_plan(int what, const int* in, int n_in, long long* out, int n_out);
FH_API int fh_debug_wino_slots(int slots);
FH_API int fh_debug_cluster_tiles(int tiles_per_wg);
FH_API int fh_debug_hist_copies(int copies);
FH_API int fh_debug_pairs_room(int room);
FH_API int fh_debug_tag_skip(int on);
FH_API int fh_debug_pack_bf16x2_dev(const float* d_in, float* d_out, long long n);
FH_API long long fh_debug_wino_gemm_rows(int batch, int h, int w, int k, int n, int mixed);
FH_API int fh_debug_wino_gemm_dev(const float* d_V, const float* d_U, float* d_M, int batch, int h, int w, int k, int n, int precision,
                                  int mixed, void* stream);
FH_API int fh_debug_topk_merge_strided_dev(const float* d_ps, const int* d_pi, int nparts, int nq, int k, long long part_stride,
                                           float* d_scores, int* d_indices, void* stream);
FH_API int fh_conv_wt_rows(int cout);
FH_API int fh_conv_pack_weights(const float* w_ohwi, int cout, int cin, int ksize, float* dst_packed);
FH_API int fh_conv_kpad(int ktot);

#ifdef __cplusplus
}
#endif
#endif
```

Measured before the change: 14210 faces/s.

## Add three-piece bf16 MFMA variant of fused F(2x2) Winograd conv

Adds a fused Winograd F(2x2,3x3) kernel for cin==64 layers that splits the transformed input and the weights into three bf16 pieces each and accumulates six bf16 MFMA products, emulating fp32 precision on the bf16 matrix cores. Weights are pre-packed into the three-piece layout at load time. The engine dispatches to this kernel when x3 precision mode is on and there are enough workgroups to fill the CUs. The aim is to replace the fp32 Winograd GEMM with faster bf16 matrix-core math, at the cost of extra weight memory and six MFMAs per product instead of one.

```diff
diff --git a/facerecognizeonnx_amd/_lib.py b/facerecognizeonnx_amd/_lib.py
--- a/facerecognizeonnx_amd/_lib.py
+++ b/facerecognizeonnx_amd/_lib.py
@@ -266,6 +266,7 @@
     "fh_rec_get_wino_x3": (_i, [_vp]),
     "fh_rec_get_conv_x3": (_i, [_vp]),
     "fh_rec_get_pw_x3": (_i, [_vp]),
+    "fh_rec_get_wino2_x3": (_i, [_vp]),
     "fh_det_set_x3": (_i, [_vp, _i]),
     "fh_det_get_x3": (_i, [_vp]),
     "fh_rec_set_shortcut_fold": (_i, [_vp, _i]),
@@ -299,6 +300,8 @@
     "fh_debug_wino_gemm_rows": (_ll, [_i, _i, _i, _i, _i, _i]),
     "fh_debug_wino_gemm_dev": (_i, [_vp, _vp, _vp, _i, _i, _i, _i, _i, _i, _i, _vp]),
     "fh_debug_wino2_clock_mhz": (_d, []),
+    "fh_conv_wino2_prec_dev": (_i, [_vp, _vp, _vp, _vp, _vp, _vp, _vp, _vp, _vp, _i, _i, _i, _i, _i, _i, _i, _i, _i, _vp]),
+    "fh_debug_wino2_pack_x3": (_i, [_vp, _i, _i, _vp]),
     "fh_conv_wino2_dev": (_i, [_vp, _vp, _vp, _vp, _vp, _vp, _i, _i, _i, _i, _i, _i, _i, _vp]),
     "fh_conv_wino2_ex_dev": (_i, [_vp, _vp, _vp, _vp, _vp, _vp, _vp, _vp, _vp, _i, _vp, _vp, _vp, _i, _i, _i, _i, _i, _i, _i, _vp]),
     "fh_conv_wt_rows": (_i, [_i]),
diff --git a/facerecognizeonnx_amd/csrc/api.cpp b/facerecognizeonnx_amd/csrc/api.cpp
--- a/facerecognizeonnx_amd/csrc/api.cpp
+++ b/facerecognizeonnx_amd/csrc/api.cpp
@@ -1826,6 +1826,7 @@
 int fh_rec_get_wino_x3(fh_rec* r) { return r && r->rec.net().wino_x3() ? 1 : 0; }
 int fh_rec_get_conv_x3(fh_rec* r) { return r ? r->rec.net().conv_x3_layers() : 0; }
 int fh_rec_get_pw_x3(fh_rec* r) { return r ? r->rec.net().pw_x3_layers() : 0; }
+int fh_rec_get_wino2_x3(fh_rec* r) { return r ? r->rec.net().wino2_x3_layers() : 0; }
 int fh_det_set_x3(fh_det* d, int on) {
     if (!d) return arg_error("null handle");
     Owns owns(&d->det.net());
@@ -2051,6 +2052,43 @@
                       int batch, int h, int w, int cin, int cout, int act, int bias_cls, void* stream) {
     return fh_conv_wino2_ex_dev(d_in, w_ohwi, d_bias, d_slope, d_res, d_out, nullptr, nullptr, nullptr, 0, nullptr, nullptr, nullptr, batch, h, w,
                                 cin, cout, act, bias_cls, stream);
+}
+int fh_conv_wino2_prec_dev(const float* d_in, const float* w_ohwi, const float* d_bias, const float* d_slope, const float* d_res, float* d_out,
+                           float* d_out2, const float* d_s2, const float* d_t2, int batch, int h, int w, int cin, int cout, int act, int bias_cls,
+                           int precision, int cus, void* stream) {
+    if (!d_in || !w_ohwi || batch <= 0 || h <= 0 || w <= 0 || cin <= 0 || cout <= 0 || cus < 0 || (!d_out && !d_out2) ||
+        (precision != FH_PREC_FP32 && precision != FH_PREC_F32X3))
+        return arg_error("fh_conv_wino2_prec_dev: bad argument");
+    if (d_out2 && (!d_s2 || !d_t2)) return arg_error("fh_conv_wino2_prec_dev: a second output needs its scale and shift");
+    if (precision == FH_PREC_F32X3 && !fh::wino2_x3_shape_ok(cin, cout))
+        return arg_error("fh_conv_wino2_prec_dev: this layer has no three-piece bf16 form (it needs cin == 64 and cout % 64 == 0)");
+    if (cin != 64 || cout % 64) return arg_error("fh_conv_wino2_prec_dev: plain layers need cin == 64 and cout % 64 == 0");
+    Owns owns(nullptr);
+    return guarded([&] {
+        fh::ConvArgs a{};
+        a.in = d_in; a.bias = d_bias; a.slope = d_slope; a.res = d_res; a.out1 = d_out; a.out2 = d_out2; a.s2 = d_s2; a.t2 = d_t2;
+        a.B = batch; a.H = h; a.W = w; a.Ho = h; a.Wo = w; a.Cin = cin; a.Cout = cout; a.ks = 3; a.stride = 1; a.pad = 1;
+        a.act = act; a.bias_cls = bias_cls; a.res_mode = d_res ? (int)fh::ResMode::SAME : (int)fh::ResMode::NONE;
+        a.cus = cus;
+        const bool x3 = precision == FH_PREC_F32X3;
+        if (!(x3 ? fh::wino2_x3_ok(a) : fh::wino2_ok(a))) throw std::runtime_error("fh_conv_wino2_prec_dev: layer shape not supported by the fused F(2x2) kernel");
+        std::vector<float> u(x3 ? fh::wino2_x3_weight_floats(cin, cout) : fh::wino2_weight_floats(cin, cout));
+        if (x3) fh::wino2_pack_weights_x3(w_ohwi, cout, cin, reinterpret_cast<unsigned short*>(u.data()));
+        else fh::wino2_pack_weights(w_ohwi, cout, cin, u.data());
+        fh::DevBuf dU;
+        dU.ensure(u.size() * sizeof(float));
+        FH_HIP(hipMemcpy(dU.p, u.data(), u.size() * sizeof(float), hipMemcpyHostToDevice));
+        a.wt = dU.as<float>();
+        if (x3) fh::launch_wino2_x3(a, S(stream)); else fh::launch_wino2(a, S(stream));
+        FH_HIP(hipGetLastError());
+        FH_HIP(hipStreamSynchronize(S(stream)));
+        return 0;
+    });
+}
+int fh_debug_wino2_pack_x3(const float* w_ohwi, int cout, int cin, unsigned short* dst) {
+    if (!w_ohwi || !dst || !fh::wino2_x3_shape_ok(cin, cout))
+        return arg_error("fh_debug_wino2_pack_x3: this layer has no three-piece bf16 form (it needs cin == 64 and cout % 64 == 0)");
+    return guarded([&] { fh::wino2_pack_weights_x3(w_ohwi, cout, cin, dst); return 0; });
 }
 double fh_debug_wino2_clock_mhz(void) { return fh::wino2_debug_clock_mhz(); }
 int fh_conv_wt_rows(int cout) { return fh::conv_wt_rows(cout); }
@@ -2117,6 +2155,8 @@
         out[2] = bn && fh::conv_pw_x3_pays(out[1], g.Kpad, g.Cout, in[10], knobs) ? 1 : 0;
     } else if (what == 7 && need(4, 1) && in[0] >= 0 && in[1] > 0 && in[2] > 0 && in[3] > 0) {
         out[0] = fh::conv_pw_x3_pays(in[0], in[1], in[2], in[3], knobs) ? 1 : 0;
+    } else if (what == 8 && need(2, 1) && in[0] >= 0 && in[1] > 0) {
+        out[0] = fh::wino2_x3_pays(in[0], in[1], knobs) ? 1 : 0;
     } else {
         return arg_error("fh_debug_conv_plan: unknown question, wrong array lengths or a non-positive size");
     }
diff --git a/facerecognizeonnx_amd/csrc/conv_plan.h b/facerecognizeonnx_amd/csrc/conv_plan.h
--- a/facerecognizeonnx_amd/csrc/conv_plan.h
+++ b/facerecognizeonnx_amd/csrc/conv_plan.h
@@ -24,6 +24,7 @@
     int conv_x3 = 1;
     int pw_x3 = 1;
     int pw_x3_bn = 0;
+    int wino2_x3 = 1;
 };
 inline const ConvKnobs& conv_knobs() {
     static const ConvKnobs k = [] {
@@ -32,6 +33,7 @@
         env("FACEHIP_SK_B_RATIO", v.sk_b_ratio); env("FACEHIP_SK_MIN_OWNER", v.sk_min_owner); env("FACEHIP_SK_MARGIN", v.sk_margin2);
         env("FACEHIP_TALL_TAIL_Q", v.tall_tail_q); env("FACEHIP_CONV_PW", v.conv_pw); env("FACEHIP_CONV_TALL", v.conv_tall);
         env("FACEHIP_EP_DIRECT", v.ep_direct); env("FACEHIP_CONV_X3", v.conv_x3); env("FACEHIP_PW_X3", v.pw_x3); env("FACEHIP_PW_X3_BN", v.pw_x3_bn);
+        env("FACEHIP_WINO2_X3", v.wino2_x3);
         return v;
     }();
     return k;
@@ -88,6 +90,12 @@
     return tiles >= (long)cus * (Cout < 32 ? 2 : 1) && Kpad >= PW_X3_MIN_KPAD;
 }
 
+inline bool wino2_x3_pays(long workgroups, int cus, const ConvKnobs& k) {
+    if (!k.wino2_x3 || workgroups <= 0 || cus <= 0) return false;
+    if (k.wino2_x3 == 2) return true;
+    return workgroups * 2 >= (long)cus * 3;
+}
+
 struct ConvTallPlan { int tiles, rows_a; size_t lds; };
 inline ConvTallPlan conv_tall_plan(const ConvGeom& g, int BM, int BN, int rp, int T, int tiles_n, int cus, const ConvKnobs& k) {
     const int occ = BM == 256 ? 2 : 3;
diff --git a/facerecognizeonnx_amd/csrc/conv_wino2.hip b/facerecognizeonnx_amd/csrc/conv_wino2.hip
--- a/facerecognizeonnx_amd/csrc/conv_wino2.hip
+++ b/facerecognizeonnx_amd/csrc/conv_wino2.hip
@@ -262,6 +262,202 @@
 #endif
 }
 
+
+__device__ __forceinline__ constexpr int w2_key(int pr, int pc) { return 2 * ((pc + 4 * (pr & 1)) & 7); }
+
+template <int NW>
+__device__ __forceinline__ void w2_load_halo(const ConvArgs& p, char* const halo, const int lane, const int wv, const int gn, const int gy, const int gx) {
+    const int H = p.H, W = p.W;
+    const int col = lane & 15, pl = lane >> 4;
+    const int y0 = 8 * gy - 1 + (pl >> 1), x0 = 8 * gx - 1 + (pl & 1);
+    const float* const img = p.in + ((size_t)gn * H * W + (size_t)y0 * W + x0) * 64;
+#pragma unroll
+    for (int i = 0; i < 25; ++i) {
+        const int pr = i / 5, pc = i - 5 * pr;
+        const int y = y0 + 2 * pr, x = x0 + 2 * pc;
+        const bool ok = (unsigned)y < (unsigned)H && (unsigned)x < (unsigned)W;
+        if (NW > 1 && (i % NW) != wv) continue;
+        lds_dma16(ok ? img + ((long)2 * pr * W + 2 * pc) * 64 + ((col ^ w2_key(pr, pc)) << 2) : p.zeros, halo + i * 1024);
+    }
+}
+
+template <int F, int CB>
+__device__ __forceinline__ void w2_y_update(v4f (&Y)[2][2][CB], const v4f (&M)[CB]) {
+    constexpr int i = F >> 2, j = F & 3;
+    constexpr int c00 = kAT[0][i] * kAT[0][j], c01 = kAT[0][i] * kAT[1][j], c10 = kAT[1][i] * kAT[0][j], c11 = kAT[1][i] * kAT[1][j];
+#pragma unroll
+    for (int cb = 0; cb < CB; ++cb) {
+        if constexpr (c00 > 0) Y[0][0][cb] += M[cb]; else if constexpr (c00 < 0) Y[0][0][cb] -= M[cb];
+        if constexpr (c01 > 0) Y[0][1][cb] += M[cb]; else if constexpr (c01 < 0) Y[0][1][cb] -= M[cb];
+        if constexpr (c10 > 0) Y[1][0][cb] += M[cb]; else if constexpr (c10 < 0) Y[1][0][cb] -= M[cb];
+        if constexpr (c11 > 0) Y[1][1][cb] += M[cb]; else if constexpr (c11 < 0) Y[1][1][cb] -= M[cb];
+        if constexpr (c00 != 0) asm volatile("" : "+v"(Y[0][0][cb]));
+        if constexpr (c01 != 0) asm volatile("" : "+v"(Y[0][1][cb]));
+        if constexpr (c10 != 0) asm volatile("" : "+v"(Y[1][0][cb]));
+        if constexpr (c11 != 0) asm volatile("" : "+v"(Y[1][1][cb]));
+    }
+}
+
+template <int CB>
+__device__ __forceinline__ void w2_store_plain(const ConvArgs& p, const v4f (&Y)[2][2][CB], const int gn, const int oy0, const int ox0, const int n0) {
+    const int Cout = p.Cout;
+    const float* __restrict__ res = p.res;
+    float* __restrict__ out1 = p.out1;
+    float* __restrict__ out2 = p.out2;
+    const bool relu = p.act == (int)Act::RELU, prelu = p.act == (int)Act::PRELU;
+    bool live[4]; size_t row[4]; v4f b4[4][CB], r4[4][CB], sl[CB];
+#pragma unroll
+    for (int cb = 0; cb < CB; ++cb) sl[cb] = prelu ? *reinterpret_cast<const v4f*>(p.slope + n0 + 16 * cb) : v4f{1.f, 1.f, 1.f, 1.f};
+#pragma unroll
+    for (int q = 0; q < 4; ++q) {
+        const int oy = oy0 + (q >> 1), ox = ox0 + (q & 1);
+        live[q] = oy < p.Ho && ox < p.Wo;
+        const int oyc = min(oy, p.Ho - 1), oxc = min(ox, p.Wo - 1);
+        row[q] = (((size_t)gn * p.Ho + oyc) * p.Wo + oxc) * Cout + n0;
+        const int cls = p.bias_cls ? 3 * (oyc == 0 ? 0 : oyc == p.Ho - 1 ? 2 : 1) + (oxc == 0 ? 0 : oxc == p.Wo - 1 ? 2 : 1) : 0;
+#pragma unroll
+        for (int cb = 0; cb < CB; ++cb) {
+            b4[q][cb] = p.bias ? *reinterpret_cast<const v4f*>(p.bias + cls * Cout + n0 + 16 * cb) : v4f{0.f, 0.f, 0.f, 0.f};
+            if (p.res_mode != (int)ResMode::NONE) r4[q][cb] = *reinterpret_cast<const v4f*>(res + row[q] + 16 * cb);
+        }
+    }
+#pragma unroll
+    for (int q = 0; q < 4; ++q) {
+        if (!live[q]) continue;
+#pragma unroll
+        for (int cb = 0; cb < CB; ++cb) {
+            v4f v;
+#pragma unroll
+            for (int e = 0; e < 4; ++e) v[e] = act1(Y[q >> 1][q & 1][cb][e] + b4[q][cb][e], relu, sl[cb][e]);
+            if (p.res_mode != (int)ResMode::NONE) v += r4[q][cb];
+            if (out1) *reinterpret_cast<v4f*>(out1 + row[q] + 16 * cb) = v;
+            if (out2) {
+                const v4f s2 = *reinterpret_cast<const v4f*>(p.s2 + n0 + 16 * cb), t2 = *reinterpret_cast<const v4f*>(p.t2 + n0 + 16 * cb);
+                *reinterpret_cast<v4f*>(out2 + row[q] + 16 * cb) = v * s2 + t2;
+            }
+        }
+    }
+}
+
+template <int CB, int NW>
+__global__ __launch_bounds__(64 * NW, 3) void wino2_x3_kernel(const ConvArgs p, const int tiles_n, const int tgx, const int tgy) {
+    extern __shared__ v4f w2sm[];
+    char* const halo = reinterpret_cast<char*>(w2sm);
+    const int lane = threadIdx.x & 63;
+    const int wv = NW == 1 ? 0 : __builtin_amdgcn_readfirstlane((int)threadIdx.x >> 6);
+    int blk;
+    {
+        const int n = gridDim.x, q = n >> 3, r = n & 7, x = blockIdx.x & 7;
+        blk = x * q + min(x, r) + (int)(blockIdx.x >> 3);
+    }
+    const int tile_n = blk % tiles_n, tg = blk / tiles_n;
+    const int per_img = tgx * tgy;
+    const int gn = tg / per_img, rem = tg - gn * per_img;
+    const int gy = rem / tgx, gx = rem - gy * tgx;
+    const int tn = lane & 15, kq = lane >> 4, tr = tn >> 2, tc = tn & 3;
+    w2_load_halo<NW>(p, halo, lane, wv, gn, gy, gx);
+    typedef const __attribute__((address_space(3))) v4f* lds_v4f;
+    const unsigned halo_base = (unsigned)(size_t)(__attribute__((address_space(3))) char*)halo;
+    unsigned rb[16];
+#pragma unroll
+    for (int dy = 0; dy < 4; ++dy)
+#pragma unroll
+        for (int dx = 0; dx < 4; ++dx) {
+            const int pl = (dy & 1) * 2 + (dx & 1), pr = tr + (dy >> 1), pc = tc + (dx >> 1);
+            rb[dy * 4 + dx] = halo_base + (unsigned)((4 * (pr * 5 + pc) + pl) * 256 + ((w2_key(pr, pc) ^ kq) << 4));
+        }
+    constexpr unsigned WSTEP = 3 * CB * 1024;
+    const char* wstep = reinterpret_cast<const char*>(p.wt) + ((size_t)tile_n * 32 * NW + (size_t)wv) * WSTEP;
+    const unsigned wlane = lane * 16;
+    bf16x8 wr[2][3][CB] = {};
+    auto fetch_w = [&](bool advance, int buf) __attribute__((always_inline)) {
+        unsigned adv = advance ? NW * WSTEP : 0;
+        asm volatile("" : "+s"(adv));
+        wstep += adv;
+#pragma unroll
+        for (int pl = 0; pl < 3; ++pl)
+#pragma unroll
+            for (int cb = 0; cb < CB; ++cb) wr[buf][pl][cb] = *reinterpret_cast<const bf16x8*>(wstep + wlane + (pl * CB + cb) * 1024);
+    };
+    v4f Y[2][2][CB], Mp[CB];
+#pragma unroll
+    for (int cb = 0; cb < CB; ++cb) {
+        Mp[cb] = v4f{0.f, 0.f, 0.f, 0.f};
+#pragma unroll
+        for (int a = 0; a < 4; ++a) Y[a >> 1][a & 1][cb] = v4f{0.f, 0.f, 0.f, 0.f};
+    }
+    v4f d[8] = {};
+    auto fetch_d = [&](auto fc, auto sc) __attribute__((always_inline)) {
+        constexpr int f = decltype(fc)::value, s = decltype(sc)::value;
+        constexpr int fi = f >> 2, fj = f & 3;
+        constexpr int ya = kYA[fi], yb = kYB[fi], xa = kYA[fj], xb = kYB[fj];
+#pragma unroll
+        for (int h = 0; h < 2; ++h) {
+            unsigned gxr = (2 * s + h) << 6;
+            asm volatile("" : "+s"(gxr));
+            d[4 * h + 0] = *reinterpret_cast<lds_v4f>((size_t)(rb[ya * 4 + xa] ^ gxr));
+            d[4 * h + 1] = *reinterpret_cast<lds_v4f>((size_t)(rb[ya * 4 + xb] ^ gxr));
+            d[4 * h + 2] = *reinterpret_cast<lds_v4f>((size_t)(rb[yb * 4 + xa] ^ gxr));
+            d[4 * h + 3] = *reinterpret_cast<lds_v4f>((size_t)(rb[yb * 4 + xb] ^ gxr));
+        }
+    };
+    auto stage = [&](auto fc) __attribute__((always_inline)) {
+        constexpr int f = decltype(fc)::value;
+        constexpr int fi = f >> 2, fj = f & 3;
+        constexpr int sab = kSA[fi] * kSB[fj], sba = kSB[fi] * kSA[fj], sbb = kSB[fi] * kSB[fj];
+        v4f M[CB];
+#pragma unroll
+        for (int cb = 0; cb < CB; ++cb) M[cb] = v4f{0.f, 0.f, 0.f, 0.f};
+        auto step = [&](auto sc) __attribute__((always_inline)) {
+            constexpr int s = decltype(sc)::value, k = f * 2 + s;
+            fetch_w(k + 1 < 32, (k + 1) & 1);
+            __builtin_amdgcn_sched_barrier(0);
+            v4f v0 = d[0], v1 = d[4];
+            v0 = sab > 0 ? v0 + d[1] : v0 - d[1];  v1 = sab > 0 ? v1 + d[5] : v1 - d[5];
+            v0 = sba > 0 ? v0 + d[2] : v0 - d[2];  v1 = sba > 0 ? v1 + d[6] : v1 - d[6];
+            v0 = sbb > 0 ? v0 + d[3] : v0 - d[3];  v1 = sbb > 0 ? v1 + d[7] : v1 - d[7];
+            asm volatile("" : "+v"(v0), "+v"(v1));
+            __builtin_amdgcn_sched_barrier(0);
+            if constexpr (s == 0) fetch_d(IC<f>{}, IC<1>{});
+            else if constexpr (f < 15) fetch_d(IC<f + 1>{}, IC<0>{});
+            bf16x8 vh, vm, vl;
+            gemm_split3(v0, v1, vh, vm, vl);
+            asm volatile("" : "+v"(vh), "+v"(vm), "+v"(vl));
+            __builtin_amdgcn_sched_barrier(0);
+            const bf16x8 (&w)[3][CB] = wr[k & 1];
+#pragma unroll
+            for (int cb = 0; cb < CB; ++cb) M[cb] = __builtin_amdgcn_mfma_f32_16x16x32_bf16(w[2][cb], vh, M[cb], 0, 0, 0);
+#pragma unroll
+            for (int cb = 0; cb < CB; ++cb) M[cb] = __builtin_amdgcn_mfma_f32_16x16x32_bf16(w[0][cb], vl, M[cb], 0, 0, 0);
+#pragma unroll
+            for (int cb = 0; cb < CB; ++cb) M[cb] = __builtin_amdgcn_mfma_f32_16x16x32_bf16(w[1][cb], vm, M[cb], 0, 0, 0);
+#pragma unroll
+            for (int cb = 0; cb < CB; ++cb) M[cb] = __builtin_amdgcn_mfma_f32_16x16x32_bf16(w[1][cb], vh, M[cb], 0, 0, 0);
+#pragma unroll
+            for (int cb = 0; cb < CB; ++cb) M[cb] = __builtin_amdgcn_mfma_f32_16x16x32_bf16(w[0][cb], vm, M[cb], 0, 0, 0);
+#pragma unroll
+            for (int cb = 0; cb < CB; ++cb) M[cb] = __builtin_amdgcn_mfma_f32_16x16x32_bf16(w[0][cb], vh, M[cb], 0, 0, 0);
+            __builtin_amdgcn_sched_barrier(0);
+        };
+        step(IC<0>{});
+        w2_y_update<(f + 15) & 15, CB>(Y, Mp);
+        step(IC<1>{});
+#pragma unroll
+        for (int cb = 0; cb < CB; ++cb) Mp[cb] = M[cb];
+        __builtin_amdgcn_sched_barrier(0);
+    };
+    fetch_w(false, 0);
+    asm volatile("s_waitcnt vmcnt(0)" ::: "memory");
+    if constexpr (NW > 1) __syncthreads();
+    fetch_d(IC<0>{}, IC<0>{});
+    stage(IC<0>{}); stage(IC<1>{}); stage(IC<2>{}); stage(IC<3>{}); stage(IC<4>{}); stage(IC<5>{}); stage(IC<6>{}); stage(IC<7>{});
+    stage(IC<8>{}); stage(IC<9>{}); stage(IC<10>{}); stage(IC<11>{}); stage(IC<12>{}); stage(IC<13>{}); stage(IC<14>{}); stage(IC<15>{});
+    w2_y_update<15, CB>(Y, Mp);
+    asm volatile("" ::: "memory");
+    __builtin_amdgcn_sched_barrier(0);
+    w2_store_plain<CB>(p, Y, gn, 2 * (4 * gy + tr), 2 * (4 * gx + tc), (tile_n * NW + wv) * 16 * CB + 4 * kq);
+}
+
 bool shape_ok(int Cin, int Cout) { return Cin == 64 && (Cout % 64 == 0 || Cout <= 32); }
 
 template <int CB, int NW, bool MERGED>
@@ -279,6 +475,23 @@
     timer.begin(s);
     hipLaunchKernelGGL((wino2_kernel<CB, NW, MERGED>), dim3((unsigned)(n_tg * tiles_n)), dim3(64 * NW), 25600, s, a, tiles_n, tgx, tgy, (int)n_tg);
     timer.end(s, 12, 2.0 * 16 * 16.0 * (double)n_tg * a.Cin * (16.0 * CB * NW * tiles_n), a.t_flops);
+}
+
+template <int CB, int NW>
+void launch_x3_cb(const ConvArgs& a, hipStream_t s) {
+    const int tgy = ((a.H + 1) / 2 + 3) / 4, tgx = ((a.W + 1) / 2 + 3) / 4;
+    const long n_tg = (long)a.B * tgy * tgx;
+    const int tiles_n = a.Cout / 64;
+    static const bool lds_ok = [] {
+        hipFuncAttributes fa{};
+        FH_HIP(hipFuncGetAttributes(&fa, reinterpret_cast<const void*>(&wino2_x3_kernel<CB, NW>)));
+        return fa.sharedSizeBytes % 256 == 0;
+    }();
+    if (!lds_ok) throw std::runtime_error("wino2: static LDS moved the halo off its 256-byte alignment (see the address XOR in fetch_d)");
+    KernelTimer& timer = KernelTimer::get();
+    timer.begin(s);
+    hipLaunchKernelGGL((wino2_x3_kernel<CB, NW>), dim3((unsigned)(n_tg * tiles_n)), dim3(64 * NW), 25600, s, a, tiles_n, tgx, tgy);
+    timer.end(s, 12, 2.0 * 16 * 16.0 * (double)n_tg * a.Cin * (64.0 * tiles_n), a.t_flops);
 }
 
 }
@@ -306,6 +519,37 @@
         }
 }
 
+bool wino2_x3_shape_ok(int Cin, int Cout) { return Cin == 64 && Cout > 0 && Cout % 64 == 0; }
+size_t wino2_x3_weight_floats(int Cin, int Cout) { return (size_t)16 * Cin * Cout * 3 / 2; }
+void wino2_pack_weights_x3(const float* w, int Cout, int Cin, unsigned short* dst) {
+    static const double Gm[4][3] = {{1, 0, 0}, {.5, .5, .5}, {.5, -.5, .5}, {0, 0, 1}};
+    if (!wino2_x3_shape_ok(Cin, Cout)) throw std::runtime_error("wino2_pack_weights_x3: layer shape not supported");
+    constexpr int CB = 2, nw = 2;
+    auto bits = [](float x) { unsigned u; memcpy(&u, &x, 4); return u; };
+    auto flt = [](unsigned u) { float x; memcpy(&x, &u, 4); return x; };
+    auto rne = [&](float x) { const unsigned u = bits(x); return (u + 0x7fffu + ((u >> 16) & 1u)) & 0xffff0000u; };
+    for (int co = 0; co < Cout; ++co)
+        for (int ci = 0; ci < Cin; ++ci) {
+            double g[3][3], t[4][3];
+            for (int k = 0; k < 9; ++k) g[k / 3][k % 3] = w[((size_t)co * 9 + k) * Cin + ci];
+            for (int i = 0; i < 4; ++i)
+                for (int x = 0; x < 3; ++x) t[i][x] = Gm[i][0] * g[0][x] + Gm[i][1] * g[1][x] + Gm[i][2] * g[2][x];
+            const int tn = co / 64, wave = (co % 64) / (16 * CB), cb = (co % (16 * CB)) / 16, m = co % 16;
+            const int gq = ci / 16, kq = (ci % 16) / 4, e = ci % 4, st = gq >> 1, j = 4 * (gq & 1) + e;
+            for (int f = 0; f < 16; ++f) {
+                const int i = f >> 2, jj = f & 3;
+                const volatile float u = (float)(t[i][0] * Gm[jj][0] + t[i][1] * Gm[jj][1] + t[i][2] * Gm[jj][2]);
+                const unsigned hb = bits(u) & 0xffff0000u;
+                const volatile float r = u - flt(hb);
+                const unsigned mb = rne(r);
+                const volatile float q = r - flt(mb);
+                const unsigned pieces[3] = {hb, mb, rne(q)};
+                const size_t step = (((size_t)tn * 16 + f) * 2 + st) * nw + wave;
+                for (int pl = 0; pl < 3; ++pl) dst[(((step * 3 + pl) * CB + cb) * 64 + kq * 16 + m) * 8 + j] = (unsigned short)(pieces[pl] >> 16);
+            }
+        }
+}
+
 bool wino2_ok(const ConvArgs& a) {
     if (!(a.ks == 3 && a.stride == 1 && a.pad == 1 && a.H == a.Ho && a.W == a.Wo && a.H >= 2 && a.W >= 2 && shape_ok(a.Cin, a.Cout) &&
           a.act != (int)Act::SIGMOID && !a.sc_in && !a.dw_w && !a.u8_src && a.wt_group_rows == 0 &&
@@ -347,4 +591,13 @@
     else launch_cb<4, 1, false>(a, s);
 }
 
-}
+bool wino2_x3_ok(const ConvArgs& a) { return wino2_ok(a) && a.n_outs == 0 && wino2_x3_shape_ok(a.Cin, a.Cout); }
+long wino2_x3_workgroups(const ConvArgs& a) { return (long)a.B * (((a.H + 1) / 2 + 3) / 4) * (((a.W + 1) / 2 + 3) / 4) * (a.Cout / 64); }
+void launch_wino2_x3(const ConvArgs& a_in, hipStream_t s) {
+    if (!wino2_x3_ok(a_in)) throw std::runtime_error("launch_wino2_x3: layer shape not supported");
+    ConvArgs a = a_in;
+    a.zeros = conv_zero_line();
+    launch_x3_cb<2, 2>(a, s);
+}
+
+}
diff --git a/facerecognizeonnx_amd/csrc/engine.cpp b/facerecognizeonnx_amd/csrc/engine.cpp
--- a/facerecognizeonnx_amd/csrc/engine.cpp
+++ b/facerecognizeonnx_amd/csrc/engine.cpp
@@ -182,6 +182,13 @@
                     wino2_pack_weights(op.weight.data(), op.Cout, op.Cin, u.data());
                     d.w2 = push(u.data(), u.size());
                     d.w2ok = true;
+                    if (wino2_x3_ok(probe)) {
+                        std::vector<float> u3(wino2_x3_weight_floats(op.Cin, op.Cout));
+                        wino2_pack_weights_x3(op.weight.data(), op.Cout, op.Cin, reinterpret_cast<unsigned short*>(u3.data()));
+                        d.w2x = push(u3.data(), u3.size());
+                        d.w2x_ok = true;
+                        ++wino2_x3_n_;
+                    }
                 }
             }
             if (op.kind == OpKind::CONV && op.ks == 3 && op.stride == 1 && op.pad == 1 && op.Cin >= kWinoMinCin && op.Cin % 32 == 0 &&
@@ -421,6 +428,7 @@
         FH_HIP(hipStreamSynchronize(s));
     }
     conv_x3_ = on && conv_x3_n_ > 0;
+    wino2_x3_ = on && wino2_x3_n_ > 0;
     set_pw_x3(on, s);
     return on ? layers : 0;
 }
@@ -510,6 +518,11 @@
                     break;
                 }
                 if (d.w2ok && winograd && force_cfg < 0 && d.sc_src < 0 && wino2_blocks(a) >= wino2_min_blocks()) {
+                    if (wino2_x3_ && d.w2x_ok && wino2_x3_pays(wino2_x3_workgroups(a), cus > 0 ? cus : conv_num_cus(), conv_knobs())) {
+                        a.wt = P + d.w2x;
+                        launch_wino2_x3(a, s);
+                        break;
+                    }
                     a.wt = P + d.w2;
                     launch_wino2(a, s);
                     break;
diff --git a/facerecognizeonnx_amd/csrc/engine.h b/facerecognizeonnx_amd/csrc/engine.h
--- a/facerecognizeonnx_amd/csrc/engine.h
+++ b/facerecognizeonnx_amd/csrc/engine.h
@@ -61,6 +61,7 @@
     int conv_x3_layers() const { return conv_x3_ ? conv_x3_n_ : 0; }
     int set_pw_x3(bool on, hipStream_t s);
     int pw_x3_layers() const { return pw_x3_ ? pw_x3_n_ : 0; }
+    int wino2_x3_layers() const { return wino2_x3_ ? wino2_x3_n_ : 0; }
     int cus = 0;
     int force_cfg = -1;
     bool sk_enable = true;
@@ -68,7 +69,7 @@
         return (long long)fuse_stem | (long long)fuse_front << 1 | (long long)winograd << 2 | (long long)halo_conv << 3 |
                (long long)fold_shortcut << 4 | (long long)fuse_wino << 5 | (long long)bf16x2_ << 6 | (long long)sk_enable << 7 |
                (long long)(cus & 0xffff) << 8 | (long long)((force_cfg + 1) & 0xff) << 24 | (long long)wino_x3_ << 32 | (long long)conv_x3_ << 33 |
-               (long long)pw_x3_ << 34;
+               (long long)pw_x3_ << 34 | (long long)wino2_x3_ << 35;
     }
 
   private:
@@ -89,6 +90,8 @@
         bool wino = false;
         size_t w2 = 0;
         bool w2ok = false;
+        size_t w2x = 0;
+        bool w2x_ok = false;
         int aff_src = -1;
         int aff_dst = -1;
         int bn_fold_src = -1;
@@ -114,8 +117,8 @@
     Plan plan_;
     std::vector<DevOp> dev_;
     DevBuf params_, arena_, partial_, wino_v_, wino_m_, w36_bf_, w36_x3_, wsc_x3_, wpw_x3_;
-    bool bf16x2_ = false, wino_x3_ = false, conv_x3_ = false, pw_x3_ = false;
-    int conv_x3_n_ = 0, pw_x3_n_ = 0;
+    bool bf16x2_ = false, wino_x3_ = false, conv_x3_ = false, pw_x3_ = false, wino2_x3_ = false;
+    int conv_x3_n_ = 0, pw_x3_n_ = 0, wino2_x3_n_ = 0;
     size_t wino_maxc_ = 0;
     size_t wino_elems_ = 0;
     int cap_ = 0;
diff --git a/facerecognizeonnx_amd/csrc/kernels.h b/facerecognizeonnx_amd/csrc/kernels.h
--- a/facerecognizeonnx_amd/csrc/kernels.h
+++ b/facerecognizeonnx_amd/csrc/kernels.h
@@ -108,6 +108,12 @@
 bool wino2_ok(const ConvArgs& a);
 void launch_wino2(const ConvArgs& a, hipStream_t s);
 long wino2_blocks(const ConvArgs& a);
+bool wino2_x3_shape_ok(int Cin, int Cout);
+size_t wino2_x3_weight_floats(int Cin, int Cout);
+void wino2_pack_weights_x3(const float* w_ohwi, int Cout, int Cin, unsigned short* dst);
+bool wino2_x3_ok(const ConvArgs& a);
+long wino2_x3_workgroups(const ConvArgs& a);
+void launch_wino2_x3(const ConvArgs& a, hipStream_t s);
 double wino2_debug_clock_mhz();
 const float* conv_zero_line();
 int conv_num_cus();
diff --git a/facerecognizeonnx_amd/csrc/plan.cpp b/facerecognizeonnx_amd/csrc/plan.cpp
--- a/facerecognizeonnx_amd/csrc/plan.cpp
+++ b/facerecognizeonnx_amd/csrc/plan.cpp
@@ -256,7 +256,7 @@
             x.group = (int)n.attr_i("group", 1);
             auto st = n.attr_ints("strides"); auto pd = n.attr_ints("pads"); auto dl = n.attr_ints("dilations");
             x.stride = st.empty() ? 1 : (int)st[0];
-            if (!st.empty() && st[0] != st[1]) fail("anisotropic stride");
+            if (!st.empty() && (st.size() < 2 || st[0] != st[1])) fail("anisotropic stride");
             x.pad = pd.empty() ? 0 : (int)pd[0];
             for (auto p : pd) if (p != x.pad) fail("asymmetric padding");
             for (auto d : dl) if (d != 1) fail("dilation != 1");
diff --git a/include/facehip.h b/include/facehip.h
--- a/include/facehip.h
+++ b/include/facehip.h
@@ -295,6 +295,7 @@
 FH_API int fh_rec_get_wino_x3(fh_rec* r);
 FH_API int fh_rec_get_conv_x3(fh_rec* r);
 FH_API int fh_rec_get_pw_x3(fh_rec* r);
+FH_API int fh_rec_get_wino2_x3(fh_rec* r);
 FH_API int fh_det_set_x3(fh_det* d, int on);
 FH_API int fh_det_get_x3(fh_det* d);
 FH_API int fh_det_set_cus(fh_det* d, int cus);
@@ -376,6 +377,10 @@
 FH_API int fh_rec_graph_stats(fh_rec* r, long long* replays);
 FH_API int fh_debug_streamk(int drop_publish, int timeout_ms);
 FH_API int fh_debug_conv_plan(int what, const int* in, int n_in, long long* out, int n_out);
+FH_API int fh_conv_wino2_prec_dev(const float* d_in, const float* w_ohwi_host, const float* d_bias, const float* d_slope, const float* d_res,
+                                  float* d_out, float* d_out2, const float* d_s2, const float* d_t2, int batch, int h, int w, int cin,
+                                  int cout, int act, int bias_cls, int precision, int cus, void* stream);
+FH_API int fh_debug_wino2_pack_x3(const float* w_ohwi_host, int cout, int cin, unsigned short* dst);
 FH_API int fh_debug_wino_slots(int slots);
 FH_API int fh_debug_cluster_tiles(int tiles_per_wg);
 FH_API int fh_debug_hist_copies(int copies);
```

New measurement: 14410 faces/s (median of 6 runs). +1.4%, better.
